# uc-vision/taichi-splatting

Measured on AMD Instinct MI355X. Metric: fwd+bwd Msplats/s, higher is better.
Workload: dtype f32; 1 GPU; config D: 6000000 random 3D gaussians, 2048x2048, SH deg 3, tile 16, fwd+bwd (render_gaussians, loss=image.sum()); n_gaussians=6000000, tile_size=16, sh_degree=3, mode=single, parallelism=single GPU

## Files before the change

### include/mi355_splat.h

```cpp
#ifndef MI355_SPLAT_H
#define MI355_SPLAT_H

#include <stddef.h>
#include <stdint.h>

#ifdef __cplusplus
extern "C" {
#endif

#define MS_VERSION 500
#define MS_ABI_GENERATION(version) ((version) / 100)

enum { MS_F32 = 0, MS_F64 = 1 };

enum {
  MS_ERR_BAD_ARG = -1,
  MS_ERR_UNSUPPORTED = -2,
  MS_ERR_TMP_TOO_SMALL = -3,
  MS_ERR_ABI = -4
};

typedef struct ms_raster_config {
  int32_t tile_size;
  int32_t antialias;
  int32_t use_alpha_blending;
  int32_t compute_visibility;
  int32_t compute_point_heuristic;
  int32_t reserved;
  double clamp_max_alpha;
  double alpha_threshold;
  double saturate_threshold;
} ms_raster_config;

int ms_version(void);
const char* ms_last_error_string(void);

int ms_project_fwd(const void* position, const void* log_scaling, const void* rotation,
                   const void* alpha_logit, const void* T_camera_world, const void* projection,
                   int image_w, int image_h, double near_plane, double far_plane,
                   double blur_cov, double clamp_margin, double alpha_threshold,
                   int64_t n, void* out_points7, void* out_depth, int32_t* out_flag,
                   int dtype, void* stream);

int ms_project_gather(const void* points7, const void* depth, const int32_t* flag,
                      const int32_t* scan, int64_t n, double near_plane, double far_plane,
                      void* out_points7, void* out_depth, void* out_ndc_depth,
                      int64_t* out_indexes, int dtype, void* stream);

int ms_project_bwd(const void* position, const void* log_scaling, const void* rotation,
                   const void* alpha_logit, const void* T_camera_world, const void* projection,
                   int image_w, int image_h, double blur_cov, double clamp_margin,
                   const int64_t* indexes, int64_t v, const void* grad_points7,
                   const void* grad_depth, void* grad_position, void* grad_log_scaling,
                   void* grad_rotation, void* grad_alpha_logit, void* grad_camera,
                   int dtype, void* stream);

int ms_sh_fwd(const void* params, const void* positions, const int64_t* indexes,
              const void* camera_pos, int64_t v, int f, int degree, void* out,
              int dtype, void* stream);

int ms_sh_fwd_active(const void* params, const void* positions, const int64_t* indexes,
                     const void* camera_pos, int64_t v, int f, int degree, int active_degree, void* out,
                     int dtype, void* stream);

int ms_sh_bwd(const void* params, const void* positions, const int64_t* indexes,
              const void* camera_pos, int64_t v, int f, int degree, const void* out,
              const void* grad_out, void* grad_params, void* grad_positions,
              void* grad_camera_pos, int unique_indexes, int dtype, void* stream);

int ms_sh_bwd_active(const void* params, const void* positions, const int64_t* indexes,
                     const void* camera_pos, int64_t v, int f, int degree, int active_degree, const void* out,
                     const void* grad_out, void* grad_params, void* grad_positions,
                     void* grad_camera_pos, int unique_indexes, int dtype, void* stream);

int ms_tile_count(const float* points7, const int32_t* order, int64_t v, int image_w, int image_h,
                  int tile_size, float alpha_threshold, int tile_row_begin, int tile_row_end,
                  int32_t* out_counts, float* out_ordered_points7 ,
                  void* stream);

int ms_depth_sort_keys(const void* depth, int64_t v, int depth16, double ndc_near, double ndc_far,
                       uint32_t* out_keys, int32_t* out_values, int dtype, void* stream);

int ms_depth_argsort(const void* depth, int64_t v, int depth16, double ndc_near, double ndc_far, int dtype,
                     uint32_t* out_sorted_keys, int32_t* out_order, void* tmp, size_t* tmp_bytes, void* stream);

int ms_exclusive_scan_i32(const int32_t* in, int64_t n, int32_t* out, int32_t* total_host,
                          void* tmp, size_t* tmp_bytes, void* stream);

int ms_tile_emit(const float* points7, const float* depth, const int32_t* order, const int32_t* cum,
                 int64_t v, int image_w, int image_h, int tile_size, float alpha_threshold,
                 int tile_row_begin, int tile_row_end, int key_mode,
                 int points_are_ordered ,
                 void* out_keys, int32_t* out_values, void* stream);

int ms_tile_emit_keys64(const float* points7, const void* depth, int depth_dtype, const int32_t* cum, int64_t v,
                        int image_w, int image_h, int tile_size, float alpha_threshold, int tile_row_begin,
                        int tile_row_end, int depth16, double ndc_near, double ndc_far, uint64_t* out_keys,
                        int32_t* out_values, void* stream);

int ms_radix_sort_pairs(const void* keys_in, const int32_t* values_in, void* keys_out,
                        int32_t* values_out, int64_t n, int key_bytes, int begin_bit, int end_bit,
                        void* tmp, size_t* tmp_bytes, void* stream);

int ms_segmented_sort_pairs(const int32_t* keys_in, const int32_t* values_in, int32_t* keys_out,
                            int32_t* values_out, int64_t n, const int64_t* start_offsets,
                            const int64_t* end_offsets, int64_t num_segments, void* stream);

int ms_find_ranges(const void* sorted_keys, int64_t k, int key_bytes, int tile_shift,
                   int64_t num_tiles, int32_t* out_ranges, void* stream);

int ms_tile_depth_sort(const int32_t* tile_ranges, int64_t num_tiles, uint64_t* sorted_keys,
                       int32_t* overlap_to_point, uint64_t* scratch, void* stream);

int ms_raster_fwd(const void* points7, const void* features, const int32_t* tile_ranges,
                  const int32_t* overlap_to_point, int image_w, int image_h, int f,
                  const ms_raster_config* cfg, void* out_image, void* out_alpha,
                  void* out_visibility, int tile_row_begin, int tile_row_end,
                  int dtype, void* stream);

int ms_raster_bwd(const void* points7, const void* features, const int32_t* tile_ranges,
                  const int32_t* overlap_to_point, const void* image, const void* grad_image,
                  int image_w, int image_h, int f, const ms_raster_config* cfg,
                  void* grad_points7, void* grad_features, void* point_heuristic,
                  int tile_row_begin, int tile_row_end, int dtype, void* stream);

#define MS_MOMENT_ROW 16
int ms_fixed_point_exponents(const float* amax_dev, int32_t* out_exp2, void* stream);
int ms_raster_bwd_moments(const void* points7, const void* features, const int32_t* tile_ranges,
                          const int32_t* overlap_to_point, const void* image, const void* grad_image,
                          int image_w, int image_h, const ms_raster_config* cfg, float* moments,
                          int deterministic, const int32_t* fixed_exp, int tile_row_begin, int tile_row_end,
                          void* stream);
int ms_raster_moments_finalize(const void* points7, const float* moments, int deterministic,
                               const int32_t* fixed_exp, int64_t n,
                               float* grad_points7, float* grad_features, float* point_heuristic,
                               void* stream);

size_t ms_raster_split_scratch_bytes(int64_t k_capacity, int tile_size, int split_min_run, int split_seg_len);
int ms_raster_fwd_split(const float* points7, const float* features, const int32_t* tile_ranges,
                        const int32_t* overlap_to_point, int64_t k_capacity, int image_w, int image_h,
                        const ms_raster_config* cfg, float* out_image, float* out_alpha, float* out_visibility,
                        void* split_scratch, int split_min_run, int split_seg_len, int tile_row_begin, int tile_row_end,
                        void* stream);
int ms_raster_bwd_moments_split(const float* points7, const float* features, const int32_t* tile_ranges,
                                const int32_t* overlap_to_point, int64_t k_capacity, const float* image,
                                const float* grad_image, int image_w, int image_h, const ms_raster_config* cfg,
                                float* moments, int deterministic, const int32_t* fixed_exp, const void* split_scratch,
                                int split_min_run, int split_seg_len, int tile_row_begin, int tile_row_end, void* stream);

int ms_probe_raster_bwd(void* start_event, void* stop_event);

#define MS_SPLAT_ROW 16
int ms_splat_rows_pack(const float* points7, const float* depth, const float* colours3, int64_t n, float* rows,
                       void* stream);
int ms_raster_fwd_rows(const float* rows, const int32_t* tile_ranges, const int32_t* overlap_to_point, int image_w,
                       int image_h, const ms_raster_config* cfg, float* out_image, float* out_alpha,
                       float* out_visibility, int tile_row_begin, int tile_row_end, void* stream);
int ms_raster_bwd_moments_rows(const float* rows, const int32_t* tile_ranges, const int32_t* overlap_to_point,
                               const float* image, const float* grad_image, int image_w, int image_h,
                               const ms_raster_config* cfg, float* moments, int deterministic,
                               const int32_t* fixed_exp, int tile_row_begin, int tile_row_end, void* stream);

#define MS_MAPPER_DIRECT 0
#define MS_MAPPER_PRESORT 1

typedef struct ms_frame_desc {
  uint32_t struct_size;
  uint32_t abi_version;
  int64_t n;
  int64_t k_capacity;
  int32_t image_w, image_h;
  int32_t dtype;
  int32_t f;
  int32_t sh_degree;
  int32_t depth16;
  int32_t tile_row_begin, tile_row_end;
  int32_t projected_input;
  int32_t mapper;
  int32_t split_long_runs;
  int32_t split_seg_len;
  int32_t sh_active_bands;
  double near_plane, far_plane, blur_cov, clamp_margin;
  ms_raster_config raster;
} ms_frame_desc;

typedef struct ms_frame_layout {
  size_t keep_n_bytes, scratch_n_bytes, keep_k_bytes, scratch_k_bytes;
  size_t points7, depth, colours, points7_f32, camera_position, counters, tile_ranges;
  size_t sorted_keys, order, counts, cum, ordered_points, tmp_n;
  size_t overlap_to_point;
  size_t keys, values, keys_sorted, tmp_k;
  size_t splat_rows;
  size_t split_scratch;
} ms_frame_layout;

typedef struct ms_frame_inputs {
  uint32_t struct_size;
  uint32_t reserved;
  const void *position, *log_scaling, *rotation, *alpha_logit, *feature, *T_camera_world, *projection;
  const void *points7, *depth, *colours;
  int32_t* longest_run_host;
  void* colours_ready_event;
} ms_frame_inputs;

enum { MS_BACKWARD_ALL = 0, MS_BACKWARD_GAUSSIANS = 1, MS_BACKWARD_RASTER = 2 };

typedef struct ms_frame_grads {
  uint32_t struct_size;
  uint32_t reserved;
  const void* image;
  const void* grad_image;
  const void *extra_points7, *extra_depth, *extra_colours;
  void* moments;
  int32_t deterministic;
  int32_t stage;
  const int32_t* fixed_exp;
  void *grad_points7, *grad_colours;
  void *grad_position, *grad_log_scaling, *grad_rotation, *grad_alpha_logit, *grad_feature, *grad_camera;
  void* point_heuristic;
  void* point_visibility;
  int32_t boundary_stride;
  int32_t gather_world;
  const void* gather_rows;
  const int32_t* gather_slots;
  const int32_t* gather_route;
  int32_t boundary_form;
  int32_t grad_image_broadcast;
} ms_frame_grads;

enum { MS_BOUNDARY_AXIS_SIGMA = 0, MS_BOUNDARY_COVARIANCE = 1 };

int ms_frame_layout_query(const ms_frame_desc* desc, ms_frame_layout* out);
int ms_frame_uses_moments(const ms_frame_desc* desc, int deterministic);
int ms_frame_project(const ms_frame_desc* desc, const ms_frame_inputs* in, void* keep_n, void* stream);
int ms_frame_project_count(const ms_frame_desc* desc, const ms_frame_inputs* in, void* keep_n, void* scratch_n,
                           int32_t* k_host, void* k_event, void* stream);
int ms_frame_sh_colours(const ms_frame_desc* desc, const ms_frame_inputs* in, void* keep_n, void* stream);
int ms_frame_map_raster(const ms_frame_desc* desc, const ms_frame_inputs* in, void* keep_n, void* scratch_n,
                        void* keep_k, void* scratch_k, void* out_image, void* out_alpha, void* out_visibility,
                        void* stream);
int ms_frame_backward(const ms_frame_desc* desc, const ms_frame_inputs* in, void* keep_n, void* keep_k,
                      const ms_frame_grads* g, void* stream);

int ms_fractional_step(int kind, int vector, float* lr_step, const int64_t* indexes,
                       const float* weight, float* m, float* v, const float* total_weight,
                       const float* grad, int64_t m_count, int d, float lr, float beta1,
                       float beta2, float eps, int bias_correction, void* stream);

int ms_fractional_update(int kind, int group_type, float* param, const float* grad, float* m, float* v,
                         const int64_t* indexes, const float* weight, const float* total_weight,
                         const float* grad_scale, const float* basis, const float* mask_lr,
                         const float* point_lr, int64_t m_count, int d, float lr, float beta1,
                         float beta2, float eps, float clip, int bias_correction, void* stream);

typedef struct ms_optim_group {
  uint32_t struct_size;
  int32_t group_type;
  float* param;
  const float* grad;
  float* m;
  float* v;
  const float* basis;
  const float* mask_lr;
  const float* point_lr;
  int32_t d;
  int32_t bias_correction;
  float lr, beta1, beta2, eps;
  float clip;
  float reserved;
} ms_optim_group;
int ms_optim_step_groups(int kind, const ms_optim_group* groups, int num_groups, const int64_t* indexes,
                         const float* weight, const float* total_weight, const float* grad_scale, int64_t m_count,
                         void* stream);

int ms_optim_visibility_weights(const int64_t* indexes, const float* visibility, int64_t m_count, float vis_beta,
                                float vis_smooth, float floor_eps, float skip_threshold, float* running_vis,
                                float* total_weight, float* out_weight, float* out_grad_scale, void* stream);

int ms_morton_codes64(const float* points3, int64_t n, const float* lower3_host, const float* inc3_host,
                      uint32_t size, uint64_t* out_codes, void* stream);

#define MS_KNN_BLOCK 256
int ms_knn_points(const float* points3, const int32_t* order, int64_t n, int k,
                  float* out_dist2, int32_t* out_index , int64_t* out_stats ,
                  void* tmp, size_t* tmp_bytes, void* stream);

int ms_camera_position(const void* t_camera_world, void* out_position3, int dtype, void* stream);

int ms_strip_route_blocks(int v);
int ms_strip_route_count(const float* points7, const float* depth ,
                         int v, int image_h, int tile_size, float alpha_threshold,
                         const int32_t* bounds_host, int world, int32_t* out_route,
                         int32_t* out_block_counts, int64_t* out_send_counts, void* stream);
int ms_strip_route_pack(const float* points7, const float* features, const float* depths,
                        const int64_t* ids, int f, int v, int world, int64_t index_offset,
                        const int32_t* route, const int32_t* block_offsets, const int64_t* send_counts,
                        int64_t bucket_capacity, int32_t* overflow_flag,
                        float* out_rows, int64_t* out_send_index, void* stream);
int ms_strip_route_pack_slots(const float* points7, const float* features, const float* depths,
                              const int64_t* ids, int f, int v, int world, int64_t index_offset,
                              const int32_t* route, const int32_t* block_offsets, const int64_t* send_counts,
                              int64_t bucket_capacity, int32_t* overflow_flag,
                              float* out_rows, int64_t* out_send_index, int32_t* out_slots, void* stream);
int ms_strip_route_pack_split(const float* points7, const float* features, const float* depths,
                              const int64_t* ids, int f, int v, int world, int64_t index_offset,
                              const int32_t* route, const int32_t* block_offsets, const int64_t* send_counts,
                              int64_t bucket_capacity, int32_t* overflow_flag, float* out_geometry_rows,
                              float* out_colour_rows, int64_t* out_send_index, int32_t* out_slots, void* stream);
int ms_strip_unpack(const float* rows, int64_t m, int f, float* out_points7, float* out_features,
                    float* out_depths, int64_t* out_ids, void* stream);
int ms_strip_return_grads(const float* back_rows, const int64_t* send_index, const int32_t* route,
                          int f, int64_t s, float* grad_points7, float* grad_features, void* stream);
int ms_strip_return_rows(const float* back_rows, const int64_t* send_index, const int32_t* route,
                         int f, int64_t s, float* grad_rows, void* stream);

int ms_densify_plan(const uint8_t* prune, const uint8_t* split, int64_t n, int children, int32_t* scan,
                    int32_t* counts, int32_t* counts_host, void* tmp, size_t* tmp_bytes, void* stream);
int ms_densify_table(const int32_t* scan, int64_t n, int children, int64_t n_out, int32_t* src_row,
                     int32_t* child_slot, void* stream);

typedef struct ms_densify_array {
  uint32_t struct_size;
  int32_t child_fill;
  const void* src;
  void* dst;
  int64_t row_bytes;
} ms_densify_array;
int ms_densify_move(const ms_densify_array* arrays, int num_arrays, const int32_t* src_row, const int32_t* child_slot,
                    int64_t n_src, int64_t n_out, void* stream);

int ms_densify_split2d(float* position, float* log_scaling, const float* rotation, float* depths, int64_t first,
                       int64_t count, int children, const float* z, const float* scale, const float* depth_offset,
                       void* stream);
int ms_densify_split3d(float* position, float* log_scaling, const float* rotation, int64_t first, int64_t count,
                       int children, const float* z, const float* scale, void* stream);

enum { MS_PAD_SAME = 0, MS_PAD_VALID = 1 };
int ms_photometric_fwd(const void* image, const void* target, int H, int W, int C, int dtype, int padding,
                       double lambda, void* map_a, void* map_b, void* map_c, void* tmp, size_t* tmp_bytes,
                       void* out_loss, void* stream);
int ms_photometric_bwd(const void* image, const void* target, const void* map_a, const void* map_b, const void* map_c,
                       const void* grad_out, int H, int W, int C, int dtype, int padding, double lambda,
                       void* grad_image, void* stream);

#define MS_SCENE_XFORM_ROWS 256
enum {
  MS_SCENE_XFORM_SRT = 0,
  MS_SCENE_XFORM_LN_S = 12,
  MS_SCENE_XFORM_QUAT = 13,
  MS_SCENE_XFORM_M1 = 17,
  MS_SCENE_XFORM_M2 = 26,
  MS_SCENE_XFORM_M3 = 51,
  MS_SCENE_XFORM_VALUES = 100
};
int ms_scene_transform(const void* position, void* out_position, const void* log_scaling, void* out_log_scaling,
                       const void* rotation, void* out_rotation, const void* feature, void* out_feature,
                       int64_t n, int f, int sh_degree, int dtype, const double* transform_host, void* stream);

#define MS_COVERAGE_CAMERA_VALUES 20
#define MS_COVERAGE_MAX_CAMERAS 65535
int ms_camera_coverage(const void* position, const void* log_scaling, const void* rotation, const void* alpha_logit,
                       const void* cameras, int num_cameras, double blur_cov, double clamp_margin,
                       double alpha_threshold, int64_t n, int32_t* out_count, void* out_max_rate, void* out_min_depth,
                       uint32_t* out_mask , int dtype, void* stream);

#define MS_RELOCATE_MAX_RATIO 51
enum { MS_RELOCATE_COPY = 0, MS_RELOCATE_ZERO_TOUCHED = 1, MS_RELOCATE_INHERIT = 2, MS_RELOCATE_OPACITY = 3,
       MS_RELOCATE_SCALE = 4 };
typedef struct ms_relocate_array {
  uint32_t struct_size;
  int32_t role;
  void* data;
  const void* fresh;
  int64_t row_bytes;
} ms_relocate_array;
int ms_relocate_weights(const float* alpha_logit, int64_t n, float threshold, int64_t* weights, int32_t* count,
                        int64_t* counts, void* stream);
int ms_relocate_draw(const int64_t* weights, const int64_t* cdf, const uint64_t* random, int64_t n, int32_t* src,
                     int32_t* count, int64_t* counts, void* stream);
int ms_relocate_fresh(const float* alpha_logit, const float* log_scaling, int scale_dims, const int32_t* count, int64_t n,
                      double min_opacity, const double* binomials, float* fresh_opacity, float* fresh_scale,
                      int64_t* counts, void* stream);
int ms_relocate_move(const ms_relocate_array* arrays, int num_arrays, const int32_t* src, const int32_t* count, int64_t n,
                     void* stream);

int ms_perturb_positions(float* position, const float* log_scaling, const float* rotation, const float* alpha_logit,
                         const float* z, int64_t n, float step, double k, double x0, void* stream);

#define MS_KMEANS_MAX_D 64
#define MS_KMEANS_MAX_K 65536
#define MS_KMEANS_CHUNK 128
#define MS_KMEANS_UPDATE_CHUNK 1024
int ms_kmeans_assign(const float* x, int64_t n, int d, const float* codebook, int k, int32_t* out_index,
                     float* out_dist2 , void* tmp, size_t* tmp_bytes, void* stream);
int ms_kmeans_update(const float* x, const int32_t* index, const float* weights , int64_t n, int d,
                     int k, float* codebook, int32_t* out_counts, double* out_weight_sums , void* tmp,
                     size_t* tmp_bytes, void* stream);

#ifdef __cplusplus
}
#endif
#endif
```

### taichi_splatting_amd/_lib.py

```python
from __future__ import annotations

import ctypes
from ctypes import c_int, c_int32, c_int64, c_double, c_float, c_void_p, c_size_t, c_char_p, POINTER
import os
from pathlib import Path
import subprocess
from typing import Optional

import torch

PACKAGE_DIR = Path(__file__).resolve().parent
CSRC_DIR = PACKAGE_DIR / 'csrc'
LIB_PATH = Path(os.environ.get('MS_SPLAT_LIB') or PACKAGE_DIR / 'libmi355_splat.so')

MS_F32, MS_F64 = 0, 1
BACKWARD_ALL, BACKWARD_GAUSSIANS, BACKWARD_RASTER = 0, 1, 2
BOUNDARY_AXIS_SIGMA, BOUNDARY_COVARIANCE = 0, 1
MAPPER_DIRECT, MAPPER_PRESORT = 0, 1
ABI_VERSION = 500
PAD_SAME, PAD_VALID = 0, 1
MOMENT_ROW = 16
SPLAT_ROW = 16
KNN_BLOCK = 256
SCENE_XFORM_ROWS = 256
SCENE_XFORM_VALUES = 100
COVERAGE_CAMERA_VALUES = 20
COVERAGE_MAX_CAMERAS = 65535
RELOCATE_MAX_RATIO = 51
KMEANS_MAX_D, KMEANS_MAX_K = 64, 65536
KMEANS_CHUNK = 128
KMEANS_UPDATE_CHUNK = 1024
RELOCATE_COPY, RELOCATE_ZERO_TOUCHED, RELOCATE_INHERIT, RELOCATE_OPACITY, RELOCATE_SCALE = range(5)

_lib: Optional[ctypes.CDLL] = None


class RasterConfigC(ctypes.Structure):
  _fields_ = [
    ('tile_size', c_int32),
    ('antialias', c_int32),
    ('use_alpha_blending', c_int32),
    ('compute_visibility', c_int32),
    ('compute_point_heuristic', c_int32),
    ('reserved', c_int32),
    ('clamp_max_alpha', c_double),
    ('alpha_threshold', c_double),
    ('saturate_threshold', c_double),
  ]


class _SizedStructure(ctypes.Structure):

  def __init__(self, *args, **kw):
    assert not args, "keyword arguments only: the leading fields are the struct's size / ABI version"
    super().__init__(**kw)
    self.struct_size = ctypes.sizeof(type(self))
    if hasattr(self, 'abi_version'):
      self.abi_version = ABI_VERSION


class FrameDescC(_SizedStructure):
  _fields_ = [
    ('struct_size', ctypes.c_uint32), ('abi_version', ctypes.c_uint32),
    ('n', c_int64), ('k_capacity', c_int64),
    ('image_w', c_int32), ('image_h', c_int32),
    ('dtype', c_int32), ('f', c_int32), ('sh_degree', c_int32), ('depth16', c_int32),
    ('tile_row_begin', c_int32), ('tile_row_end', c_int32),
    ('projected_input', c_int32), ('mapper', c_int32), ('split_long_runs', c_int32), ('split_seg_len', c_int32),
    ('sh_active_bands', c_int32),
    ('near_plane', c_double), ('far_plane', c_double), ('blur_cov', c_double), ('clamp_margin', c_double),
    ('raster', RasterConfigC),
  ]


class FrameLayoutC(ctypes.Structure):
  _fields_ = [(name, c_size_t) for name in (
    'keep_n_bytes', 'scratch_n_bytes', 'keep_k_bytes', 'scratch_k_bytes',
    'points7', 'depth', 'colours', 'points7_f32', 'camera_position', 'counters', 'tile_ranges',
    'sorted_keys', 'order', 'counts', 'cum', 'ordered_points', 'tmp_n',
    'overlap_to_point',
    'keys', 'values', 'keys_sorted', 'tmp_k',
    'splat_rows', 'split_scratch')]


class FrameInputsC(_SizedStructure):
  _fields_ = [('struct_size', ctypes.c_uint32), ('reserved', ctypes.c_uint32)] + [(name, c_void_p) for name in (
    'position', 'log_scaling', 'rotation', 'alpha_logit', 'feature', 'T_camera_world', 'projection',
    'points7', 'depth', 'colours', 'longest_run_host', 'colours_ready_event')]


class FrameGradsC(_SizedStructure):
  _fields_ = [
    ('struct_size', ctypes.c_uint32), ('reserved', ctypes.c_uint32),
    ('image', c_void_p), ('grad_image', c_void_p),
    ('extra_points7', c_void_p), ('extra_depth', c_void_p), ('extra_colours', c_void_p),
    ('moments', c_void_p), ('deterministic', c_int32), ('stage', c_int32), ('fixed_exp', c_void_p),
    ('grad_points7', c_void_p), ('grad_colours', c_void_p),
    ('grad_position', c_void_p), ('grad_log_scaling', c_void_p), ('grad_rotation', c_void_p),
    ('grad_alpha_logit', c_void_p), ('grad_feature', c_void_p), ('grad_camera', c_void_p),
    ('point_heuristic', c_void_p),
    ('point_visibility', c_void_p),
    ('boundary_stride', c_int32), ('gather_world', c_int32),
    ('gather_rows', c_void_p), ('gather_slots', c_void_p), ('gather_route', c_void_p),
    ('boundary_form', c_int32), ('grad_image_broadcast', c_int32),
  ]


class OptimGroupC(ctypes.Structure):
  _fields_ = [
    ('struct_size', ctypes.c_uint32), ('group_type', c_int32),
    ('param', c_void_p), ('grad', c_void_p), ('m', c_void_p), ('v', c_void_p),
    ('basis', c_void_p), ('mask_lr', c_void_p), ('point_lr', c_void_p),
    ('d', c_int32), ('bias_correction', c_int32),
    ('lr', c_float), ('beta1', c_float), ('beta2', c_float), ('eps', c_float), ('clip', c_float), ('reserved', c_float),
  ]


class DensifyArrayC(ctypes.Structure):
  _fields_ = [
    ('struct_size', ctypes.c_uint32), ('child_fill', c_int32),
    ('src', c_void_p), ('dst', c_void_p), ('row_bytes', c_int64),
  ]


class RelocateArrayC(ctypes.Structure):
  _fields_ = [
    ('struct_size', ctypes.c_uint32), ('role', c_int32),
    ('data', c_void_p), ('fresh', c_void_p), ('row_bytes', c_int64),
  ]


SIGNATURES = {
  'ms_version': (c_int, []),
  'ms_last_error_string': (c_char_p, []),
  'ms_project_fwd': (c_int, [c_void_p] * 6 + [c_int, c_int] + [c_double] * 5 + [c_int64, c_void_p, c_void_p, c_void_p, c_int, c_void_p]),
  'ms_project_gather': (c_int, [c_void_p] * 4 + [c_int64, c_double, c_double] + [c_void_p] * 4 + [c_int, c_void_p]),
  'ms_project_bwd': (c_int, [c_void_p] * 6 + [c_int, c_int, c_double, c_double, c_void_p, c_int64] + [c_void_p] * 7 + [c_int, c_void_p]),
  'ms_sh_fwd': (c_int, [c_void_p] * 4 + [c_int64, c_int, c_int, c_void_p, c_int, c_void_p]),
  'ms_sh_bwd': (c_int, [c_void_p] * 4 + [c_int64, c_int, c_int] + [c_void_p] * 5 + [c_int, c_int, c_void_p]),
  'ms_sh_fwd_active': (c_int, [c_void_p] * 4 + [c_int64, c_int, c_int, c_int, c_void_p, c_int, c_void_p]),
  'ms_sh_bwd_active': (c_int, [c_void_p] * 4 + [c_int64, c_int, c_int, c_int] + [c_void_p] * 5 + [c_int, c_int, c_void_p]),
  'ms_tile_count': (c_int, [c_void_p, c_void_p, c_int64, c_int, c_int, c_int, c_float, c_int, c_int, c_void_p, c_void_p, c_void_p]),
  'ms_depth_sort_keys': (c_int, [c_void_p, c_int64, c_int, c_double, c_double, c_void_p, c_void_p, c_int, c_void_p]),
  'ms_depth_argsort': (c_int, [c_void_p, c_int64, c_int, c_double, c_double, c_int, c_void_p, c_void_p, c_void_p, POINTER(c_size_t), c_void_p]),
  'ms_exclusive_scan_i32': (c_int, [c_void_p, c_int64, c_void_p, c_void_p, c_void_p, POINTER(c_size_t), c_void_p]),
  'ms_tile_emit_keys64': (c_int, [c_void_p, c_void_p, c_int, c_void_p, c_int64, c_int, c_int, c_int, c_float, c_int, c_int, c_int, ctypes.c_double, ctypes.c_double, c_void_p, c_void_p, c_void_p]),
  'ms_tile_emit': (c_int, [c_void_p, c_void_p, c_void_p, c_void_p, c_int64, c_int, c_int, c_int, c_float, c_int, c_int, c_int, c_int, c_void_p, c_void_p, c_void_p]),
  'ms_radix_sort_pairs': (c_int, [c_void_p] * 4 + [c_int64, c_int, c_int, c_int, c_void_p, POINTER(c_size_t), c_void_p]),
  'ms_segmented_sort_pairs': (c_int, [c_void_p] * 4 + [c_int64, c_void_p, c_void_p, c_int64, c_void_p]),
  'ms_find_ranges': (c_int, [c_void_p, c_int64, c_int, c_int, c_int64, c_void_p, c_void_p]),
  'ms_tile_depth_sort': (c_int, [c_void_p, c_int64, c_void_p, c_void_p, c_void_p, c_void_p]),
  'ms_fractional_step': (c_int, [c_int, c_int] + [c_void_p] * 7 + [c_int64, c_int, c_float, c_float, c_float, c_float, c_int, c_void_p]),
  'ms_morton_codes64': (c_int, [c_void_p, c_int64, c_void_p, c_void_p, ctypes.c_uint32, c_void_p, c_void_p]),
  'ms_knn_points': (c_int, [c_void_p, c_void_p, c_int64, c_int, c_void_p, c_void_p, c_void_p, c_void_p, POINTER(c_size_t), c_void_p]),
  'ms_camera_position': (c_int, [c_void_p, c_void_p, c_int, c_void_p]),
  'ms_strip_route_blocks': (c_int, [c_int]),
  'ms_strip_route_count': (c_int, [c_void_p, c_void_p, c_int, c_int, c_int, c_float, c_void_p, c_int, c_void_p, c_void_p, c_void_p, c_void_p]),
  'ms_strip_route_pack': (c_int, [c_void_p] * 4 + [c_int, c_int, c_int, c_int64] + [c_void_p] * 3 + [c_int64, c_void_p] + [c_void_p] * 2 + [c_void_p]),
  'ms_strip_unpack': (c_int, [c_void_p, c_int64, c_int] + [c_void_p] * 4 + [c_void_p]),
  'ms_strip_return_grads': (c_int, [c_void_p, c_void_p, c_void_p, c_int, c_int64, c_void_p, c_void_p, c_void_p]),
  'ms_strip_route_pack_slots': (c_int, [c_void_p] * 4 + [c_int, c_int, c_int, c_int64] + [c_void_p] * 3 + [c_int64] + [c_void_p] * 5),
  'ms_strip_route_pack_split': (c_int, [c_void_p] * 4 + [c_int, c_int, c_int, c_int64] + [c_void_p] * 3 + [c_int64] + [c_void_p] * 6),
  'ms_strip_return_rows': (c_int, [c_void_p, c_void_p, c_void_p, c_int, c_int64, c_void_p, c_void_p]),
  'ms_fractional_update': (c_int, [c_int, c_int] + [c_void_p] * 11 + [c_int64, c_int, c_float, c_float, c_float, c_float, c_float, c_int, c_void_p]),
  'ms_raster_fwd': (c_int, [c_void_p] * 4 + [c_int, c_int, c_int, POINTER(RasterConfigC)] + [c_void_p] * 3 + [c_int, c_int, c_int, c_void_p]),
  'ms_fixed_point_exponents': (c_int, [c_void_p, c_void_p, c_void_p]),
  'ms_raster_bwd_moments': (c_int, [c_void_p] * 6 + [c_int, c_int, POINTER(RasterConfigC), c_void_p, c_int, c_void_p, c_int, c_int, c_void_p]),
  'ms_raster_moments_finalize': (c_int, [c_void_p, c_void_p, c_int, c_void_p, c_int64, c_void_p, c_void_p, c_void_p, c_void_p]),
  'ms_raster_split_scratch_bytes': (c_size_t, [c_int64, c_int, c_int, c_int]),
  'ms_raster_fwd_split': (c_int, [c_void_p] * 4 + [c_int64, c_int, c_int, POINTER(RasterConfigC)] + [c_void_p] * 4 + [c_int, c_int, c_int, c_int, c_void_p]),
  'ms_raster_bwd_moments_split': (c_int, [c_void_p] * 4 + [c_int64, c_void_p, c_void_p, c_int, c_int, POINTER(RasterConfigC), c_void_p, c_int, c_void_p, c_void_p, c_int, c_int, c_int, c_int, c_void_p]),
  'ms_splat_rows_pack': (c_int, [c_void_p, c_void_p, c_void_p, c_int64, c_void_p, c_void_p]),
  'ms_raster_fwd_rows': (c_int, [c_void_p] * 3 + [c_int, c_int, POINTER(RasterConfigC)] + [c_void_p] * 3 + [c_int, c_int, c_void_p]),
  'ms_raster_bwd_moments_rows': (c_int, [c_void_p] * 5 + [c_int, c_int, POINTER(RasterConfigC), c_void_p, c_int, c_void_p, c_int, c_int, c_void_p]),
  'ms_frame_layout_query': (c_int, [POINTER(FrameDescC), POINTER(FrameLayoutC)]),
  'ms_frame_uses_moments': (c_int, [POINTER(FrameDescC), c_int]),
  'ms_frame_project': (c_int, [POINTER(FrameDescC), POINTER(FrameInputsC), c_void_p, c_void_p]),
  'ms_frame_sh_colours': (c_int, [POINTER(FrameDescC), POINTER(FrameInputsC), c_void_p, c_void_p]),
  'ms_frame_project_count': (c_int, [POINTER(FrameDescC), POINTER(FrameInputsC), c_void_p, c_void_p, c_void_p, c_void_p, c_void_p]),
  'ms_frame_map_raster': (c_int, [POINTER(FrameDescC), POINTER(FrameInputsC)] + [c_void_p] * 8),
  'ms_frame_backward': (c_int, [POINTER(FrameDescC), POINTER(FrameInputsC), c_void_p, c_void_p, POINTER(FrameGradsC), c_void_p]),
  'ms_probe_raster_bwd': (c_int, [c_void_p, c_void_p]),
  'ms_optim_step_groups': (c_int, [c_int, POINTER(OptimGroupC), c_int, c_void_p, c_void_p, c_void_p, c_void_p, c_int64, c_void_p]),
  'ms_optim_visibility_weights': (c_int, [c_void_p, c_void_p, c_int64, c_float, c_float, c_float, c_float] + [c_void_p] * 5),
  'ms_raster_bwd': (c_int, [c_void_p] * 6 + [c_int, c_int, c_int, POINTER(RasterConfigC)] + [c_void_p] * 3 + [c_int, c_int, c_int, c_void_p]),
  'ms_densify_plan': (c_int, [c_void_p, c_void_p, c_int64, c_int, c_void_p, c_void_p, c_void_p, c_void_p, POINTER(c_size_t), c_void_p]),
  'ms_densify_table': (c_int, [c_void_p, c_int64, c_int, c_int64, c_void_p, c_void_p, c_void_p]),
  'ms_densify_move': (c_int, [POINTER(DensifyArrayC), c_int, c_void_p, c_void_p, c_int64, c_int64, c_void_p]),
  'ms_densify_split2d': (c_int, [c_void_p] * 4 + [c_int64, c_int64, c_int] + [c_void_p] * 4),
  'ms_densify_split3d': (c_int, [c_void_p] * 3 + [c_int64, c_int64, c_int] + [c_void_p] * 3),
  'ms_photometric_fwd': (c_int, [c_void_p, c_void_p, c_int, c_int, c_int, c_int, c_int, c_double] + [c_void_p] * 4 + [POINTER(c_size_t), c_void_p, c_void_p]),
  'ms_photometric_bwd': (c_int, [c_void_p] * 6 + [c_int, c_int, c_int, c_int, c_int, c_double, c_void_p, c_void_p]),
  'ms_scene_transform': (c_int, [c_void_p] * 8 + [c_int64, c_int, c_int, c_int, POINTER(c_double), c_void_p]),
  'ms_camera_coverage': (c_int, [c_void_p] * 5 + [c_int, c_double, c_double, c_double, c_int64] + [c_void_p] * 4 + [c_int, c_void_p]),
  'ms_relocate_weights': (c_int, [c_void_p, c_int64, c_float] + [c_void_p] * 4),
  'ms_relocate_draw': (c_int, [c_void_p] * 3 + [c_int64] + [c_void_p] * 4),
  'ms_relocate_fresh': (c_int, [c_void_p, c_void_p, c_int, c_void_p, c_int64, c_double] + [c_void_p] * 5),
  'ms_relocate_move': (c_int, [POINTER(RelocateArrayC), c_int, c_void_p, c_void_p, c_int64, c_void_p]),
  'ms_perturb_positions': (c_int, [c_void_p] * 5 + [c_int64, c_float, c_double, c_double, c_void_p]),
  'ms_kmeans_assign': (c_int, [c_void_p, c_int64, c_int, c_void_p, c_int, c_void_p, c_void_p, c_void_p, POINTER(c_size_t), c_void_p]),
  'ms_kmeans_update': (c_int, [c_void_p] * 3 + [c_int64, c_int, c_int] + [c_void_p] * 4 + [POINTER(c_size_t), c_void_p]),
}


def build(verbose: bool = False, jobs: Optional[int] = None) -> Path:
  jobs = jobs or os.cpu_count() or 4
  cmd = ['make', '-C', str(CSRC_DIR), f'-j{jobs}']
  proc = subprocess.run(cmd, capture_output=True, text=True)
  if proc.returncode != 0:
    raise RuntimeError(f"building libmi355_splat.so failed:\n{proc.stdout}\n{proc.stderr}")
  if verbose:
    print(proc.stdout)
  return LIB_PATH


def load() -> ctypes.CDLL:
  global _lib
  if _lib is not None:
    return _lib
  if not LIB_PATH.exists():
    raise RuntimeError(
      f"{LIB_PATH} not found: the gfx950 kernel library has not been built. "
      "Run `python -c 'import __graft_entry__ as g; g.build()'` or `make -C taichi_splatting_amd/csrc`. "
      "There is no CPU fallback for this path.")
  lib = ctypes.CDLL(str(LIB_PATH))
  for name, (restype, argtypes) in SIGNATURES.items():
    fn = getattr(lib, name)
    fn.restype = restype
    fn.argtypes = argtypes
  _lib = lib
  return lib


def check(rc: int, what: str):
  if rc != 0:
    msg = load().ms_last_error_string().decode('utf-8', 'replace')
    if rc == -2:
      raise NotImplementedError(f"{what}: {msg}")
    if rc == -4:
      raise RuntimeError(f"{what}: ABI mismatch between taichi_splatting_amd/_lib.py and libmi355_splat.so: {msg}")
    if rc < 0:
      raise ValueError(f"{what}: {msg}")
    raise RuntimeError(f"{what}: HIP error {rc}: {msg}")


def ptr(t: Optional[torch.Tensor]) -> Optional[int]:
  if t is None:
    return None
  assert t.is_contiguous(), "tensor must be contiguous"
  return t.data_ptr()


def require_gpu(*tensors: torch.Tensor):
  for t in tensors:
    if t is not None and not t.is_cuda:
      raise RuntimeError(
        "taichi_splatting_amd runs on MI355X (gfx950) only: got a tensor on "
        f"{t.device}. There is no CPU fallback; move the inputs to the GPU.")


def dtype_code(dtype: torch.dtype) -> int:
  if dtype == torch.float32:
    return MS_F32
  if dtype == torch.float64:
    return MS_F64
  raise TypeError(f"unsupported dtype {dtype}: float32 or float64 expected")


def current_stream(device) -> int:
  return torch.cuda.current_stream(device).cuda_stream


def raster_config_c(config) -> RasterConfigC:
  return RasterConfigC(
    tile_size=config.tile_size, antialias=int(config.antialias),
    use_alpha_blending=int(config.use_alpha_blending),
    compute_visibility=int(config.compute_visibility),
    compute_point_heuristic=int(config.compute_point_heuristic), reserved=0,
    clamp_max_alpha=config.clamp_max_alpha, alpha_threshold=config.alpha_threshold,
    saturate_threshold=config.saturate_threshold)


def fixed_point_exponents(grad_image: torch.Tensor) -> torch.Tensor:
  amax = grad_image.detach().abs().amax().to(torch.float32).reshape(1)
  out = torch.empty((2,), dtype=torch.int32, device=grad_image.device)
  check(load().ms_fixed_point_exponents(amax.data_ptr(), out.data_ptr(), current_stream(grad_image.device)),
        "fixed_point_exponents")
  return out
```

### taichi_splatting_amd/csrc/frame.hip

```cpp
#include <cstdlib>
#include <cstring>
#include "common.h"
#include "frame_internal.h"
#include "raster_common.h"

namespace ms {

struct FrameGeom {
  int w_pad, h_pad, tiles_wide, tiles_high, num_tiles, tile_bits, row_begin, row_end;
  size_t es;
};

static FrameGeom frame_geom(const ms_frame_desc* d) {
  FrameGeom g;
  const int ts = d->raster.tile_size;
  g.tiles_wide = (d->image_w + ts - 1) / ts;
  g.tiles_high = (d->image_h + ts - 1) / ts;
  g.w_pad = g.tiles_wide * ts;
  g.h_pad = g.tiles_high * ts;
  g.num_tiles = g.tiles_wide * g.tiles_high;
  int bits = 1;
  while ((1ll << bits) < (long long)g.num_tiles) ++bits;
  g.tile_bits = bits;
  g.row_begin = d->tile_row_begin < 0 ? 0 : d->tile_row_begin;
  g.row_end = d->tile_row_end > g.tiles_high ? g.tiles_high : d->tile_row_end;
  g.es = d->dtype == MS_F64 ? 8 : 4;
  return g;
}

static int check_desc(const ms_frame_desc* d, const char* who) {
  if (!d) { set_error("%s: desc is null", who); return MS_ERR_BAD_ARG; }
  if (d->struct_size != sizeof(ms_frame_desc) || MS_ABI_GENERATION(d->abi_version) != MS_ABI_GENERATION(MS_VERSION)) {
    set_error("%s: ms_frame_desc of another ABI (struct_size %u, abi_version %u; this library: %u, %d) — set desc.struct_size = "
              "sizeof(ms_frame_desc) and desc.abi_version = MS_VERSION of the include/mi355_splat.h you compile against",
              who, d->struct_size, d->abi_version, (unsigned)sizeof(ms_frame_desc), MS_VERSION);
    return MS_ERR_ABI;
  }
  if (d->split_long_runs < 0 || d->split_seg_len < 0) { set_error("%s: negative split parameter", who); return MS_ERR_BAD_ARG; }
  if (d->n < 0 || d->k_capacity < 0) { set_error("%s: negative size", who); return MS_ERR_BAD_ARG; }
  if (d->n >= (1ll << 31) || d->k_capacity >= (1ll << 31)) { set_error("%s: sizes are int32 indexes (< 2^31)", who); return MS_ERR_BAD_ARG; }
  if (d->image_w <= 0 || d->image_h <= 0) { set_error("%s: bad image size", who); return MS_ERR_BAD_ARG; }
  if (d->dtype != MS_F32 && d->dtype != MS_F64) { set_error("%s: dtype must be MS_F32 or MS_F64", who); return MS_ERR_BAD_ARG; }
  const int ts = d->raster.tile_size;
  if (ts != 8 && ts != 16 && ts != 32) { set_error("%s: tile_size must be 8, 16 or 32 (got %d)", who, ts); return MS_ERR_UNSUPPORTED; }
  if (d->f < 1 || d->f > 4) { set_error("%s: 1..4 colour channels (got %d)", who, d->f); return MS_ERR_UNSUPPORTED; }
  if (d->sh_degree < -1 || d->sh_degree > 3) { set_error("%s: SH degree must be in [0, 3]", who); return MS_ERR_BAD_ARG; }
  if (d->sh_active_bands < 0 || d->sh_active_bands > d->sh_degree + 1) {
    set_error("%s: sh_active_bands must be 0 (all) or 1 .. sh_degree + 1 (got %d with sh_degree %d)", who, d->sh_active_bands, d->sh_degree);
    return MS_ERR_BAD_ARG;
  }
  if (d->mapper != MS_MAPPER_DIRECT && d->mapper != MS_MAPPER_PRESORT) { set_error("%s: mapper must be MS_MAPPER_DIRECT or MS_MAPPER_PRESORT (got %d)", who, d->mapper); return MS_ERR_BAD_ARG; }
  if (d->projected_input && d->sh_degree >= 0) { set_error("%s: projected input carries colours, not SH", who); return MS_ERR_BAD_ARG; }
  if (d->depth16) {
    const FrameGeom g = frame_geom(d);
    if (g.num_tiles > 65536) { set_error("%s: use_depth16 keys hold a 16 bit tile id: too many tiles", who); return MS_ERR_BAD_ARG; }
  }
  return 0;
}

static bool frame_uses_rows(const ms_frame_desc* d) {
  static const bool on = [] { const char* e = getenv("MS_SPLAT_ROWS"); return e && e[0] == '1'; }();
  return on && !d->projected_input && d->n > 0 && raster_uses_splat_rows(&d->raster, d->f, d->dtype);
}

static bool frame_uses_split(const ms_frame_desc* d) {
  return d->split_long_runs != 0 && d->n > 0 && d->k_capacity > 0 && raster_uses_splat_rows(&d->raster, d->f, d->dtype);
}
static SplitParams frame_split_params(const ms_frame_desc* d) {
  return split_params(d->raster.tile_size, d->split_long_runs, d->split_seg_len);
}

static int check_inputs(const ms_frame_inputs* in, const char* who) {
  if (!in) { set_error("%s: inputs are null", who); return MS_ERR_BAD_ARG; }
  if (in->struct_size != sizeof(ms_frame_inputs)) {
    set_error("%s: ms_frame_inputs of another ABI (struct_size %u, this library: %u)", who, in->struct_size, (unsigned)sizeof(ms_frame_inputs));
    return MS_ERR_ABI;
  }
  return 0;
}

static int check_grads(const ms_frame_grads* g, const char* who) {
  if (!g) { set_error("%s: grads are null", who); return MS_ERR_BAD_ARG; }
  if (g->struct_size != sizeof(ms_frame_grads)) {
    set_error("%s: ms_frame_grads of another ABI (struct_size %u, this library: %u)", who, g->struct_size, (unsigned)sizeof(ms_frame_grads));
    return MS_ERR_ABI;
  }
  return 0;
}

struct Carve {
  size_t off = 0;
  size_t take(size_t bytes) { const size_t o = off; off += align_up(bytes > 0 ? bytes : 1, 256); return o; }
};

static void frame_layout(const ms_frame_desc* d, ms_frame_layout* L) {
  const FrameGeom g = frame_geom(d);
  const size_t n = (size_t)d->n, k = (size_t)d->k_capacity;
  const bool own_points = !d->projected_input;
  Carve keep_n, scratch_n, keep_k, scratch_k;
  L->points7 = keep_n.take(own_points ? n * 7 * g.es : 0);
  L->depth = keep_n.take(own_points ? n * g.es : 0);
  L->colours = keep_n.take(d->sh_degree >= 0 ? n * d->f * g.es : 0);
  L->camera_position = keep_n.take(4 * g.es);
  L->counters = keep_n.take(8 * sizeof(int32_t));
  L->tile_ranges = keep_n.take((size_t)g.num_tiles * 2 * sizeof(int32_t));
  L->splat_rows = keep_n.take(frame_uses_rows(d) ? n * SPLAT_ROW * sizeof(float) : 0);
  L->keep_n_bytes = keep_n.off;

  L->sorted_keys = scratch_n.take(n * 4);
  L->order = scratch_n.take(n * 4);
  L->counts = scratch_n.take(n * 4);
  L->cum = scratch_n.take((n + 1) * 4);
  L->ordered_points = scratch_n.take(n * 7 * 4);
  L->points7_f32 = scratch_n.take(d->dtype == MS_F64 ? n * 7 * 4 : 0);
  const size_t t1 = sort_tmp_size(d->n, 4, true), t2 = scan_tmp_size(d->n);
  L->tmp_n = scratch_n.take(t1 > t2 ? t1 : t2);
  L->scratch_n_bytes = scratch_n.off;

  L->overlap_to_point = keep_k.take(k * 4);
  L->split_scratch = keep_k.take(frame_uses_split(d) ? split_scratch_bytes(d->k_capacity, d->raster.tile_size, frame_split_params(d)) : 0);
  L->keep_k_bytes = keep_k.off;

  L->keys = scratch_k.take(k * 8);
  L->values = scratch_k.take(k * 4);
  L->keys_sorted = scratch_k.take(k * 8);
  L->tmp_k = scratch_k.take(sort_tmp_size(d->k_capacity, 8));
  L->scratch_k_bytes = scratch_k.off;
}

template <typename T>
__global__ void __launch_bounds__(256)
frame_prepare_kernel(int32_t* __restrict__ counters, int32_t capacity, const T* __restrict__ Tcw, T* __restrict__ cam_out,
                     int32_t* __restrict__ ranges, int64_t range_words) {
  const int64_t i = (int64_t)blockIdx.x * blockDim.x + threadIdx.x;
  if (i < range_words) ranges[i] = 0;
  if (i == 0) {
    const int32_t k = counters[0];
    const bool ok = k >= 0 && k <= capacity;
    counters[1] = ok ? k : 0;
    counters[2] = ok ? 0 : 1;
    counters[3] = 0;
    counters[4] = 0;
    counters[5] = 0;
    if (cam_out) camera_position_solve(Tcw, cam_out);
  }
}

__global__ void __launch_bounds__(256)
f64_to_f32_kernel(const double* __restrict__ in, float* __restrict__ out, int64_t count) {
  const int64_t i = (int64_t)blockIdx.x * blockDim.x + threadIdx.x;
  if (i < count) out[i] = (float)in[i];
}

static bool mapper_presort(const ms_frame_desc& d) {
  static const int forced = [] {
    const char* e = getenv("MS_MAPPER");
    if (e && strcmp(e, "presort") == 0) return MS_MAPPER_PRESORT;
    if (e && strcmp(e, "direct") == 0) return MS_MAPPER_DIRECT;
    return -1;
  }();
  return (forced >= 0 ? forced : d.mapper) == MS_MAPPER_PRESORT;
}

static bool frame_uses_moments(const ms_frame_desc* d, int deterministic) {
  (void)deterministic;
  return d->dtype == MS_F32 && d->f == 3 && !d->raster.antialias && d->raster.use_alpha_blending;
}

}

using namespace ms;

extern "C" int ms_frame_layout_query(const ms_frame_desc* desc, ms_frame_layout* out) {
  int rc = check_desc(desc, "ms_frame_layout_query");
  if (rc) return rc;
  MS_CHECK_ARG(out != nullptr, "out is null");
  frame_layout(desc, out);
  return 0;
}

extern "C" int ms_frame_uses_moments(const ms_frame_desc* desc, int deterministic) {
  return desc && frame_uses_moments(desc, deterministic) ? 1 : 0;
}

#define MS_TRY(expr)            \
  do {                          \
    const int rc__ = (expr);    \
    if (rc__ != 0) return rc__; \
  } while (0)

static int frame_project_impl(const ms_frame_desc* desc, const ms_frame_inputs* in, void* keep_n, bool projection,
                              bool colours, void* stream, const char* who) {
  const ms_frame_desc& d = *desc;
  if (d.projected_input) { set_error("%s: projected input has no per-gaussian stage", who); return MS_ERR_BAD_ARG; }
  if (d.n == 0) return 0;
  ms_frame_layout L;
  frame_layout(desc, &L);
  char* kn = (char*)keep_n;
  if (!(in->position && in->log_scaling && in->rotation && in->alpha_logit && in->T_camera_world && in->projection)) {
    set_error("%s: null gaussian / camera input", who); return MS_ERR_BAD_ARG;
  }
  if (!in->feature) { set_error("%s: feature is null", who); return MS_ERR_BAD_ARG; }
  float* rows = frame_uses_rows(desc) ? (float*)(kn + L.splat_rows) : nullptr;
  if (projection) {
    if (d.sh_degree >= 0 && colours)
      MS_TRY(ms_camera_position(in->T_camera_world, kn + L.camera_position, d.dtype, stream));
    MS_TRY(project_fwd_launch(in->position, in->log_scaling, in->rotation, in->alpha_logit, in->T_camera_world, in->projection,
                              d.image_w, d.image_h, d.near_plane, d.far_plane, d.blur_cov, d.clamp_margin,
                              d.raster.alpha_threshold, d.n, kn + L.points7, kn + L.depth, nullptr, d.dtype, stream, rows,
                              rows && d.sh_degree < 0 ? in->feature : nullptr));
  }
  if (colours && d.sh_degree >= 0)
    MS_TRY(sh_fwd_inplace_launch(in->feature, in->position, kn + L.depth, kn + L.camera_position, d.n, d.f,
                                 d.sh_degree, d.sh_active_bands > 0 ? d.sh_active_bands - 1 : d.sh_degree, kn + L.colours,
                                 d.dtype, (hipStream_t)stream, rows));
  return 0;
}

extern "C" int ms_frame_project(const ms_frame_desc* desc, const ms_frame_inputs* in, void* keep_n, void* stream) {
  MS_TRY(check_desc(desc, "ms_frame_project"));
  MS_TRY(check_inputs(in, "ms_frame_project"));
  MS_CHECK_ARG(in && keep_n, "null pointer");
  return frame_project_impl(desc, in, keep_n, true, true, stream, "ms_frame_project");
}

extern "C" int ms_frame_sh_colours(const ms_frame_desc* desc, const ms_frame_inputs* in, void* keep_n, void* stream) {
  MS_TRY(check_desc(desc, "ms_frame_sh_colours"));
  MS_TRY(check_inputs(in, "ms_frame_sh_colours"));
  MS_CHECK_ARG(in && keep_n, "null pointer");
  const ms_frame_desc& d = *desc;
  MS_CHECK_ARG(!d.projected_input && d.sh_degree >= 0, "a frame that evaluates SH colours itself");
  MS_CHECK_ARG(!frame_uses_rows(desc), "the splat-row table is filled on the frame's own stream");
  if (d.n == 0) return 0;
  ms_frame_layout L;
  frame_layout(desc, &L);
  MS_CHECK_ARG(in->T_camera_world != nullptr, "T_camera_world is null");
  MS_TRY(ms_camera_position(in->T_camera_world, (char*)keep_n + L.camera_position, d.dtype, stream));
  return frame_project_impl(desc, in, keep_n, false, true, stream, "ms_frame_sh_colours");
}

extern "C" int ms_frame_project_count(const ms_frame_desc* desc, const ms_frame_inputs* in, void* keep_n,
                                      void* scratch_n, int32_t* k_host, void* k_event, void* stream) {
  MS_TRY(check_desc(desc, "ms_frame_project_count"));
  MS_TRY(check_inputs(in, "ms_frame_project_count"));
  MS_CHECK_ARG(in && keep_n && scratch_n, "null pointer");
  const ms_frame_desc& d = *desc;
  const FrameGeom g = frame_geom(desc);
  ms_frame_layout L;
  frame_layout(desc, &L);
  hipStream_t s = (hipStream_t)stream;
  char* kn = (char*)keep_n;
  char* sn = (char*)scratch_n;
  int32_t* counters = (int32_t*)(kn + L.counters);

  if (d.n == 0) {
    MS_CHECK_HIP(hipMemsetAsync(counters, 0, 8 * sizeof(int32_t), s));
    if (k_host) *k_host = 0;
    if (k_event) MS_CHECK_HIP(hipEventRecord((hipEvent_t)k_event, s));
    return 0;
  }

  const void* points7;
  const void* depth;
  if (!d.projected_input) {
    MS_TRY(frame_project_impl(desc, in, keep_n, true, false, stream, "ms_frame_project_count"));
    points7 = kn + L.points7;
    depth = kn + L.depth;
  } else {
    MS_CHECK_ARG(in->points7 && in->depth && in->colours, "null projected input");
    points7 = in->points7;
    depth = in->depth;
  }

  const float* points_f32 = (const float*)points7;
  if (d.dtype == MS_F64) {
    float* copy = (float*)(sn + L.points7_f32);
    f64_to_f32_kernel<<<dim3((unsigned)div_up(d.n * 7, 256)), dim3(256), 0, s>>>((const double*)points7, copy, d.n * 7);
    points_f32 = copy;
  }

  uint32_t* sorted_keys = (uint32_t*)(sn + L.sorted_keys);
  int32_t* order = (int32_t*)(sn + L.order);
  int32_t* counts = (int32_t*)(sn + L.counts);
  int32_t* cum = (int32_t*)(sn + L.cum);
  const int cull = d.projected_input ? 0 : 1;
  if (mapper_presort(d)) {
    depth_argsort_launch(depth, d.n, d.depth16, d.near_plane > 0.0 ? d.near_plane : 0.0, d.far_plane, d.dtype, cull,
                         sorted_keys, order, sn + L.tmp_n, s);
    tile_count_launch(points_f32, order, cull ? sorted_keys : nullptr, d.n, g.w_pad, g.h_pad, d.raster.tile_size,
                      (float)d.raster.alpha_threshold, g.row_begin, g.row_end, counts, (float*)(sn + L.ordered_points), s);
  } else {
    tile_count_direct_launch(points_f32, cull ? depth : nullptr, d.dtype, d.n, g.w_pad, g.h_pad, d.raster.tile_size,
                             (float)d.raster.alpha_threshold, g.row_begin, g.row_end, counts, s);
  }
  exclusive_scan_launch(counts, d.n, cum, k_host, sn + L.tmp_n, s, counters);
  MS_CHECK_LAUNCH();
  if (k_event) MS_CHECK_HIP(hipEventRecord((hipEvent_t)k_event, s));
  return 0;
}

extern "C" int ms_frame_map_raster(const ms_frame_desc* desc, const ms_frame_inputs* in, void* keep_n, void* scratch_n,
                                   void* keep_k, void* scratch_k, void* out_image, void* out_alpha,
                                   void* out_visibility, void* stream) {
  MS_TRY(check_desc(desc, "ms_frame_map_raster"));
  MS_TRY(check_inputs(in, "ms_frame_map_raster"));
  MS_CHECK_ARG(in && keep_n && scratch_n && out_image && out_alpha, "null pointer");
  const ms_frame_desc& d = *desc;
  const FrameGeom g = frame_geom(desc);
  ms_frame_layout L;
  frame_layout(desc, &L);
  hipStream_t s = (hipStream_t)stream;
  char* kn = (char*)keep_n;
  char* sn = (char*)scratch_n;
  char* kk = (char*)keep_k;
  char* sk = (char*)scratch_k;
  int32_t* counters = (int32_t*)(kn + L.counters);
  int32_t* ranges = (int32_t*)(kn + L.tile_ranges);
  int32_t* o2p = (int32_t*)(kk + L.overlap_to_point);
  const bool colours_elsewhere = !d.projected_input && d.sh_degree >= 0 && in->colours_ready_event != nullptr;

  {
    const bool want_cam = !d.projected_input && d.sh_degree >= 0 && d.n > 0 && !colours_elsewhere;
    if (want_cam) MS_CHECK_ARG(in->T_camera_world != nullptr, "T_camera_world is null");
    const int64_t words = (int64_t)g.num_tiles * 2;
    const dim3 grid((unsigned)(words > 0 ? div_up(words, 256) : 1)), block(256);
    if (d.dtype == MS_F64)
      frame_prepare_kernel<double><<<grid, block, 0, s>>>(counters, (int32_t)d.k_capacity, (const double*)in->T_camera_world,
                                                          want_cam ? (double*)(kn + L.camera_position) : nullptr, ranges, words);
    else
      frame_prepare_kernel<float><<<grid, block, 0, s>>>(counters, (int32_t)d.k_capacity, (const float*)in->T_camera_world,
                                                         want_cam ? (float*)(kn + L.camera_position) : nullptr, ranges, words);
  }
  if (!d.projected_input && !colours_elsewhere) MS_TRY(frame_project_impl(desc, in, keep_n, false, true, stream, "ms_frame_map_raster"));
  if (d.n > 0 && d.k_capacity > 0) {
    MS_CHECK_ARG(keep_k && scratch_k, "null overlap buffers");
    int32_t* values = (int32_t*)(sk + L.values);
    if (mapper_presort(d)) {
      uint32_t* keys = (uint32_t*)(sk + L.keys);
      uint32_t* keys_sorted = (uint32_t*)(sk + L.keys_sorted);
      tile_emit_ordered_launch((const float*)(sn + L.ordered_points), (const int32_t*)(sn + L.order),
                               (const int32_t*)(sn + L.cum), d.n, g.w_pad, g.h_pad, d.raster.tile_size,
                               (float)d.raster.alpha_threshold, g.row_begin, g.row_end, counters + 1, keys, values, s);
      sort_pairs_u32_dev_launch(keys, values, keys_sorted, o2p, d.k_capacity, counters + 1, g.tile_bits, sk + L.tmp_k, s);
      MS_TRY(find_ranges_dev_launch(keys_sorted, d.k_capacity, counters + 1, g.num_tiles, ranges, s, true));
    } else {
      uint64_t* keys = (uint64_t*)(sk + L.keys);
      uint64_t* keys_sorted = (uint64_t*)(sk + L.keys_sorted);
      const void* depth = d.projected_input ? in->depth : (const void*)(kn + L.depth);
      const float* points_f32 = d.dtype == MS_F64 ? (const float*)(sn + L.points7_f32)
                                                  : (const float*)(d.projected_input ? in->points7 : (const void*)(kn + L.points7));
      tile_emit_direct_launch(points_f32, depth, d.dtype, (const int32_t*)(sn + L.cum), d.n, g.w_pad, g.h_pad,
                              d.raster.tile_size, (float)d.raster.alpha_threshold, g.row_begin, g.row_end, d.depth16,
                              d.near_plane > 0.0 ? d.near_plane : 0.0, d.far_plane, counters + 1, keys, values, s);
      sort_pairs_u64_dev_launch(keys, values, keys_sorted, o2p, d.k_capacity, counters + 1, 32, 32 + g.tile_bits,
                                sk + L.tmp_k, s);
      MS_TRY(find_ranges_u64_dev_launch(keys_sorted, d.k_capacity, counters + 1, g.num_tiles, ranges, s));
      const int64_t first_tile = (int64_t)g.row_begin * g.tiles_wide;
      const int64_t strip_tiles = (int64_t)(g.row_end > g.row_begin ? g.row_end - g.row_begin : 0) * g.tiles_wide;
      tile_depth_sort_launch(ranges + 2 * first_tile, strip_tiles, keys_sorted, o2p, keys, s, counters + 3, in->longest_run_host);
    }
  }
  MS_CHECK_LAUNCH();

  const void* points7 = d.projected_input ? in->points7 : (const void*)(kn + L.points7);
  const void* colours = d.sh_degree >= 0 ? (const void*)(kn + L.colours) : (d.projected_input ? in->colours : in->feature);
  MS_CHECK_ARG(d.n == 0 || colours != nullptr, "colours are null");
  SplitScratch split{};
  const bool cut = frame_uses_split(desc) && keep_k != nullptr;
  if (cut) split = split_scratch_carve(kk + L.split_scratch, d.k_capacity, d.raster.tile_size, frame_split_params(desc));
  if (in->colours_ready_event) MS_CHECK_HIP(hipStreamWaitEvent(s, (hipEvent_t)in->colours_ready_event, 0));
  return raster_fwd_launch(points7, colours, frame_uses_rows(desc) ? (const float*)(kn + L.splat_rows) : nullptr, ranges, o2p,
                           d.image_w, d.image_h, d.f, &d.raster, out_image, out_alpha, out_visibility, g.row_begin, g.row_end,
                           d.dtype, stream, cut ? &split : nullptr, in->longest_run_host);
}

extern "C" int ms_frame_backward(const ms_frame_desc* desc, const ms_frame_inputs* in, void* keep_n, void* keep_k,
                                 const ms_frame_grads* gr, void* stream) {
  MS_TRY(check_desc(desc, "ms_frame_backward"));
  MS_TRY(check_inputs(in, "ms_frame_backward"));
  MS_TRY(check_grads(gr, "ms_frame_backward"));
  MS_CHECK_ARG(in && keep_n && gr, "null pointer");
  MS_CHECK_ARG(gr->stage == MS_BACKWARD_GAUSSIANS || (gr->image && gr->grad_image), "null image / grad_image");
  const ms_frame_desc& d = *desc;
  const FrameGeom g = frame_geom(desc);
  ms_frame_layout L;
  frame_layout(desc, &L);
  hipStream_t s = (hipStream_t)stream;
  char* kn = (char*)keep_n;
  char* kk = (char*)keep_k;
  const int32_t* ranges = (const int32_t*)(kn + L.tile_ranges);
  const int32_t* o2p = (const int32_t*)(kk + L.overlap_to_point);
  const void* points7 = d.projected_input ? in->points7 : (const void*)(kn + L.points7);
  const void* depth = d.projected_input ? in->depth : (const void*)(kn + L.depth);
  const void* colours = d.sh_degree >= 0 ? (const void*)(kn + L.colours) : (d.projected_input ? in->colours : in->feature);
  if (d.n == 0) return 0;

  const bool given = gr->stage == MS_BACKWARD_GAUSSIANS;
  const bool raster_only = gr->stage == MS_BACKWARD_RASTER || d.projected_input;
  const bool moments = !given && frame_uses_moments(desc, gr->deterministic);
  MS_CHECK_ARG(!gr->grad_image_broadcast || (!given && moments), "grad_image_broadcast: moments path only (float32 RGB, plain pdf)");
  MS_CHECK_ARG(gr->boundary_form == MS_BOUNDARY_AXIS_SIGMA || gr->boundary_form == MS_BOUNDARY_COVARIANCE, "boundary_form");
  MS_CHECK_ARG(gr->boundary_form == 0 || given || (moments && gr->stage == MS_BACKWARD_RASTER),
               "MS_BOUNDARY_COVARIANCE rows: MS_BACKWARD_GAUSSIANS, or MS_BACKWARD_RASTER on the moments path");
  if (gr->boundary_stride != 0) {
    MS_CHECK_ARG(gr->boundary_stride >= 7 + d.f && d.dtype == MS_F32, "boundary_stride: rows of >= 7 + f floats, float32 frames");
    MS_CHECK_ARG(given || (moments && raster_only), "boundary_stride: MS_BACKWARD_GAUSSIANS, or MS_BACKWARD_RASTER on the moments path");
  }
  if (given) {
    MS_CHECK_ARG(!d.projected_input, "projected input has no per-gaussian backward");
    if (gr->gather_world > 0)
      MS_CHECK_ARG(gr->gather_rows && gr->gather_slots && gr->gather_route && gr->boundary_stride >= 7 + d.f && d.dtype == MS_F32,
                   "gathered boundary gradients: rows, slots, route, boundary_stride >= 7 + f, float32");
    else
      MS_CHECK_ARG(gr->grad_points7 != nullptr, "grad_points7 is null");
  } else if (moments) {
    MS_CHECK_ARG(gr->moments != nullptr, "moments is null");
    SplitScratch split{};
    const bool cut = frame_uses_split(desc) && keep_k != nullptr;
    if (cut) split = split_scratch_carve(kk + L.split_scratch, d.k_capacity, d.raster.tile_size, frame_split_params(desc));
    MS_TRY(raster_bwd_moments_launch(points7, colours, ranges, o2p, gr->image, gr->grad_image, d.image_w, d.image_h, &d.raster,
                                     (float*)gr->moments, gr->deterministic, gr->fixed_exp, g.row_begin, g.row_end,
                                     gr->grad_image_broadcast, s,
                                     frame_uses_rows(desc) ? (const float*)(kn + L.splat_rows) : nullptr,
                                     cut ? &split : nullptr));
    if (raster_only)
      return moments_finalize_rezero_launch((const float*)points7, (float*)gr->moments, gr->deterministic, gr->fixed_exp,
                                            d.n, (float*)gr->grad_points7, (float*)gr->grad_colours,
                                            d.raster.compute_point_heuristic ? (float*)gr->point_heuristic : nullptr, s,
                                            gr->boundary_stride, d.projected_input && gr->stage != MS_BACKWARD_RASTER ? 0 : gr->boundary_form);
  } else {
    MS_CHECK_ARG(gr->grad_points7 || gr->grad_colours, "no gradient accumulator");
    MS_TRY(ms_raster_bwd(points7, colours, ranges, o2p, gr->image, gr->grad_image, d.image_w, d.image_h, d.f, &d.raster,
                         gr->grad_points7, gr->grad_colours, d.raster.compute_point_heuristic ? gr->point_heuristic : nullptr,
                         g.row_begin, g.row_end, d.dtype, stream));
    if (raster_only) return 0;
  }

  GaussianBwdArgs a{};
  a.dtype = d.dtype;
  a.n = d.n;
  a.position = in->position; a.log_scaling = in->log_scaling; a.rotation = in->rotation; a.alpha_logit = in->alpha_logit;
  a.T_camera_world = in->T_camera_world; a.projection = in->projection;
  a.image_w = d.image_w; a.image_h = d.image_h;
  a.blur_cov = d.blur_cov; a.clamp_margin = d.clamp_margin;
  a.depth = depth;
  if (moments) {
    a.moments = gr->moments; a.deterministic = gr->deterministic; a.fixed_exp = gr->fixed_exp;
    a.store_points7 = gr->grad_points7; a.store_colours = gr->grad_colours;
    a.point_heuristic = d.raster.compute_point_heuristic ? gr->point_heuristic : nullptr;
    a.point_visibility = d.raster.compute_point_heuristic ? gr->point_visibility : nullptr;
  } else {
    a.grad_points7 = gr->grad_points7; a.grad_colours = gr->grad_colours;
    a.boundary_stride = gr->boundary_stride;
    a.boundary_cov = given ? gr->boundary_form : 0;
    if (given && gr->gather_world > 0) {
      a.gather_world = gr->gather_world; a.gather_rows = gr->gather_rows;
      a.gather_slots = gr->gather_slots; a.gather_route = gr->gather_route;
    }
  }
  a.extra_points7 = gr->extra_points7; a.extra_depth = gr->extra_depth; a.extra_colours = gr->extra_colours;
  a.sh_degree = d.sh_degree; a.f = d.f; a.sh_active_bands = d.sh_active_bands;
  a.camera_position = kn + L.camera_position; a.colours = colours;
  a.grad_position = gr->grad_position; a.grad_log_scaling = gr->grad_log_scaling; a.grad_rotation = gr->grad_rotation;
  a.grad_alpha_logit = gr->grad_alpha_logit; a.grad_feature = gr->grad_feature; a.grad_camera = gr->grad_camera;
  return gaussian_bwd_launch(a, s);
}
```

### taichi_splatting_amd/csrc/frame_internal.h

```cpp
#pragma once
#include "common.h"

namespace ms {

constexpr uint32_t CULLED_DEPTH_KEY = 0xffffffffu;

template <typename T>
__device__ inline void camera_position_solve(const T* __restrict__ m, T* __restrict__ out) {
#pragma clang fp contract(off)
  double a[4][5];
  for (int r = 0; r < 4; ++r) {
    for (int c = 0; c < 4; ++c) a[r][c] = (double)m[r * 4 + c];
    a[r][4] = r == 3 ? 1.0 : 0.0;
  }
  for (int col = 0; col < 4; ++col) {
    int piv = col;
    for (int r = col + 1; r < 4; ++r)
      if (fabs(a[r][col]) > fabs(a[piv][col])) piv = r;
    for (int c = 0; c < 5; ++c) { const double t = a[col][c]; a[col][c] = a[piv][c]; a[piv][c] = t; }
    const double inv = 1.0 / a[col][col];
    for (int c = 0; c < 5; ++c) a[col][c] *= inv;
    for (int r = 0; r < 4; ++r) {
      if (r == col) continue;
      const double fct = a[r][col];
      for (int c = 0; c < 5; ++c) a[r][c] -= fct * a[col][c];
    }
  }
  for (int k = 0; k < 3; ++k) out[k] = (T)a[k][4];
}

size_t scan_tmp_size(int64_t n);
size_t sort_tmp_size(int64_t n, int key_bytes, bool adaptive = false);
void exclusive_scan_launch(const int32_t* in, int64_t n, int32_t* out, int32_t* total_host, void* tmp, hipStream_t s,
                           int32_t* total_copy = nullptr);
void depth_argsort_launch(const void* depth, int64_t n, int depth16, double ndc_near, double ndc_far, int dtype,
                          int cull, uint32_t* out_sorted_keys, int32_t* out_order, char* tmp, hipStream_t s);
void sort_pairs_u32_dev_launch(const uint32_t* keys_in, const int32_t* vals_in, uint32_t* keys_out, int32_t* vals_out,
                               int64_t capacity, const int32_t* n_dev, int end_bit, char* tmp, hipStream_t s);
int find_ranges_dev_launch(const uint32_t* sorted_keys, int64_t capacity, const int32_t* k_dev, int64_t num_tiles,
                           int32_t* out_ranges, hipStream_t s, bool zeroed = false);

void sort_pairs_u64_dev_launch(const uint64_t* keys_in, const int32_t* vals_in, uint64_t* keys_out, int32_t* vals_out,
                               int64_t capacity, const int32_t* n_dev, int begin_bit, int end_bit, char* tmp, hipStream_t s);
int find_ranges_u64_dev_launch(const uint64_t* sorted_keys, int64_t capacity, const int32_t* k_dev, int64_t num_tiles,
                               int32_t* out_ranges, hipStream_t s);

void tile_count_launch(const float* points7, const int32_t* order, const uint32_t* cull_keys, int64_t v, int image_w,
                       int image_h, int tile_size, float alpha_threshold, int row_begin, int row_end,
                       int32_t* out_counts, float* out_ordered, hipStream_t s);
void tile_emit_ordered_launch(const float* ordered_points7, const int32_t* order, const int32_t* cum, int64_t v,
                              int image_w, int image_h, int tile_size, float alpha_threshold, int row_begin,
                              int row_end, const int32_t* k_limit_dev, uint32_t* out_keys, int32_t* out_values,
                              hipStream_t s);

void tile_count_direct_launch(const float* points7, const void* cull_depth, int dtype, int64_t v, int image_w, int image_h,
                              int tile_size, float alpha_threshold, int row_begin, int row_end, int32_t* out_counts,
                              hipStream_t s);
void tile_emit_direct_launch(const float* points7, const void* depth, int dtype, const int32_t* cum, int64_t v, int image_w,
                             int image_h, int tile_size, float alpha_threshold, int row_begin, int row_end, int depth16,
                             double ndc_near, double ndc_far, const int32_t* k_limit_dev, uint64_t* out_keys,
                             int32_t* out_values, hipStream_t s);

void tile_depth_sort_launch(const int32_t* tile_ranges, int64_t num_tiles, uint64_t* sorted_keys, int32_t* overlap_to_point,
                            uint64_t* scratch, hipStream_t s, int32_t* run_stats = nullptr, int32_t* run_host = nullptr);

int project_fwd_launch(const void* position, const void* log_scaling, const void* rotation, const void* alpha_logit,
                       const void* T_camera_world, const void* projection, int image_w, int image_h, double near_plane,
                       double far_plane, double blur_cov, double clamp_margin, double alpha_threshold, int64_t n,
                       void* out_points7, void* out_depth, int32_t* out_flag, int dtype, void* stream, float* splat_rows,
                       const void* colours_in);

int sh_fwd_inplace_launch(const void* params, const void* positions, const void* depth, const void* cam_pos,
                          int64_t n, int f, int degree, int active_degree, void* out, int dtype, hipStream_t s,
                          float* splat_rows = nullptr);

bool raster_uses_splat_rows(const ms_raster_config* cfg, int f, int dtype);
int raster_fwd_launch(const void* points7, const void* features, const float* splat_rows, const int32_t* tile_ranges,
                      const int32_t* overlap_to_point, int image_w, int image_h, int f, const ms_raster_config* cfg,
                      void* out_image, void* out_alpha, void* out_visibility, int tile_row_begin, int tile_row_end,
                      int dtype, void* stream, const struct SplitScratch* split = nullptr, int32_t* long_run_word = nullptr);

int raster_bwd_moments_launch(const void* points7, const void* features, const int32_t* tile_ranges,
                              const int32_t* overlap_to_point, const void* image, const void* grad_image, int image_w,
                              int image_h, const ms_raster_config* cfg, float* moments, int deterministic,
                              const int32_t* fixed_exp, int tile_row_begin, int tile_row_end, int grad_broadcast,
                              hipStream_t s, const float* splat_rows = nullptr, const struct SplitScratch* split = nullptr);
int moments_finalize_rezero_launch(const float* points7, float* moments, int deterministic, const int32_t* fixed_exp,
                                   int64_t n, float* grad_points7, float* grad_features, float* point_heuristic,
                                   hipStream_t s, int row_stride = 0, int covariance_form = 0);

struct GaussianBwdArgs {
  int dtype;
  int64_t n;
  const void *position, *log_scaling, *rotation, *alpha_logit, *T_camera_world, *projection;
  int image_w, image_h;
  double blur_cov, clamp_margin;
  const void* depth;
  void* moments;
  int deterministic;
  const int32_t* fixed_exp;
  const void* grad_points7;
  const void* grad_colours;
  int boundary_cov;
  int boundary_stride;
  int gather_world;
  const void* gather_rows;
  const int32_t *gather_slots, *gather_route;
  const void *extra_points7, *extra_depth, *extra_colours;
  int sh_degree, f;
  int sh_active_bands;
  const void *camera_position, *colours;
  void *grad_position, *grad_log_scaling, *grad_rotation, *grad_alpha_logit;
  void* grad_feature;
  void* grad_camera;
  void *store_points7, *store_colours;
  void* point_heuristic;
  void* point_visibility;
};
int gaussian_bwd_launch(const GaussianBwdArgs& a, hipStream_t s);

}
```

### taichi_splatting_amd/csrc/mapper.hip

```cpp
#pragma clang fp contract(off)
#include "common.h"
#include "frame_internal.h"

namespace ms {

__device__ __forceinline__ void load_point7(const float* __restrict__ points, int64_t i, float g[7]) {
#pragma unroll
  for (int k = 0; k < 7; ++k) g[k] = points[i * 7 + k];
}


__device__ __forceinline__ float readlane_f(float v, int lane) {
  return __int_as_float(__builtin_amdgcn_readlane(__float_as_int(v), lane));
}
__device__ __forceinline__ ObbQuery wave_broadcast(const ObbQuery& q, int lane) {
  ObbQuery r;
  r.inv00 = readlane_f(q.inv00, lane); r.inv01 = readlane_f(q.inv01, lane);
  r.inv10 = readlane_f(q.inv10, lane); r.inv11 = readlane_f(q.inv11, lane);
  r.rel_min_x = readlane_f(q.rel_min_x, lane); r.rel_min_y = readlane_f(q.rel_min_y, lane);
  r.min_tile_x = __builtin_amdgcn_readlane(q.min_tile_x, lane); r.min_tile_y = __builtin_amdgcn_readlane(q.min_tile_y, lane);
  r.span_x = __builtin_amdgcn_readlane(q.span_x, lane); r.span_y = __builtin_amdgcn_readlane(q.span_y, lane);
  return r;
}
__device__ __forceinline__ unsigned long long wide_span_lanes(const ObbQuery& q, bool valid, int* my_span) {
  const int span = valid && q.span_x > 0 && q.span_y > 0 ? q.span_x * q.span_y : 0;
  *my_span = span;
  const int total = (int)readlane_f(wave_sum_to_lane63((float)span), 63);
  int thr = total / 32;
  thr = thr > 16 ? thr : 16;
  return __ballot(span > thr);
}
template <typename F>
__device__ __forceinline__ void wave_walk_span(const ObbQuery& b, int tile_size, int row_begin, int row_end, F on_hits) {
  const int n = b.span_x * b.span_y, lane = lane_id();
  for (int base = 0; base < n; base += 64) {
    const int idx = base + lane;
    bool hit = false;
    int tu = 0, tv = 0;
    if (idx < n) {
      tv = idx / b.span_x; tu = idx - tv * b.span_x;
      const int ty = b.min_tile_y + tv;
      hit = ty >= row_begin && ty < row_end && obb_test_tile(b, tu, tv, tile_size);
    }
    on_hits(hit, b.min_tile_x + tu, b.min_tile_y + tv);
  }
}
__device__ __forceinline__ int count_span(const ObbQuery& q, bool valid, int tile_size, int row_begin, int row_end) {
  int span;
  unsigned long long wide = wide_span_lanes(q, valid, &span);
  const bool mine_is_wide = (wide >> lane_id()) & 1ull;
  int count = 0;
  if (span > 0 && !mine_is_wide) {
    for (int tv = 0; tv < q.span_y; ++tv) {
      const int ty = q.min_tile_y + tv;
      if (ty < row_begin || ty >= row_end) continue;
      for (int tu = 0; tu < q.span_x; ++tu)
        if (obb_test_tile(q, tu, tv, tile_size)) ++count;
    }
  }
  while (wide != 0) {
    const int src = __builtin_ctzll(wide);
    wide &= wide - 1;
    const ObbQuery b = wave_broadcast(q, src);
    int total = 0;
    wave_walk_span(b, tile_size, row_begin, row_end, [&](bool hit, int, int) { total += __builtin_popcountll(__ballot(hit)); });
    if (lane_id() == src) count = total;
  }
  return count;
}
template <typename F>
__device__ __forceinline__ void emit_span(const ObbQuery& q, bool valid, int64_t first, int tile_size, int row_begin,
                                          int row_end, F emit) {
  int span;
  unsigned long long wide = wide_span_lanes(q, valid, &span);
  const bool mine_is_wide = (wide >> lane_id()) & 1ull;
  if (span > 0 && !mine_is_wide) {
    int64_t o = first;
    for (int tu = 0; tu < q.span_x; ++tu) {
      for (int tv = 0; tv < q.span_y; ++tv) {
        const int ty = q.min_tile_y + tv;
        if (ty < row_begin || ty >= row_end) continue;
        if (obb_test_tile(q, tu, tv, tile_size)) emit(o++, q.min_tile_x + tu, ty, -1);
      }
    }
  }
  while (wide != 0) {
    const int src = __builtin_ctzll(wide);
    wide &= wide - 1;
    const ObbQuery b = wave_broadcast(q, src);
    const int lo = __builtin_amdgcn_readlane((int)(uint32_t)first, src), hi = __builtin_amdgcn_readlane((int)(uint32_t)(first >> 32), src);
    int64_t o = (int64_t)(((uint64_t)(uint32_t)hi << 32) | (uint32_t)lo);
    wave_walk_span(b, tile_size, row_begin, row_end, [&](bool hit, int tx, int ty) {
      const unsigned long long m = __ballot(hit);
      if (hit) emit(o + (int)__builtin_amdgcn_mbcnt_hi((uint32_t)(m >> 32), __builtin_amdgcn_mbcnt_lo((uint32_t)m, 0u)), tx, ty, src);
      o += __builtin_popcountll(m);
    });
  }
}

__global__ void __launch_bounds__(256)
tile_count_kernel(const float* __restrict__ points, const int32_t* __restrict__ order,
                  const uint32_t* __restrict__ cull_keys, int64_t v, int image_w,
                  int image_h, int tile_size, float alpha_threshold, int row_begin, int row_end,
                  int32_t* __restrict__ counts, float* __restrict__ ordered_points) {
  const int64_t i = (int64_t)blockIdx.x * blockDim.x + threadIdx.x;
  const bool valid = i < v && !(cull_keys && cull_keys[i] == CULLED_DEPTH_KEY);
  float g[7] = {0.f, 0.f, 1.f, 0.f, 1.f, 1.f, 0.f};
  if (valid) {
    load_point7(points, order ? (int64_t)order[i] : i, g);
    if (ordered_points) {
#pragma unroll
      for (int k = 0; k < 7; ++k) ordered_points[i * 7 + k] = g[k];
    }
  }
  const ObbQuery q = obb_grid_query(g, image_w, image_h, tile_size, alpha_threshold);
  const int count = count_span(q, valid, tile_size, row_begin, row_end);
  if (i < v) counts[i] = count;
}

template <typename KeyT, int MODE>
__global__ void __launch_bounds__(256)
tile_emit_kernel(const float* __restrict__ points, const float* __restrict__ depth,
                 const int32_t* __restrict__ order, const int32_t* __restrict__ cum, int64_t v,
                 int image_w, int image_h, int tile_size, float alpha_threshold, int row_begin,
                 int row_end, int points_ordered, const int32_t* __restrict__ k_limit,
                 KeyT* __restrict__ keys, int32_t* __restrict__ values) {
  const int64_t i = (int64_t)blockIdx.x * blockDim.x + threadIdx.x;
  if (k_limit && *k_limit == 0) return;
  const bool valid = i < v && !(k_limit && cum[i + 1] == cum[i]);
  const int64_t src = valid ? (order ? (int64_t)order[i] : i) : 0;
  float g[7] = {0.f, 0.f, 1.f, 0.f, 1.f, 1.f, 0.f};
  if (valid) load_point7(points, points_ordered ? i : src, g);
  const ObbQuery q = obb_grid_query(g, image_w, image_h, tile_size, alpha_threshold);
  const int tiles_wide = image_w / tile_size;
  KeyT depth_key = 0;
  if (valid) {
    if (MODE == 1) {
      const float c = fminf(fmaxf(depth[src], 0.0f), 1.0f);
      depth_key = (KeyT)(uint32_t)(c * 65535.0f);
    } else if (MODE == 0) {
      depth_key = (KeyT)__float_as_uint(depth[src]);
    }
  }
  const uint32_t dk_lo = (uint32_t)depth_key, dk_hi = (uint32_t)((uint64_t)depth_key >> 32);
  emit_span(q, valid, valid ? (int64_t)cum[i] : 0, tile_size, row_begin, row_end, [&](int64_t o, int tx, int ty, int from) {
    const int64_t tile_id = (int64_t)tx + (int64_t)ty * tiles_wide;
    KeyT dk = depth_key;
    int32_t who = (int32_t)src;
    if (from >= 0) {
      dk = (KeyT)(((uint64_t)(uint32_t)__builtin_amdgcn_readlane((int)dk_hi, from) << 32) | (uint32_t)__builtin_amdgcn_readlane((int)dk_lo, from));
      who = __builtin_amdgcn_readlane((int32_t)src, from);
    }
    if constexpr (MODE == 2) keys[o] = (KeyT)tile_id;
    else if constexpr (MODE == 1) keys[o] = (KeyT)(dk | ((KeyT)tile_id << 16));
    else keys[o] = (KeyT)(dk | ((KeyT)tile_id << 32));
    values[o] = who;
  });
}

template <typename T>
__global__ void __launch_bounds__(256, 8)
tile_count_direct_kernel(const float* __restrict__ points, const T* __restrict__ cull_depth, int64_t v, int image_w,
                         int image_h, int tile_size, float alpha_threshold, int row_begin, int row_end,
                         int32_t* __restrict__ counts) {
  const int64_t i = (int64_t)blockIdx.x * blockDim.x + threadIdx.x;
  const bool valid = i < v && !(cull_depth && !(cull_depth[i] > T(0)));
  float g[7] = {0.f, 0.f, 1.f, 0.f, 1.f, 1.f, 0.f};
  if (valid) load_point7(points, i, g);
  const ObbQuery q = obb_grid_query(g, image_w, image_h, tile_size, alpha_threshold);
  const int count = count_span(q, valid, tile_size, row_begin, row_end);
  if (i < v) counts[i] = count;
}

template <typename T>
__global__ void __launch_bounds__(256)
tile_emit_direct_kernel(const float* __restrict__ points, const T* __restrict__ depth, const int32_t* __restrict__ cum,
                        int64_t v, int image_w, int image_h, int tile_size, float alpha_threshold, int row_begin,
                        int row_end, int depth16, double near_plane, double far_plane,
                        const int32_t* __restrict__ k_limit, uint64_t* __restrict__ keys, int32_t* __restrict__ values) {
  const int64_t i = (int64_t)blockIdx.x * blockDim.x + threadIdx.x;
  if (k_limit && *k_limit == 0) return;
  const int64_t first = i < v ? (int64_t)cum[i] : 0;
  const bool valid = i < v && cum[i + 1] != first;
  float g[7] = {0.f, 0.f, 1.f, 0.f, 1.f, 1.f, 0.f};
  if (valid) load_point7(points, i, g);
  const ObbQuery q = obb_grid_query(g, image_w, image_h, tile_size, alpha_threshold);
  const int tiles_wide = image_w / tile_size;
  const uint32_t depth_key = valid ? (uint32_t)depth_sort_key(depth[i], depth16, near_plane, far_plane) : 0u;
  emit_span(q, valid, first, tile_size, row_begin, row_end, [&](int64_t o, int tx, int ty, int from) {
    const uint64_t tile_id = (uint64_t)((int64_t)tx + (int64_t)ty * tiles_wide);
    uint32_t dk = depth_key;
    int32_t who = (int32_t)i;
    if (from >= 0) { dk = (uint32_t)__builtin_amdgcn_readlane((int)depth_key, from); who = __builtin_amdgcn_readlane((int32_t)i, from); }
    keys[o] = (tile_id << 32) | dk;
    values[o] = who;
  });
}

template <typename T>
__global__ void __launch_bounds__(256)
depth_keys_kernel(const T* __restrict__ depth, int64_t v, int depth16, double near_plane, double far_plane,
                  uint32_t* __restrict__ keys, int32_t* __restrict__ values) {
  const int64_t i = (int64_t)blockIdx.x * blockDim.x + threadIdx.x;
  if (i >= v) return;
  keys[i] = depth_sort_key(depth[i], depth16, near_plane, far_plane);
  values[i] = (int32_t)i;
}

void tile_count_launch(const float* points7, const int32_t* order, const uint32_t* cull_keys, int64_t v, int image_w,
                       int image_h, int tile_size, float alpha_threshold, int row_begin, int row_end,
                       int32_t* out_counts, float* out_ordered, hipStream_t s) {
  tile_count_kernel<<<dim3((unsigned)div_up(v, 256)), dim3(256), 0, s>>>(
      points7, order, cull_keys, v, image_w, image_h, tile_size, alpha_threshold, row_begin, row_end, out_counts, out_ordered);
}

void tile_emit_ordered_launch(const float* ordered_points7, const int32_t* order, const int32_t* cum, int64_t v,
                              int image_w, int image_h, int tile_size, float alpha_threshold, int row_begin,
                              int row_end, const int32_t* k_limit_dev, uint32_t* out_keys, int32_t* out_values,
                              hipStream_t s) {
  tile_emit_kernel<uint32_t, 2><<<dim3((unsigned)div_up(v, 256)), dim3(256), 0, s>>>(
      ordered_points7, nullptr, order, cum, v, image_w, image_h, tile_size, alpha_threshold, row_begin, row_end, 1,
      k_limit_dev, out_keys, out_values);
}

void tile_count_direct_launch(const float* points7, const void* cull_depth, int dtype, int64_t v, int image_w, int image_h,
                              int tile_size, float alpha_threshold, int row_begin, int row_end, int32_t* out_counts,
                              hipStream_t s) {
  const dim3 grid((unsigned)div_up(v, 256)), block(256);
  if (dtype == MS_F64)
    tile_count_direct_kernel<double><<<grid, block, 0, s>>>(points7, (const double*)cull_depth, v, image_w, image_h, tile_size,
                                                            alpha_threshold, row_begin, row_end, out_counts);
  else
    tile_count_direct_kernel<float><<<grid, block, 0, s>>>(points7, (const float*)cull_depth, v, image_w, image_h, tile_size,
                                                           alpha_threshold, row_begin, row_end, out_counts);
}

void tile_emit_direct_launch(const float* points7, const void* depth, int dtype, const int32_t* cum, int64_t v, int image_w,
                             int image_h, int tile_size, float alpha_threshold, int row_begin, int row_end, int depth16,
                             double ndc_near, double ndc_far, const int32_t* k_limit_dev, uint64_t* out_keys,
                             int32_t* out_values, hipStream_t s) {
  const dim3 grid((unsigned)div_up(v, 256)), block(256);
  if (dtype == MS_F64)
    tile_emit_direct_kernel<double><<<grid, block, 0, s>>>(points7, (const double*)depth, cum, v, image_w, image_h, tile_size,
                                                           alpha_threshold, row_begin, row_end, depth16, ndc_near, ndc_far,
                                                           k_limit_dev, out_keys, out_values);
  else
    tile_emit_direct_kernel<float><<<grid, block, 0, s>>>(points7, (const float*)depth, cum, v, image_w, image_h, tile_size,
                                                          alpha_threshold, row_begin, row_end, depth16, ndc_near, ndc_far,
                                                          k_limit_dev, out_keys, out_values);
}

}

using namespace ms;

extern "C" int ms_depth_sort_keys(const void* depth, int64_t v, int depth16, double ndc_near, double ndc_far,
                                  uint32_t* out_keys, int32_t* out_values, int dtype, void* stream) {
  MS_CHECK_ARG(v >= 0, "v < 0");
  MS_CHECK_ARG(dtype == MS_F32 || dtype == MS_F64, "dtype must be MS_F32 or MS_F64");
  if (v == 0) return 0;
  MS_CHECK_ARG(depth && out_keys && out_values, "null pointer");
  const dim3 grid((unsigned)div_up(v, 256)), block(256);
  if (dtype == MS_F32)
    depth_keys_kernel<float><<<grid, block, 0, (hipStream_t)stream>>>((const float*)depth, v, depth16, ndc_near, ndc_far, out_keys, out_values);
  else
    depth_keys_kernel<double><<<grid, block, 0, (hipStream_t)stream>>>((const double*)depth, v, depth16, ndc_near, ndc_far, out_keys, out_values);
  MS_CHECK_LAUNCH();
  return 0;
}

extern "C" int ms_tile_count(const float* points7, const int32_t* order, int64_t v, int image_w, int image_h, int tile_size,
                             float alpha_threshold, int tile_row_begin, int tile_row_end,
                             int32_t* out_counts, float* out_ordered_points7, void* stream) {
  MS_CHECK_ARG(v >= 0, "v < 0");
  MS_CHECK_ARG(tile_size > 0 && image_w > 0 && image_h > 0, "bad image/tile size");
  MS_CHECK_ARG(image_w % tile_size == 0 && image_h % tile_size == 0, "image size must be padded to the tile size");
  if (v == 0) return 0;
  MS_CHECK_ARG(points7 && out_counts, "null pointer");
  tile_count_kernel<<<dim3((unsigned)div_up(v, 256)), dim3(256), 0, (hipStream_t)stream>>>(
      points7, order, nullptr, v, image_w, image_h, tile_size, alpha_threshold, tile_row_begin, tile_row_end, out_counts, out_ordered_points7);
  MS_CHECK_LAUNCH();
  return 0;
}

extern "C" int ms_tile_emit(const float* points7, const float* depth, const int32_t* order, const int32_t* cum,
                            int64_t v, int image_w, int image_h, int tile_size, float alpha_threshold,
                            int tile_row_begin, int tile_row_end, int key_mode, int points_are_ordered,
                            void* out_keys, int32_t* out_values, void* stream) {
  MS_CHECK_ARG(v >= 0, "v < 0");
  MS_CHECK_ARG(key_mode >= 0 && key_mode <= 2, "key_mode must be 0 (tile|depth32), 1 (tile|depth16) or 2 (tile only)");
  MS_CHECK_ARG(tile_size > 0 && image_w > 0 && image_h > 0, "bad image/tile size");
  MS_CHECK_ARG(image_w % tile_size == 0 && image_h % tile_size == 0, "image size must be padded to the tile size");
  if (key_mode == 1) {
    const int64_t tiles = (int64_t)(image_w / tile_size) * (image_h / tile_size);
    MS_CHECK_ARG(tiles <= 65536, "use_depth16 keys hold a 16 bit tile id: too many tiles");
  }
  if (v == 0) return 0;
  MS_CHECK_ARG(points7 && cum && out_keys && out_values, "null pointer");
  MS_CHECK_ARG(key_mode == 2 || depth, "depth is null");
  const dim3 block(256), grid((unsigned)div_up(v, 256));
  hipStream_t s = (hipStream_t)stream;
#define MS_EMIT(KeyT, MODE) tile_emit_kernel<KeyT, MODE><<<grid, block, 0, s>>>(points7, depth, order, cum, v, image_w, image_h, tile_size, alpha_threshold, tile_row_begin, tile_row_end, points_are_ordered, nullptr, (KeyT*)out_keys, out_values)
  if (key_mode == 0) MS_EMIT(uint64_t, 0);
  else if (key_mode == 1) MS_EMIT(uint32_t, 1);
  else MS_EMIT(uint32_t, 2);
#undef MS_EMIT
  MS_CHECK_LAUNCH();
  return 0;
}

extern "C" int ms_tile_emit_keys64(const float* points7, const void* depth, int depth_dtype, const int32_t* cum, int64_t v,
                                   int image_w, int image_h, int tile_size, float alpha_threshold, int tile_row_begin,
                                   int tile_row_end, int depth16, double ndc_near, double ndc_far, uint64_t* out_keys,
                                   int32_t* out_values, void* stream) {
  MS_CHECK_ARG(v >= 0, "v < 0");
  MS_CHECK_ARG(depth_dtype == MS_F32 || depth_dtype == MS_F64, "depth_dtype must be MS_F32 or MS_F64");
  MS_CHECK_ARG(tile_size > 0 && image_w > 0 && image_h > 0, "bad image/tile size");
  MS_CHECK_ARG(image_w % tile_size == 0 && image_h % tile_size == 0, "image size must be padded to the tile size");
  if (depth16) {
    const int64_t tiles = (int64_t)(image_w / tile_size) * (image_h / tile_size);
    MS_CHECK_ARG(tiles <= 65536, "use_depth16 keys hold a 16 bit tile id: too many tiles");
  }
  if (v == 0) return 0;
  MS_CHECK_ARG(points7 && depth && cum && out_keys && out_values, "null pointer");
  tile_emit_direct_launch(points7, depth, depth_dtype, cum, v, image_w, image_h, tile_size, alpha_threshold, tile_row_begin,
                          tile_row_end, depth16, ndc_near > 0.0 ? ndc_near : 0.0, ndc_far, nullptr, out_keys, out_values,
                          (hipStream_t)stream);
  MS_CHECK_LAUNCH();
  return 0;
}
```

### taichi_splatting_amd/csrc/scan_sort.hip

```cpp
#include "common.h"
#include "frame_internal.h"

namespace ms {

constexpr int SCAN_THREADS = 256;
constexpr int SCAN_ITEMS = 16;
constexpr int SCAN_TILE = SCAN_THREADS * SCAN_ITEMS;

__device__ __forceinline__ int block_exclusive_scan(int v, int* lds , int* block_total) {
  const int lane = lane_id(), wave = threadIdx.x >> 6;
  int incl = v;
#pragma unroll
  for (int off = 1; off < 64; off <<= 1) {
    const int t = __shfl_up(incl, off, 64);
    if (lane >= off) incl += t;
  }
  if (lane == 63) lds[wave] = incl;
  __syncthreads();
  int wave_off = 0, total = 0;
#pragma unroll
  for (int w = 0; w < SCAN_THREADS / 64; ++w) {
    const int s = lds[w];
    if (w < wave) wave_off += s;
    total += s;
  }
  __syncthreads();
  *block_total = total;
  return wave_off + incl - v;
}

__device__ __forceinline__ void load_items(const int32_t* __restrict__ in, int64_t base, int64_t n, int (&vals)[SCAN_ITEMS]) {
  if (base + SCAN_ITEMS <= n && (reinterpret_cast<uintptr_t>(in + base) & 15) == 0) {
    const int4* p = reinterpret_cast<const int4*>(in + base);
#pragma unroll
    for (int q = 0; q < SCAN_ITEMS / 4; ++q) {
      const int4 v = p[q];
      vals[4 * q] = v.x; vals[4 * q + 1] = v.y; vals[4 * q + 2] = v.z; vals[4 * q + 3] = v.w;
    }
  } else {
#pragma unroll
    for (int k = 0; k < SCAN_ITEMS; ++k) vals[k] = base + k < n ? in[base + k] : 0;
  }
}

__device__ __forceinline__ void store_items(int32_t* __restrict__ out, int64_t base, int64_t n, const int (&vals)[SCAN_ITEMS]) {
  if (base + SCAN_ITEMS <= n && (reinterpret_cast<uintptr_t>(out + base) & 15) == 0) {
    int4* p = reinterpret_cast<int4*>(out + base);
#pragma unroll
    for (int q = 0; q < SCAN_ITEMS / 4; ++q) p[q] = make_int4(vals[4 * q], vals[4 * q + 1], vals[4 * q + 2], vals[4 * q + 3]);
  } else {
#pragma unroll
    for (int k = 0; k < SCAN_ITEMS; ++k) if (base + k < n) out[base + k] = vals[k];
  }
}

__global__ void __launch_bounds__(SCAN_THREADS)
scan_block_sums_kernel(const int32_t* __restrict__ in, int64_t n, int32_t* __restrict__ block_sums) {
  __shared__ int lds[4];
  const int64_t base = (int64_t)blockIdx.x * SCAN_TILE + (int64_t)threadIdx.x * SCAN_ITEMS;
  int items[SCAN_ITEMS];
  load_items(in, base, n, items);
  int s = 0;
#pragma unroll
  for (int k = 0; k < SCAN_ITEMS; ++k) s += items[k];
  int total;
  block_exclusive_scan(s, lds, &total);
  if (threadIdx.x == 0) block_sums[blockIdx.x] = total;
}

__global__ void __launch_bounds__(SCAN_THREADS)
scan_spine_kernel(int32_t* __restrict__ block_sums, int64_t num_blocks, int32_t* __restrict__ total_out,
                  int32_t* __restrict__ total_host, int32_t* __restrict__ total_copy = nullptr) {
  __shared__ int lds[4];
  int carry = 0;
  for (int64_t base = 0; base < num_blocks; base += SCAN_THREADS) {
    const int64_t i = base + threadIdx.x;
    const int v = i < num_blocks ? block_sums[i] : 0;
    int total;
    const int ex = block_exclusive_scan(v, lds, &total);
    if (i < num_blocks) block_sums[i] = carry + ex;
    carry += total;
  }
  if (threadIdx.x == 0) {
    *total_out = carry;
    if (total_copy) *total_copy = carry;
    if (total_host) *total_host = carry;
  }
}

__global__ void __launch_bounds__(SCAN_THREADS)
scan_downsweep_kernel(const int32_t* __restrict__ in, int64_t n, const int32_t* __restrict__ block_offsets,
                      int32_t* __restrict__ out) {
  __shared__ int lds[4];
  const int64_t base = (int64_t)blockIdx.x * SCAN_TILE + (int64_t)threadIdx.x * SCAN_ITEMS;
  int vals[SCAN_ITEMS];
  load_items(in, base, n, vals);
  int s = 0;
#pragma unroll
  for (int k = 0; k < SCAN_ITEMS; ++k) s += vals[k];
  int total;
  int prefix = block_exclusive_scan(s, lds, &total) + block_offsets[blockIdx.x];
#pragma unroll
  for (int k = 0; k < SCAN_ITEMS; ++k) {
    const int v = vals[k];
    vals[k] = prefix;
    prefix += v;
  }
  store_items(out, base, n, vals);
}

constexpr int64_t SCAN_SELF_MAX_BLOCKS = 8192;

__global__ void __launch_bounds__(SCAN_THREADS)
scan_downsweep_self_kernel(const int32_t* __restrict__ in, int64_t n, const int32_t* __restrict__ block_sums,
                           int32_t* __restrict__ out, int32_t* __restrict__ total_host,
                           int32_t* __restrict__ total_copy = nullptr) {
  __shared__ int lds[4];
  int before = 0;
  for (int j = threadIdx.x; j < (int)blockIdx.x; j += SCAN_THREADS) before += block_sums[j];
  int block_prefix;
  block_exclusive_scan(before, lds, &block_prefix);

  const int64_t base = (int64_t)blockIdx.x * SCAN_TILE + (int64_t)threadIdx.x * SCAN_ITEMS;
  int vals[SCAN_ITEMS];
  load_items(in, base, n, vals);
  int s = 0;
#pragma unroll
  for (int k = 0; k < SCAN_ITEMS; ++k) s += vals[k];
  int total;
  int prefix = block_exclusive_scan(s, lds, &total) + block_prefix;
#pragma unroll
  for (int k = 0; k < SCAN_ITEMS; ++k) {
    const int v = vals[k];
    vals[k] = prefix;
    prefix += v;
  }
  store_items(out, base, n, vals);
  if (blockIdx.x == gridDim.x - 1 && threadIdx.x == 0) {
    out[n] = block_prefix + total;
    if (total_copy) *total_copy = block_prefix + total;
    if (total_host) *total_host = block_prefix + total;
  }
}

static size_t scan_tmp_bytes(int64_t n) { return align_up((size_t)div_up(n > 0 ? n : 1, SCAN_TILE) * sizeof(int32_t), 256); }

static int exclusive_scan_i32(const int32_t* in, int64_t n, int32_t* out, int32_t* total_host, void* tmp,
                              hipStream_t s, int32_t* total_copy = nullptr) {
  const int64_t blocks = div_up(n, SCAN_TILE);
  int32_t* block_sums = (int32_t*)tmp;
  scan_block_sums_kernel<<<dim3((unsigned)blocks), dim3(SCAN_THREADS), 0, s>>>(in, n, block_sums);
  if (blocks <= SCAN_SELF_MAX_BLOCKS) {
    scan_downsweep_self_kernel<<<dim3((unsigned)blocks), dim3(SCAN_THREADS), 0, s>>>(in, n, block_sums, out, total_host, total_copy);
    return 0;
  }
  scan_spine_kernel<<<dim3(1), dim3(SCAN_THREADS), 0, s>>>(block_sums, blocks, out + n, total_host, total_copy);
  scan_downsweep_kernel<<<dim3((unsigned)blocks), dim3(SCAN_THREADS), 0, s>>>(in, n, block_sums, out);
  return 0;
}

constexpr int RS_THREADS = 256;
constexpr int RS_WAVES = RS_THREADS / 64;
constexpr int RS_ROUNDS = 16;
constexpr int RS_WAVE_ITEMS = RS_ROUNDS * 64;
constexpr int RS_TILE = RS_THREADS * RS_ROUNDS;
constexpr int RS_RADIX = 256;

template <typename KeyT>
__device__ __forceinline__ unsigned key_digit(KeyT k, int shift, unsigned mask) {
  return (unsigned)(k >> shift) & mask;
}

template <typename KeyT> struct PlainPairs {
  const KeyT* keys;
  const int32_t* vals;
  __device__ __forceinline__ KeyT key(int64_t i) const { return keys[i]; }
  __device__ __forceinline__ int32_t val(int64_t i) const { return vals[i]; }
};
template <typename T> struct DepthPairs {
  const T* depth;
  int depth16;
  double near_plane, far_plane;
  int cull;
  __device__ __forceinline__ uint32_t key(int64_t i) const {
    const T d = depth[i];
    if (cull && !(d > T(0))) return CULLED_DEPTH_KEY;
    return depth_sort_key(d, depth16, near_plane, far_plane);
  }
  __device__ __forceinline__ int32_t val(int64_t i) const { return (int32_t)i; }
};

template <typename KeyT, typename Source, bool VARY = false>
__device__ __forceinline__ void upsweep_block(const Source src, int64_t n, int shift, unsigned mask,
                                              int32_t* __restrict__ hist, int64_t num_blocks,
                                              uint32_t* __restrict__ blk_or = nullptr, uint32_t* __restrict__ blk_and = nullptr) {
  constexpr int RS_COPIES = 4;
  __shared__ unsigned cnt[RS_WAVES][RS_COPIES][RS_RADIX];
  __shared__ unsigned s_or, s_and;
  for (int i = threadIdx.x; i < RS_WAVES * RS_COPIES * RS_RADIX; i += RS_THREADS) (&cnt[0][0][0])[i] = 0;
  if (VARY && threadIdx.x == 0) { s_or = 0u; s_and = ~0u; }
  __syncthreads();
  const int wave = threadIdx.x >> 6, lane = lane_id();
  unsigned* mine = cnt[wave][lane & (RS_COPIES - 1)];
  const int64_t base = (int64_t)blockIdx.x * RS_TILE + (int64_t)wave * RS_WAVE_ITEMS + lane;
  unsigned v_or = 0u, v_and = ~0u;
  if ((int64_t)(blockIdx.x + 1) * RS_TILE <= n) {
    KeyT k[RS_ROUNDS];
#pragma unroll
    for (int j = 0; j < RS_ROUNDS; ++j) k[j] = src.key(base + j * 64);
#pragma unroll
    for (int j = 0; j < RS_ROUNDS; ++j) {
      atomicAdd(&mine[key_digit(k[j], shift, mask)], 1u);
      if (VARY && (uint32_t)k[j] != 0xffffffffu) { v_or |= (uint32_t)k[j]; v_and &= (uint32_t)k[j]; }
    }
  } else {
#pragma unroll 4
    for (int j = 0; j < RS_ROUNDS; ++j) {
      const int64_t i = base + j * 64;
      if (i < n) {
        const KeyT key = src.key(i);
        atomicAdd(&mine[key_digit(key, shift, mask)], 1u);
        if (VARY && (uint32_t)key != 0xffffffffu) { v_or |= (uint32_t)key; v_and &= (uint32_t)key; }
      }
    }
  }
  if (VARY) {
#pragma unroll
    for (int off = 32; off >= 1; off >>= 1) { v_or |= __shfl_xor(v_or, off); v_and &= __shfl_xor(v_and, off); }
    if (lane == 0) { atomicOr(&s_or, v_or); atomicAnd(&s_and, v_and); }
  }
  __syncthreads();
  for (int d = threadIdx.x; d < RS_RADIX; d += RS_THREADS) {
    unsigned t = 0;
#pragma unroll
    for (int w = 0; w < RS_WAVES; ++w)
#pragma unroll
      for (int c = 0; c < RS_COPIES; ++c) t += cnt[w][c][d];
    hist[(int64_t)d * num_blocks + blockIdx.x] = (int32_t)t;
  }
  if (VARY && threadIdx.x == 0) { blk_or[blockIdx.x] = s_or; blk_and[blockIdx.x] = s_and; }
}

template <typename KeyT, typename Source>
__global__ void __launch_bounds__(RS_THREADS)
radix_upsweep_kernel(const Source src, int64_t n, const int32_t* __restrict__ n_dev, int shift, unsigned mask,
                     int32_t* __restrict__ hist, int64_t num_blocks) {
  if (n_dev) n = *n_dev;
  upsweep_block<KeyT, Source>(src, n, shift, mask, hist, num_blocks);
}

__device__ __forceinline__ void row_scan_body(int32_t* __restrict__ hist, int64_t num_blocks, int32_t* __restrict__ digit_totals) {
  __shared__ int lds[4];
  int32_t* row = hist + (int64_t)blockIdx.x * num_blocks;
  int carry = 0;
  for (int64_t base = 0; base < num_blocks; base += SCAN_TILE) {
    const int64_t mine = base + (int64_t)threadIdx.x * SCAN_ITEMS;
    int vals[SCAN_ITEMS];
    load_items(row, mine, num_blocks, vals);
    int s = 0;
#pragma unroll
    for (int k = 0; k < SCAN_ITEMS; ++k) s += vals[k];
    int total;
    int prefix = carry + block_exclusive_scan(s, lds, &total);
#pragma unroll
    for (int k = 0; k < SCAN_ITEMS; ++k) {
      const int v = vals[k];
      vals[k] = prefix;
      prefix += v;
    }
    store_items(row, mine, num_blocks, vals);
    carry += total;
  }
  if (threadIdx.x == 0) digit_totals[blockIdx.x] = carry;
}

__global__ void __launch_bounds__(SCAN_THREADS)
radix_row_scan_kernel(int32_t* __restrict__ hist, int64_t num_blocks, int32_t* __restrict__ digit_totals) {
  row_scan_body(hist, num_blocks, digit_totals);
}

template <typename KeyT> struct DownsweepShared {
  unsigned cnt[RS_WAVES][RS_RADIX];
  int scan[4];
  unsigned digit_shift[RS_RADIX];
  KeyT keys[RS_TILE];
  int32_t vals[RS_TILE];
};

template <typename KeyT, bool FULL, typename Source>
__device__ __forceinline__ void downsweep_block(DownsweepShared<KeyT>& sh, const Source src, KeyT* __restrict__ keys_out,
                                                int32_t* __restrict__ vals_out, int64_t n, int shift, unsigned mask,
                                                const int32_t* __restrict__ hist_scanned,
                                                const int32_t* __restrict__ digit_totals, int64_t num_blocks) {
  for (int i = threadIdx.x; i < RS_WAVES * RS_RADIX; i += RS_THREADS) (&sh.cnt[0][0])[i] = 0;
  __syncthreads();

  const int wave = threadIdx.x >> 6, lane = lane_id();
  const int64_t base = (int64_t)blockIdx.x * RS_TILE + (int64_t)wave * RS_WAVE_ITEMS + lane;
  const unsigned long long lanes_below = (1ull << lane) - 1ull;

  KeyT k[RS_ROUNDS];
  int32_t v[RS_ROUNDS];
  unsigned rank[RS_ROUNDS];

#pragma unroll
  for (int j = 0; j < RS_ROUNDS; ++j) {
    const int64_t i = base + j * 64;
    const bool valid = FULL || i < n;
    k[j] = valid ? src.key(i) : (KeyT)0;
    v[j] = valid ? src.val(i) : 0;
  }

#pragma unroll
  for (int j = 0; j < RS_ROUNDS; ++j) {
    const int64_t i = base + j * 64;
    const bool valid = FULL || i < n;
    const unsigned d = key_digit(k[j], shift, mask);
    const unsigned long long valid_lanes = FULL ? ~0ull : __ballot(valid);
    unsigned peers_lo = (unsigned)valid_lanes, peers_hi = (unsigned)(valid_lanes >> 32);
#pragma unroll
    for (int b = 0; b < 8; ++b) {
      const int m = __builtin_amdgcn_sbfe((int)d, b, 1);
      const unsigned long long bal = __ballot(m != 0);
      peers_lo &= ~((unsigned)bal ^ (unsigned)m);
      peers_hi &= ~((unsigned)(bal >> 32) ^ (unsigned)m);
    }
    const unsigned long long peers = ((unsigned long long)peers_hi << 32) | peers_lo;
    const unsigned below = (unsigned)__popcll(peers & lanes_below);
    unsigned prev = 0;
    if (valid) {
      prev = sh.cnt[wave][d];
    }
    __builtin_amdgcn_wave_barrier();
    if (valid && below == 0) sh.cnt[wave][d] = prev + (unsigned)__popcll(peers);
    __builtin_amdgcn_wave_barrier();
    rank[j] = prev + below;
  }
  __syncthreads();

  {
    const int d = threadIdx.x;
    unsigned total = 0;
#pragma unroll
    for (int w = 0; w < RS_WAVES; ++w) total += sh.cnt[w][d];
    int block_total;
    const unsigned local = (unsigned)block_exclusive_scan((int)total, sh.scan, &block_total);
    unsigned run = local;
#pragma unroll
    for (int w = 0; w < RS_WAVES; ++w) {
      const unsigned c = sh.cnt[w][d];
      sh.cnt[w][d] = run;
      run += c;
    }
    int all_items;
    const unsigned digit_base = (unsigned)block_exclusive_scan(digit_totals[d], sh.scan, &all_items);
    sh.digit_shift[d] = digit_base + (unsigned)hist_scanned[(int64_t)d * num_blocks + blockIdx.x] - local;
  }
  __syncthreads();

#pragma unroll
  for (int j = 0; j < RS_ROUNDS; ++j) {
    const int64_t i = base + j * 64;
    if (FULL || i < n) {
      const unsigned d = key_digit(k[j], shift, mask);
      const unsigned lp = sh.cnt[wave][d] + rank[j];
      sh.keys[lp] = k[j];
      sh.vals[lp] = v[j];
    }
  }
  __syncthreads();
  const int64_t block_base = (int64_t)blockIdx.x * RS_TILE;
  const int block_items = FULL ? RS_TILE : (int)(n - block_base);
#pragma unroll
  for (int j = 0; j < RS_ROUNDS; ++j) {
    const int idx = (int)threadIdx.x + j * RS_THREADS;
    if (FULL || idx < block_items) {
      const KeyT key = sh.keys[idx];
      const unsigned d = key_digit(key, shift, mask);
      const int64_t pos = (int64_t)(unsigned)(sh.digit_shift[d] + (unsigned)idx);
      keys_out[pos] = key;
      vals_out[pos] = sh.vals[idx];
    }
  }
}

template <typename KeyT, typename Source>
__global__ void __launch_bounds__(RS_THREADS)
radix_downsweep_kernel(const Source src,
                       KeyT* __restrict__ keys_out, int32_t* __restrict__ vals_out, int64_t n,
                       const int32_t* __restrict__ n_dev, int shift,
                       unsigned mask, const int32_t* __restrict__ hist_scanned,
                       const int32_t* __restrict__ digit_totals, int64_t num_blocks) {
  __shared__ DownsweepShared<KeyT> sh;
  if (n_dev) {
    n = *n_dev;
    if ((int64_t)blockIdx.x * RS_TILE >= n) return;
  }
  if ((int64_t)(blockIdx.x + 1) * RS_TILE <= n)
    downsweep_block<KeyT, true>(sh, src, keys_out, vals_out, n, shift, mask, hist_scanned, digit_totals, num_blocks);
  else
    downsweep_block<KeyT, false>(sh, src, keys_out, vals_out, n, shift, mask, hist_scanned, digit_totals, num_blocks);
}

template <typename KeyT>
__global__ void __launch_bounds__(256)
copy_pairs_kernel(const KeyT* __restrict__ ki, const int32_t* __restrict__ vi, KeyT* __restrict__ ko,
                  int32_t* __restrict__ vo, int64_t n) {
  const int64_t i = (int64_t)blockIdx.x * blockDim.x + threadIdx.x;
  if (i < n) { ko[i] = ki[i]; vo[i] = vi[i]; }
}

struct SortTmp {
  size_t hist_off, scan_off, keys_off, vals_off, keys2_off, vals2_off, vary_off, total;
};

static SortTmp sort_tmp_layout(int64_t n, int key_bytes, bool adaptive = false) {
  const int64_t blocks = div_up(n > 0 ? n : 1, RS_TILE);
  SortTmp t;
  size_t off = 0;
  t.hist_off = off; off += align_up((size_t)(RS_RADIX * blocks + 1) * sizeof(int32_t), 256);
  t.scan_off = off; off += align_up((size_t)RS_RADIX * sizeof(int32_t), 256);
  t.keys_off = off; off += align_up((size_t)n * key_bytes, 256);
  t.vals_off = off; off += align_up((size_t)n * sizeof(int32_t), 256);
  t.keys2_off = t.vals2_off = t.vary_off = off;
  if (adaptive) {
    t.keys2_off = off; off += align_up((size_t)n * key_bytes, 256);
    t.vals2_off = off; off += align_up((size_t)n * sizeof(int32_t), 256);
    t.vary_off = off; off += align_up((size_t)(64 + 2 * blocks) * sizeof(uint32_t), 256);
  }
  t.total = off;
  return t;
}

template <typename KeyT, typename First>
static int radix_sort_passes(const First first, KeyT* keys_out, int32_t* vals_out, int64_t n, int begin_bit, int end_bit,
                             char* tmp, hipStream_t s, const int32_t* n_dev = nullptr) {
  const int64_t blocks = div_up(n, RS_TILE);
  const SortTmp lay = sort_tmp_layout(n, sizeof(KeyT));
  int32_t* hist = (int32_t*)(tmp + lay.hist_off);
  int32_t* digit_totals = (int32_t*)(tmp + lay.scan_off);
  KeyT* keys_alt = (KeyT*)(tmp + lay.keys_off);
  int32_t* vals_alt = (int32_t*)(tmp + lay.vals_off);
  const int passes = (end_bit - begin_bit + 7) / 8;
  const dim3 grid((unsigned)blocks), block(RS_THREADS);
  PlainPairs<KeyT> src{nullptr, nullptr};
  const int total_bits = end_bit - begin_bit, base_bits = total_bits / passes, wide = total_bits % passes;
  int shift = begin_bit;
  for (int p = 0; p < passes; shift += base_bits + (p < wide ? 1 : 0), ++p) {
    const int bits = base_bits + (p < wide ? 1 : 0);
    const unsigned mask = (1u << bits) - 1u;
    const bool to_out = ((passes - 1 - p) % 2) == 0;
    KeyT* dst_k = to_out ? keys_out : keys_alt;
    int32_t* dst_v = to_out ? vals_out : vals_alt;
    if (p == 0) radix_upsweep_kernel<KeyT, First><<<grid, block, 0, s>>>(first, n, n_dev, shift, mask, hist, blocks);
    else radix_upsweep_kernel<KeyT, PlainPairs<KeyT>><<<grid, block, 0, s>>>(src, n, n_dev, shift, mask, hist, blocks);
    radix_row_scan_kernel<<<dim3(RS_RADIX), dim3(SCAN_THREADS), 0, s>>>(hist, blocks, digit_totals);
    if (p == 0) radix_downsweep_kernel<KeyT, First><<<grid, block, 0, s>>>(first, dst_k, dst_v, n, n_dev, shift, mask, hist, digit_totals, blocks);
    else radix_downsweep_kernel<KeyT, PlainPairs<KeyT>><<<grid, block, 0, s>>>(src, dst_k, dst_v, n, n_dev, shift, mask, hist, digit_totals, blocks);
    src = PlainPairs<KeyT>{dst_k, dst_v};
  }
  return 0;
}

struct AdaptiveBufs {
  uint32_t *k_alt[2], *k_out;
  int32_t *v_alt[2], *v_out;
  uint32_t* vary;
};

__device__ __forceinline__ void adaptive_route(uint32_t vary, int p, int passes, bool& active, int& k, bool& last) {
  unsigned m = 1u;
  for (int q = 1; q < passes; ++q)
    if ((vary >> (8 * q)) & 0xffu) m |= 1u << q;
  active = ((m >> p) & 1u) != 0u;
  k = __popc(m & ((1u << p) - 1u));
  last = (m >> (p + 1)) == 0u;
}

template <typename First>
__global__ void __launch_bounds__(RS_THREADS)
depth_upsweep_first_kernel(const First first, AdaptiveBufs b, int64_t n, int32_t* __restrict__ hist, int64_t num_blocks) {
  upsweep_block<uint32_t, First, true>(first, n, 0, 0xffu, hist, num_blocks, b.vary + 64, b.vary + 64 + num_blocks);
}

__global__ void __launch_bounds__(RS_THREADS)
depth_upsweep_kernel(AdaptiveBufs b, int p, int passes, int64_t n, int32_t* __restrict__ hist, int64_t num_blocks) {
  bool active, last; int k;
  adaptive_route(b.vary[0], p, passes, active, k, last);
  if (!active) return;
  upsweep_block<uint32_t, PlainPairs<uint32_t>>(PlainPairs<uint32_t>{b.k_alt[(k - 1) & 1], b.v_alt[(k - 1) & 1]}, n, 8 * p, 0xffu, hist, num_blocks);
}

__global__ void __launch_bounds__(SCAN_THREADS)
depth_row_scan_kernel(int32_t* __restrict__ hist, int64_t num_blocks, int32_t* __restrict__ digit_totals, AdaptiveBufs b,
                      int p, int passes) {
  if (p > 0) {
    bool active, last; int k;
    adaptive_route(b.vary[0], p, passes, active, k, last);
    if (!active) return;
  }
  row_scan_body(hist, num_blocks, digit_totals);
  if (p == 0 && blockIdx.x == 0) {
    __shared__ unsigned s_or, s_and;
    if (threadIdx.x == 0) { s_or = 0u; s_and = ~0u; }
    __syncthreads();
    unsigned v_or = 0u, v_and = ~0u;
    for (int64_t i = threadIdx.x; i < num_blocks; i += blockDim.x) { v_or |= b.vary[64 + i]; v_and &= b.vary[64 + num_blocks + i]; }
    atomicOr(&s_or, v_or); atomicAnd(&s_and, v_and);
    __syncthreads();
    if (threadIdx.x == 0) b.vary[0] = s_or >= s_and && s_or != 0u ? (s_or ^ s_and) : 0u;
  }
}

template <typename First>
__global__ void __launch_bounds__(RS_THREADS)
depth_downsweep_first_kernel(const First first, AdaptiveBufs b, int passes, int64_t n,
                             const int32_t* __restrict__ hist_scanned, const int32_t* __restrict__ digit_totals, int64_t num_blocks) {
  __shared__ DownsweepShared<uint32_t> sh;
  bool active, last; int k;
  adaptive_route(b.vary[0], 0, passes, active, k, last);
  uint32_t* ko = last ? b.k_out : b.k_alt[0];
  int32_t* vo = last ? b.v_out : b.v_alt[0];
  if ((int64_t)(blockIdx.x + 1) * RS_TILE <= n) downsweep_block<uint32_t, true>(sh, first, ko, vo, n, 0, 0xffu, hist_scanned, digit_totals, num_blocks);
  else downsweep_block<uint32_t, false>(sh, first, ko, vo, n, 0, 0xffu, hist_scanned, digit_totals, num_blocks);
}

__global__ void __launch_bounds__(RS_THREADS)
depth_downsweep_kernel(AdaptiveBufs b, int p, int passes, int64_t n, const int32_t* __restrict__ hist_scanned,
                       const int32_t* __restrict__ digit_totals, int64_t num_blocks) {
  __shared__ DownsweepShared<uint32_t> sh;
  bool active, last; int k;
  adaptive_route(b.vary[0], p, passes, active, k, last);
  if (!active) return;
  uint32_t* ko = last ? b.k_out : b.k_alt[k & 1];
  int32_t* vo = last ? b.v_out : b.v_alt[k & 1];
  const PlainPairs<uint32_t> src{b.k_alt[(k - 1) & 1], b.v_alt[(k - 1) & 1]};
  if ((int64_t)(blockIdx.x + 1) * RS_TILE <= n) downsweep_block<uint32_t, true>(sh, src, ko, vo, n, 8 * p, 0xffu, hist_scanned, digit_totals, num_blocks);
  else downsweep_block<uint32_t, false>(sh, src, ko, vo, n, 8 * p, 0xffu, hist_scanned, digit_totals, num_blocks);
}

template <typename First>
static int radix_sort_depth_adaptive(const First first, uint32_t* keys_out, int32_t* vals_out, int64_t n, int end_bit,
                                     char* tmp, hipStream_t s) {
  const int64_t blocks = div_up(n, RS_TILE);
  const SortTmp lay = sort_tmp_layout(n, 4, true);
  int32_t* hist = (int32_t*)(tmp + lay.hist_off);
  int32_t* digit_totals = (int32_t*)(tmp + lay.scan_off);
  AdaptiveBufs b;
  b.k_alt[0] = (uint32_t*)(tmp + lay.keys_off); b.v_alt[0] = (int32_t*)(tmp + lay.vals_off);
  b.k_alt[1] = (uint32_t*)(tmp + lay.keys2_off); b.v_alt[1] = (int32_t*)(tmp + lay.vals2_off);
  b.k_out = keys_out; b.v_out = vals_out;
  b.vary = (uint32_t*)(tmp + lay.vary_off);
  const int passes = (end_bit + 7) / 8;
  const dim3 grid((unsigned)blocks), block(RS_THREADS);
  for (int p = 0; p < passes; ++p) {
    if (p == 0) depth_upsweep_first_kernel<First><<<grid, block, 0, s>>>(first, b, n, hist, blocks);
    else depth_upsweep_kernel<<<grid, block, 0, s>>>(b, p, passes, n, hist, blocks);
    depth_row_scan_kernel<<<dim3(RS_RADIX), dim3(SCAN_THREADS), 0, s>>>(hist, blocks, digit_totals, b, p, passes);
    if (p == 0) depth_downsweep_first_kernel<First><<<grid, block, 0, s>>>(first, b, passes, n, hist, digit_totals, blocks);
    else depth_downsweep_kernel<<<grid, block, 0, s>>>(b, p, passes, n, hist, digit_totals, blocks);
  }
  return 0;
}

template <typename KeyT>
static int radix_sort_pairs_impl(const KeyT* keys_in, const int32_t* vals_in, KeyT* keys_out,
                                 int32_t* vals_out, int64_t n, int begin_bit, int end_bit, char* tmp,
                                 hipStream_t s) {
  if ((end_bit - begin_bit + 7) / 8 == 0) {
    copy_pairs_kernel<KeyT><<<dim3((unsigned)div_up(n, 256)), dim3(256), 0, s>>>(keys_in, vals_in, keys_out, vals_out, n);
    return 0;
  }
  return radix_sort_passes<KeyT>(PlainPairs<KeyT>{keys_in, vals_in}, keys_out, vals_out, n, begin_bit, end_bit, tmp, s);
}

__global__ void __launch_bounds__(256)
segmented_rank_sort_kernel(const int32_t* __restrict__ keys_in, const int32_t* __restrict__ vals_in,
                           int32_t* __restrict__ keys_out, int32_t* __restrict__ vals_out,
                           const int64_t* __restrict__ starts, const int64_t* __restrict__ ends) {
  const int64_t b = starts[blockIdx.x], e = ends[blockIdx.x];
  for (int64_t i = b + threadIdx.x; i < e; i += blockDim.x) {
    const int32_t k = keys_in[i];
    int64_t r = 0;
    for (int64_t j = b; j < e; ++j) {
      const int32_t kj = keys_in[j];
      r += (kj < k) || (kj == k && j < i);
    }
    keys_out[b + r] = k;
    vals_out[b + r] = vals_in[i];
  }
}

template <typename KeyT>
__global__ void __launch_bounds__(256)
find_ranges_kernel(const KeyT* __restrict__ keys, int64_t k, const int32_t* __restrict__ k_dev, int shift,
                   int64_t num_tiles, int32_t* __restrict__ ranges) {
  const int64_t i = (int64_t)blockIdx.x * blockDim.x + threadIdx.x;
  if (k_dev) k = *k_dev;
  if (i >= k) return;
  const bool whole = shift >= (int)(8 * sizeof(KeyT));
  const int64_t tile = whole ? 0 : (int64_t)(keys[i] >> shift);
  const int64_t next = (i + 1 < k) ? (whole ? 0 : (int64_t)(keys[i + 1] >> shift)) : -1;
  if (i == 0 && tile < num_tiles) ranges[tile * 2 + 0] = 0;
  if (tile != next) {
    if (tile < num_tiles) ranges[tile * 2 + 1] = (int32_t)(i + 1);
    if (next >= 0 && next < num_tiles) ranges[next * 2 + 0] = (int32_t)(i + 1);
  }
}

__global__ void __launch_bounds__(256)
find_ranges4_kernel(const uint32_t* __restrict__ keys, int64_t capacity, const int32_t* __restrict__ k_dev,
                    int64_t num_tiles, int32_t* __restrict__ ranges) {
  const int64_t i0 = ((int64_t)blockIdx.x * blockDim.x + threadIdx.x) * 4;
  const int64_t k = k_dev ? (int64_t)*k_dev : capacity;
  if (i0 >= k) return;
  uint32_t t[5];
  if (i0 + 4 < k) {
    const uint4 v = *reinterpret_cast<const uint4*>(keys + i0);
    t[0] = v.x; t[1] = v.y; t[2] = v.z; t[3] = v.w; t[4] = keys[i0 + 4];
  } else {
#pragma unroll
    for (int j = 0; j < 5; ++j) t[j] = i0 + j < k ? keys[i0 + j] : 0xffffffffu;
  }
  if (i0 == 0 && (int64_t)t[0] < num_tiles) ranges[(int64_t)t[0] * 2 + 0] = 0;
#pragma unroll
  for (int j = 0; j < 4; ++j) {
    const int64_t i = i0 + j;
    if (i >= k) break;
    const int64_t tile = t[j], next = (i + 1 < k) ? (int64_t)t[j + 1] : -1;
    if (tile != next) {
      if (tile < num_tiles) ranges[tile * 2 + 1] = (int32_t)(i + 1);
      if (next >= 0 && next < num_tiles) ranges[next * 2 + 0] = (int32_t)(i + 1);
    }
  }
}

__global__ void __launch_bounds__(256)
find_ranges2_u64_kernel(const uint64_t* __restrict__ keys, int64_t capacity, const int32_t* __restrict__ k_dev,
                        int64_t num_tiles, int32_t* __restrict__ ranges) {
  const int64_t i0 = ((int64_t)blockIdx.x * blockDim.x + threadIdx.x) * 2;
  const int64_t k = k_dev ? (int64_t)*k_dev : capacity;
  uint32_t t0 = 0xffffffffu, t1 = 0xffffffffu;
  if (i0 + 1 < k) {
    const uint4 a = *reinterpret_cast<const uint4*>(keys + i0);
    t0 = a.y; t1 = a.w;
  } else if (i0 < k) {
    t0 = (uint32_t)(keys[i0] >> 32);
  }
  uint32_t t2 = (uint32_t)__shfl_down((int)t0, 1);
  if ((threadIdx.x & 63) == 63) t2 = i0 + 2 < k ? (uint32_t)(keys[i0 + 2] >> 32) : 0xffffffffu;
  if (i0 >= k) return;
  if (i0 == 0 && (int64_t)t0 < num_tiles) ranges[(int64_t)t0 * 2 + 0] = 0;
  const uint32_t t[3] = {t0, t1, t2};
#pragma unroll
  for (int j = 0; j < 2; ++j) {
    const int64_t i = i0 + j;
    if (i >= k) break;
    const int64_t tile = t[j], next = (i + 1 < k) ? (int64_t)t[j + 1] : -1;
    if (tile != next) {
      if (tile < num_tiles) ranges[tile * 2 + 1] = (int32_t)(i + 1);
      if (next >= 0 && next < num_tiles) ranges[next * 2 + 0] = (int32_t)(i + 1);
    }
  }
}

size_t scan_tmp_size(int64_t n) { return scan_tmp_bytes(n); }
size_t sort_tmp_size(int64_t n, int key_bytes, bool adaptive) { return sort_tmp_layout(n, key_bytes, adaptive).total; }

void exclusive_scan_launch(const int32_t* in, int64_t n, int32_t* out, int32_t* total_host, void* tmp, hipStream_t s,
                           int32_t* total_copy) {
  exclusive_scan_i32(in, n, out, total_host, tmp, s, total_copy);
}

void depth_argsort_launch(const void* depth, int64_t n, int depth16, double ndc_near, double ndc_far, int dtype,
                          int cull, uint32_t* out_sorted_keys, int32_t* out_order, char* tmp, hipStream_t s) {
  const int end_bit = depth16 ? 16 : 32;
  if (dtype == MS_F32)
    radix_sort_depth_adaptive(DepthPairs<float>{(const float*)depth, depth16, ndc_near, ndc_far, cull}, out_sorted_keys, out_order, n, end_bit, tmp, s);
  else
    radix_sort_depth_adaptive(DepthPairs<double>{(const double*)depth, depth16, ndc_near, ndc_far, cull}, out_sorted_keys, out_order, n, end_bit, tmp, s);
}

void sort_pairs_u32_dev_launch(const uint32_t* keys_in, const int32_t* vals_in, uint32_t* keys_out, int32_t* vals_out,
                               int64_t capacity, const int32_t* n_dev, int end_bit, char* tmp, hipStream_t s) {
  radix_sort_passes<uint32_t>(PlainPairs<uint32_t>{keys_in, vals_in}, keys_out, vals_out, capacity, 0, end_bit, tmp, s, n_dev);
}

int find_ranges_dev_launch(const uint32_t* sorted_keys, int64_t capacity, const int32_t* k_dev, int64_t num_tiles,
                           int32_t* out_ranges, hipStream_t s, bool zeroed) {
  if (num_tiles > 0 && !zeroed) MS_CHECK_HIP(hipMemsetAsync(out_ranges, 0, (size_t)num_tiles * 2 * sizeof(int32_t), s));
  if (capacity > 0)
    find_ranges4_kernel<<<dim3((unsigned)div_up(capacity, 1024)), dim3(256), 0, s>>>(sorted_keys, capacity, k_dev, num_tiles, out_ranges);
  return 0;
}

void sort_pairs_u64_dev_launch(const uint64_t* keys_in, const int32_t* vals_in, uint64_t* keys_out, int32_t* vals_out,
                               int64_t capacity, const int32_t* n_dev, int begin_bit, int end_bit, char* tmp, hipStream_t s) {
  radix_sort_passes<uint64_t>(PlainPairs<uint64_t>{keys_in, vals_in}, keys_out, vals_out, capacity, begin_bit, end_bit, tmp, s, n_dev);
}

int find_ranges_u64_dev_launch(const uint64_t* sorted_keys, int64_t capacity, const int32_t* k_dev, int64_t num_tiles,
                               int32_t* out_ranges, hipStream_t s) {
  if (capacity > 0)
    find_ranges2_u64_kernel<<<dim3((unsigned)div_up(capacity, 512)), dim3(256), 0, s>>>(sorted_keys, capacity, k_dev, num_tiles, out_ranges);
  return 0;
}

}

using namespace ms;

extern "C" int ms_exclusive_scan_i32(const int32_t* in, int64_t n, int32_t* out, int32_t* total_host,
                                     void* tmp, size_t* tmp_bytes, void* stream) {
  MS_CHECK_ARG(n >= 0, "n < 0");
  MS_CHECK_ARG(tmp_bytes != nullptr, "tmp_bytes is null");
  const size_t need = scan_tmp_bytes(n);
  if (tmp == nullptr) { *tmp_bytes = need; return 0; }
  if (*tmp_bytes < need) { set_error("ms_exclusive_scan_i32: tmp too small (%zu < %zu)", *tmp_bytes, need); return MS_ERR_TMP_TOO_SMALL; }
  MS_CHECK_ARG(out != nullptr, "out is null");
  MS_CHECK_ARG(n == 0 || in != nullptr, "in is null");
  if (n == 0) {
    MS_CHECK_HIP(hipMemsetAsync(out, 0, sizeof(int32_t), (hipStream_t)stream));
    if (total_host) *total_host = 0;
    return 0;
  }
  exclusive_scan_i32(in, n, out, total_host, tmp, (hipStream_t)stream);
  MS_CHECK_LAUNCH();
  return 0;
}

extern "C" int ms_radix_sort_pairs(const void* keys_in, const int32_t* values_in, void* keys_out,
                                   int32_t* values_out, int64_t n, int key_bytes, int begin_bit,
                                   int end_bit, void* tmp, size_t* tmp_bytes, void* stream) {
  MS_CHECK_ARG(n >= 0, "n < 0");
  MS_CHECK_ARG(key_bytes == 4 || key_bytes == 8, "key_bytes must be 4 or 8");
  MS_CHECK_ARG(begin_bit >= 0 && end_bit >= begin_bit && end_bit <= key_bytes * 8, "bad bit range");
  MS_CHECK_ARG(tmp_bytes != nullptr, "tmp_bytes is null");
  const size_t need = sort_tmp_layout(n, key_bytes).total;
  if (tmp == nullptr) { *tmp_bytes = need; return 0; }
  if (*tmp_bytes < need) { set_error("ms_radix_sort_pairs: tmp too small (%zu < %zu)", *tmp_bytes, need); return MS_ERR_TMP_TOO_SMALL; }
  if (n == 0) return 0;
  MS_CHECK_ARG(keys_in && values_in && keys_out && values_out, "null pointer");
  if (key_bytes == 4)
    radix_sort_pairs_impl<uint32_t>((const uint32_t*)keys_in, values_in, (uint32_t*)keys_out, values_out, n, begin_bit, end_bit, (char*)tmp, (hipStream_t)stream);
  else
    radix_sort_pairs_impl<uint64_t>((const uint64_t*)keys_in, values_in, (uint64_t*)keys_out, values_out, n, begin_bit, end_bit, (char*)tmp, (hipStream_t)stream);
  MS_CHECK_LAUNCH();
  return 0;
}

extern "C" int ms_depth_argsort(const void* depth, int64_t v, int depth16, double ndc_near, double ndc_far,
                               int dtype, uint32_t* out_sorted_keys, int32_t* out_order, void* tmp,
                               size_t* tmp_bytes, void* stream) {
  MS_CHECK_ARG(v >= 0, "v < 0");
  MS_CHECK_ARG(dtype == MS_F32 || dtype == MS_F64, "dtype must be MS_F32 or MS_F64");
  MS_CHECK_ARG(tmp_bytes != nullptr, "tmp_bytes is null");
  const size_t need = sort_tmp_layout(v, 4).total;
  if (tmp == nullptr) { *tmp_bytes = need; return 0; }
  if (*tmp_bytes < need) { set_error("ms_depth_argsort: tmp too small (%zu < %zu)", *tmp_bytes, need); return MS_ERR_TMP_TOO_SMALL; }
  if (v == 0) return 0;
  MS_CHECK_ARG(depth && out_sorted_keys && out_order, "null pointer");
  const int end_bit = depth16 ? 16 : 32;
  if (dtype == MS_F32)
    radix_sort_passes<uint32_t>(DepthPairs<float>{(const float*)depth, depth16, ndc_near, ndc_far, 0}, out_sorted_keys, out_order, v, 0, end_bit, (char*)tmp, (hipStream_t)stream);
  else
    radix_sort_passes<uint32_t>(DepthPairs<double>{(const double*)depth, depth16, ndc_near, ndc_far, 0}, out_sorted_keys, out_order, v, 0, end_bit, (char*)tmp, (hipStream_t)stream);
  MS_CHECK_LAUNCH();
  return 0;
}

extern "C" int ms_segmented_sort_pairs(const int32_t* keys_in, const int32_t* values_in, int32_t* keys_out,
                                       int32_t* values_out, int64_t n, const int64_t* start_offsets,
                                       const int64_t* end_offsets, int64_t num_segments, void* stream) {
  MS_CHECK_ARG(n >= 0 && num_segments >= 0, "negative size");
  if (n == 0) return 0;
  MS_CHECK_ARG(keys_in && values_in && keys_out && values_out, "null pointer");
  MS_CHECK_ARG(num_segments == 0 || (start_offsets && end_offsets), "null segment offsets");
  copy_pairs_kernel<int32_t><<<dim3((unsigned)div_up(n, 256)), dim3(256), 0, (hipStream_t)stream>>>(
      keys_in, values_in, keys_out, values_out, n);
  if (num_segments > 0)
    segmented_rank_sort_kernel<<<dim3((unsigned)num_segments), dim3(256), 0, (hipStream_t)stream>>>(
        keys_in, values_in, keys_out, values_out, start_offsets, end_offsets);
  MS_CHECK_LAUNCH();
  return 0;
}

extern "C" int ms_find_ranges(const void* sorted_keys, int64_t k, int key_bytes, int tile_shift,
                              int64_t num_tiles, int32_t* out_ranges, void* stream) {
  MS_CHECK_ARG(k >= 0 && num_tiles >= 0, "negative size");
  MS_CHECK_ARG(key_bytes == 4 || key_bytes == 8, "key_bytes must be 4 or 8");
  MS_CHECK_ARG(tile_shift >= 0 && tile_shift <= key_bytes * 8, "tile_shift outside the key");
  MS_CHECK_ARG(out_ranges != nullptr || num_tiles == 0, "out_ranges is null");
  if (num_tiles > 0)
    MS_CHECK_HIP(hipMemsetAsync(out_ranges, 0, (size_t)num_tiles * 2 * sizeof(int32_t), (hipStream_t)stream));
  if (k == 0) return 0;
  MS_CHECK_ARG(sorted_keys != nullptr, "sorted_keys is null");
  const dim3 block(256), grid((unsigned)div_up(k, 256));
  if (key_bytes == 4)
    find_ranges_kernel<uint32_t><<<grid, block, 0, (hipStream_t)stream>>>((const uint32_t*)sorted_keys, k, nullptr, tile_shift, num_tiles, out_ranges);
  else
    find_ranges_kernel<uint64_t><<<grid, block, 0, (hipStream_t)stream>>>((const uint64_t*)sorted_keys, k, nullptr, tile_shift, num_tiles, out_ranges);
  MS_CHECK_LAUNCH();
  return 0;
}
```

### taichi_splatting_amd/csrc/tile_sort.hip

```cpp
#include "common.h"
#include "frame_internal.h"

namespace ms {

constexpr int TS_THREADS = 256;
constexpr int TS_WAVES = TS_THREADS / 64;
constexpr int TS_COST_LIMIT = 64;
constexpr int SMALL_R = 4, MID_R = 10, LONG_R = 20;

constexpr int TS_PER_WAVE = 256;
struct TsShared {
  uint32_t red[2 * TS_WAVES];
  uint32_t hist[256];
};
constexpr uint64_t TS_DECLINED = ~0ull;
constexpr int TS_REPORT_ABOVE = 16384;

__device__ __forceinline__ uint32_t ts_wave_min(uint32_t v) {
#pragma unroll
  for (int o = 32; o > 0; o >>= 1) { const uint32_t w = (uint32_t)__shfl_xor((int)v, o); v = w < v ? w : v; }
  return v;
}
__device__ __forceinline__ uint32_t ts_wave_max(uint32_t v) {
#pragma unroll
  for (int o = 32; o > 0; o >>= 1) { const uint32_t w = (uint32_t)__shfl_xor((int)v, o); v = w > v ? w : v; }
  return v;
}
__device__ __forceinline__ uint32_t ts_wave_or(uint32_t v) {
#pragma unroll
  for (int o = 32; o > 0; o >>= 1) v |= (uint32_t)__shfl_xor((int)v, o);
  return v;
}
__device__ __forceinline__ uint32_t ts_wave_and(uint32_t v) {
#pragma unroll
  for (int o = 32; o > 0; o >>= 1) v &= (uint32_t)__shfl_xor((int)v, o);
  return v;
}
__device__ __forceinline__ uint32_t ts_wave_sum(uint32_t v) {
#pragma unroll
  for (int o = 32; o > 0; o >>= 1) v += (uint32_t)__shfl_xor((int)v, o);
  return v;
}
__device__ __forceinline__ uint32_t ts_wave_scan(uint32_t v) {
  const int lane = threadIdx.x & 63;
#pragma unroll
  for (int o = 1; o < 64; o <<= 1) { const uint32_t w = (uint32_t)__shfl_up((int)v, o); if (lane >= o) v += w; }
  return v;
}

__device__ __forceinline__ uint32_t ts_block_exclusive(uint32_t v, uint32_t* red, uint32_t* total) {
  const int lane = threadIdx.x & 63, wave = threadIdx.x >> 6;
  const uint32_t inc = ts_wave_scan(v);
  __syncthreads();
  if (lane == 63) red[wave] = inc;
  __syncthreads();
  uint32_t before = 0, all = 0;
#pragma unroll
  for (int w = 0; w < TS_WAVES; ++w) { const uint32_t c = red[w]; if (w < wave) before += c; all += c; }
  *total = all;
  return before + inc - v;
}

__device__ void tile_radix_sort_global(uint64_t* srt, int32_t* o2p, uint64_t* alt,
                                       int64_t b, int n, TsShared& sh, uint32_t* wcnt) {
  const int t = threadIdx.x, lane = t & 63, wave = t >> 6;
  uint32_t kor = 0u, kand = 0xffffffffu;
  for (int i = t; i < n; i += TS_THREADS) {
    const uint32_t k = (uint32_t)srt[b + i];
    srt[b + i] = ((uint64_t)k << 32) | (uint32_t)o2p[b + i];
    kor |= k;
    kand &= k;
  }
  kor = ts_wave_or(kor);
  kand = ts_wave_and(kand);
  __syncthreads();
  if (lane == 0) { sh.red[wave] = kor; sh.red[TS_WAVES + wave] = kand; }
  __syncthreads();
  kor = 0u; kand = 0xffffffffu;
#pragma unroll
  for (int w = 0; w < TS_WAVES; ++w) { kor |= sh.red[w]; kand &= sh.red[TS_WAVES + w]; }
  const uint32_t vary = kor ^ kand;

  uint64_t* src = srt;
  uint64_t* dst = alt;
  for (int pass = 0; pass < 4; ++pass) {
    if (((vary >> (8 * pass)) & 0xffu) == 0u) continue;
    const int shift = 32 + 8 * pass;
    __syncthreads();
    sh.hist[t] = 0u;
    __syncthreads();
    for (int i = t; i < n; i += TS_THREADS) atomicAdd(&sh.hist[(uint32_t)(src[b + i] >> shift) & 0xffu], 1u);
    __syncthreads();
    uint32_t total;
    const uint32_t base = ts_block_exclusive(sh.hist[t], sh.red, &total);
    __syncthreads();
    sh.hist[t] = base;
    __syncthreads();
    for (int c = 0; c < n; c += TS_WAVES * TS_PER_WAVE) {
      for (int j = t; j < TS_WAVES * 256; j += TS_THREADS) wcnt[j] = 0u;
      __syncthreads();
      uint64_t p[TS_PER_WAVE / 64];
      uint32_t rank[TS_PER_WAVE / 64];
#pragma unroll
      for (int g = 0; g < TS_PER_WAVE / 64; ++g) {
        const int i = c + wave * TS_PER_WAVE + g * 64 + lane;
        const bool valid = i < n;
        p[g] = valid ? src[b + i] : 0ull;
        const uint32_t d = (uint32_t)(p[g] >> shift) & 0xffu;
        uint64_t peers = __ballot(valid);
#pragma unroll
        for (int bit = 0; bit < 8; ++bit) {
          const bool one = (d >> bit) & 1u;
          const uint64_t bal = __ballot(one);
          peers &= one ? bal : ~bal;
        }
        const uint64_t below = peers & ((1ull << lane) - 1ull);
        uint32_t prev = 0u;
        if (valid) prev = wcnt[wave * 256 + d];
        __builtin_amdgcn_wave_barrier();
        if (valid && below == 0ull) wcnt[wave * 256 + d] = prev + (uint32_t)__popcll(peers);
        __builtin_amdgcn_wave_barrier();
        rank[g] = prev + (uint32_t)__popcll(below);
      }
      __syncthreads();
      {
        uint32_t at = sh.hist[t];
#pragma unroll
        for (int w = 0; w < TS_WAVES; ++w) { const uint32_t cw = wcnt[w * 256 + t]; wcnt[w * 256 + t] = at; at += cw; }
        sh.hist[t] = at;
      }
      __syncthreads();
#pragma unroll
      for (int g = 0; g < TS_PER_WAVE / 64; ++g) {
        const int i = c + wave * TS_PER_WAVE + g * 64 + lane;
        if (i < n) dst[b + wcnt[wave * 256 + ((uint32_t)(p[g] >> shift) & 0xffu)] + rank[g]] = p[g];
      }
      __syncthreads();
    }
    uint64_t* const swap = src; src = dst; dst = swap;
  }
  __syncthreads();
  if (src == srt && vary == 0u) return;
  for (int i = t; i < n; i += TS_THREADS) o2p[b + i] = (int32_t)(uint32_t)src[b + i];
}

struct BucketMap {
  uint32_t kmin, top;
  float base, scale;
  int by_value;
  __device__ __forceinline__ uint32_t operator()(uint32_t k) const {
    const float x = by_value ? __uint_as_float(k) - base : (float)(k - kmin);
    const uint32_t bkt = (uint32_t)(x * scale);
    return bkt < top ? bkt : top;
  }
};

template <int R>
__device__ __forceinline__ bool tile_bucket_sort(uint64_t* __restrict__ srt, int32_t* __restrict__ o2p,
                                                 int64_t b, int n, uint64_t* pairs, uint32_t* cnt, TsShared& sh) {
  const int t = threadIdx.x, lane = t & 63, wave = t >> 6;
  uint32_t key[R], id[R];
  uint32_t kmin = 0xffffffffu, kmax = 0u;
#pragma unroll
  for (int r = 0; r < R; ++r) {
    const int i = t + TS_THREADS * r;
    key[r] = 0u; id[r] = 0u;
    if (i < n) {
      key[r] = (uint32_t)srt[b + i];
      id[r] = (uint32_t)o2p[b + i];
      kmin = key[r] < kmin ? key[r] : kmin;
      kmax = key[r] > kmax ? key[r] : kmax;
    }
  }
  kmin = ts_wave_min(kmin);
  kmax = ts_wave_max(kmax);
  if (lane == 0) { sh.red[wave] = kmin; sh.red[TS_WAVES + wave] = kmax; }
  __syncthreads();
#pragma unroll
  for (int w = 0; w < TS_WAVES; ++w) {
    kmin = sh.red[w] < kmin ? sh.red[w] : kmin;
    kmax = sh.red[TS_WAVES + w] > kmax ? sh.red[TS_WAVES + w] : kmax;
  }
  if (kmin == kmax) return true;

  const uint32_t nb = (uint32_t)n;
  BucketMap bucket;
  bucket.kmin = kmin;
  bucket.top = nb - 1u;
  bucket.by_value = kmin >= 0x00800000u && kmax < 0x7f800000u;
  bucket.base = __uint_as_float(kmin);
  bucket.scale = (float)nb / (__uint_as_float(kmax) - bucket.base);
  if (bucket.by_value && !(bucket.scale < 3.0e38f)) bucket.by_value = 0;
  if (!bucket.by_value) bucket.scale = (float)nb / (float)(kmax - kmin);

  for (uint32_t j = t; j < nb; j += TS_THREADS) cnt[j] = 0u;
  __syncthreads();
  uint32_t bkt[R], slot[R];
#pragma unroll
  for (int r = 0; r < R; ++r) {
    bkt[r] = 0u; slot[r] = 0u;
    if (t + TS_THREADS * r < n) {
      bkt[r] = bucket(key[r]);
      slot[r] = atomicAdd(&cnt[bkt[r]], 1u);
    }
  }
  __syncthreads();

  const uint32_t per = (nb + TS_THREADS - 1u) / TS_THREADS;
  const uint32_t j0 = t * per, j1 = j0 + per < nb ? j0 + per : nb;
  uint32_t mine = 0u, squares = 0u;
  for (uint32_t j = j0; j < j1; ++j) { const uint32_t c = cnt[j]; mine += c; squares += c * c; }
  const uint32_t inc = ts_wave_scan(mine);
  squares = ts_wave_sum(squares);
  if (lane == 63) { sh.red[wave] = inc; sh.red[TS_WAVES + wave] = squares; }
  __syncthreads();
  uint32_t run = inc - mine, cost = 0u;
#pragma unroll
  for (int w = 0; w < TS_WAVES; ++w) {
    if (w < wave) run += sh.red[w];
    cost += sh.red[TS_WAVES + w];
  }
  if (cost > (uint32_t)TS_COST_LIMIT * nb) return false;
  for (uint32_t j = j0; j < j1; ++j) { const uint32_t c = cnt[j]; cnt[j] = run; run += c; }
  __syncthreads();

#pragma unroll
  for (int r = 0; r < R; ++r)
    if (t + TS_THREADS * r < n) pairs[cnt[bkt[r]] + slot[r]] = ((uint64_t)key[r] << 32) | id[r];
  __syncthreads();

#pragma unroll
  for (int r = 0; r < R; ++r) {
    const int i = t + TS_THREADS * r;
    if (i < n) {
      const uint64_t p = pairs[i];
      const uint32_t g = bucket((uint32_t)(p >> 32));
      const uint32_t first = cnt[g], last = g + 1u < nb ? cnt[g + 1u] : nb;
      uint32_t rank = first;
      for (uint32_t m = first; m < last; ++m) rank += pairs[m] < p ? 1u : 0u;
      o2p[b + rank] = (int32_t)(uint32_t)p;
    }
  }
  return true;
}

template <int R>
__global__ void __launch_bounds__(TS_THREADS, R <= 4 ? 8 : 1)
tile_depth_sort_kernel(const int32_t* __restrict__ ranges, uint64_t* __restrict__ srt, int32_t* __restrict__ o2p,
                       uint64_t* __restrict__ alt, int lo, int hi, int32_t* __restrict__ run_stats) {
  constexpr int CAP = TS_THREADS * R;
  __shared__ uint64_t pairs[CAP];
  __shared__ uint32_t cnt[CAP];
  __shared__ TsShared sh;
  const int64_t tile = blockIdx.x;
  const int64_t b = ranges[2 * tile];
  const int n = ranges[2 * tile + 1] - (int32_t)b;
  if (n <= lo || n > hi) return;
  const bool sorted = tile_bucket_sort<R>(srt, o2p, b, n, pairs, cnt, sh);
  if (threadIdx.x == 0) {
    alt[b] = sorted ? 0ull : TS_DECLINED;
    if (!sorted && run_stats) atomicOr(run_stats + 2, 1);
  }
}

template <int R>
__global__ void __launch_bounds__(TS_THREADS)
tile_depth_sort_long_kernel(const int32_t* __restrict__ ranges, int64_t num_tiles, uint64_t* __restrict__ srt,
                            int32_t* __restrict__ o2p, uint64_t* __restrict__ alt, int lo, int32_t* __restrict__ run_stats,
                            int32_t* __restrict__ run_host) {
  constexpr int CAP = TS_THREADS * R;
  static_assert(CAP >= TS_WAVES * 256, "the bucket counters double as the bounded path's digit counters");
  __shared__ uint64_t pairs[CAP];
  __shared__ uint32_t cnt[CAP];
  __shared__ TsShared sh;
  __shared__ int32_t todo[TS_THREADS];
  __shared__ int32_t todo_count;
  const int64_t share = (num_tiles + gridDim.x - 1) / gridDim.x;
  const int64_t first = (int64_t)blockIdx.x * share;
  const int64_t last = first + share < num_tiles ? first + share : num_tiles;
  const bool any_declined = run_stats ? run_stats[2] != 0 : true;
  for (int64_t base = first; base < last; base += TS_THREADS) {
    __syncthreads();
    if (threadIdx.x == 0) todo_count = 0;
    __syncthreads();
    const int64_t mine = base + threadIdx.x;
    if (mine < last) {
      const int64_t mb = ranges[2 * mine];
      const int mn = ranges[2 * mine + 1] - (int32_t)mb;
      if (mn > lo) {
        todo[atomicAdd(&todo_count, 1)] = (int32_t)(mine - base);
        if (mn > TS_REPORT_ABOVE && run_host) *run_host = mn;
      }
      else if (any_declined && mn > 1 && alt[mb] == TS_DECLINED) todo[atomicAdd(&todo_count, 1)] = (int32_t)(mine - base) | (1 << 30);
    }
    __syncthreads();
    const int count = todo_count;
    for (int j = 0; j < count; ++j) {
      const int entry = todo[j];
      const int64_t tile = base + (entry & 0xffff);
      const int64_t b = ranges[2 * tile];
      const int n = ranges[2 * tile + 1] - (int32_t)b;
      bool sorted = false;
      if (n <= CAP && !(entry >> 30)) sorted = tile_bucket_sort<R>(srt, o2p, b, n, pairs, cnt, sh);
      if (!sorted) {
        __syncthreads();
        tile_radix_sort_global(srt, o2p, alt, b, n, sh, cnt);
      }
      __syncthreads();
    }
  }
}

void tile_depth_sort_launch(const int32_t* tile_ranges, int64_t num_tiles, uint64_t* sorted_keys, int32_t* overlap_to_point,
                            uint64_t* scratch, hipStream_t s, int32_t* run_stats, int32_t* run_host) {
  if (num_tiles <= 0) return;
  const dim3 per_tile((unsigned)num_tiles), block(TS_THREADS);
  tile_depth_sort_kernel<SMALL_R><<<per_tile, block, 0, s>>>(tile_ranges, sorted_keys, overlap_to_point, scratch, 1,
                                                            TS_THREADS * SMALL_R, run_stats);
  tile_depth_sort_kernel<MID_R><<<per_tile, block, 0, s>>>(tile_ranges, sorted_keys, overlap_to_point, scratch,
                                                          TS_THREADS * SMALL_R, TS_THREADS * MID_R, run_stats);
  const int64_t few = 2 * 256;
  tile_depth_sort_long_kernel<LONG_R><<<dim3((unsigned)(num_tiles < few ? num_tiles : few)), block, 0, s>>>(
      tile_ranges, num_tiles, sorted_keys, overlap_to_point, scratch, TS_THREADS * MID_R, run_stats, run_host);
}

}

using namespace ms;

extern "C" int ms_tile_depth_sort(const int32_t* tile_ranges, int64_t num_tiles, uint64_t* sorted_keys,
                                  int32_t* overlap_to_point, uint64_t* scratch, void* stream) {
  MS_CHECK_ARG(num_tiles >= 0 && num_tiles < (1ll << 31), "num_tiles out of range");
  if (num_tiles == 0) return 0;
  MS_CHECK_ARG(tile_ranges && sorted_keys && overlap_to_point && scratch, "null pointer");
  tile_depth_sort_launch(tile_ranges, num_tiles, sorted_keys, overlap_to_point, scratch, (hipStream_t)stream);
  MS_CHECK_LAUNCH();
  return 0;
}
```

Before: 2038 Msplats/s.

## Sort compact tile ids with packed depth|point payload in direct mapper

The direct tile mapper now emits 16- or 32-bit tile ids plus a 64-bit payload packing depth key and point index, instead of 64-bit tile|depth keys with separate int32 values. The global radix sort runs only over the tile-id bits, and the per-tile depth sort reads depth and id from the payload. This cuts key bytes per sort pass and may reduce the number of passes. It adds a new sort/range path and a standalone ms_map_tiles_direct entry point. The per-tile sort must now always write o2p, which adds writes for single-element and constant-key tiles.

```diff
diff --git a/include/mi355_splat.h b/include/mi355_splat.h
--- a/include/mi355_splat.h
+++ b/include/mi355_splat.h
@@ -111,6 +111,12 @@
 
 int ms_tile_depth_sort(const int32_t* tile_ranges, int64_t num_tiles, uint64_t* sorted_keys,
                        int32_t* overlap_to_point, uint64_t* scratch, void* stream);
+
+int ms_map_tiles_direct(const float* points7, const void* depth, int depth_dtype, const int32_t* cum, int64_t v,
+                        int image_w, int image_h, int tile_size, float alpha_threshold, int tile_row_begin,
+                        int tile_row_end, int depth16, double ndc_near, double ndc_far, int64_t k_capacity,
+                        int32_t* out_overlap_to_point, int32_t* out_tile_ranges, int32_t* out_counters,
+                        void* scratch, size_t* scratch_bytes, void* stream);
 
 int ms_raster_fwd(const void* points7, const void* features, const int32_t* tile_ranges,
                   const int32_t* overlap_to_point, int image_w, int image_h, int f,
diff --git a/taichi_splatting_amd/_lib.py b/taichi_splatting_amd/_lib.py
--- a/taichi_splatting_amd/_lib.py
+++ b/taichi_splatting_amd/_lib.py
@@ -150,6 +150,8 @@
   'ms_segmented_sort_pairs': (c_int, [c_void_p] * 4 + [c_int64, c_void_p, c_void_p, c_int64, c_void_p]),
   'ms_find_ranges': (c_int, [c_void_p, c_int64, c_int, c_int, c_int64, c_void_p, c_void_p]),
   'ms_tile_depth_sort': (c_int, [c_void_p, c_int64, c_void_p, c_void_p, c_void_p, c_void_p]),
+  'ms_map_tiles_direct': (c_int, [c_void_p, c_void_p, c_int, c_void_p, c_int64, c_int, c_int, c_int, c_float, c_int, c_int, c_int,
+                                  c_double, c_double, c_int64, c_void_p, c_void_p, c_void_p, c_void_p, POINTER(c_size_t), c_void_p]),
   'ms_fractional_step': (c_int, [c_int, c_int] + [c_void_p] * 7 + [c_int64, c_int, c_float, c_float, c_float, c_float, c_int, c_void_p]),
   'ms_morton_codes64': (c_int, [c_void_p, c_int64, c_void_p, c_void_p, ctypes.c_uint32, c_void_p, c_void_p]),
   'ms_knn_points': (c_int, [c_void_p, c_void_p, c_int64, c_int, c_void_p, c_void_p, c_void_p, c_void_p, POINTER(c_size_t), c_void_p]),
diff --git a/taichi_splatting_amd/csrc/frame.hip b/taichi_splatting_amd/csrc/frame.hip
--- a/taichi_splatting_amd/csrc/frame.hip
+++ b/taichi_splatting_amd/csrc/frame.hip
@@ -124,8 +124,38 @@
   L->keys = scratch_k.take(k * 8);
   L->values = scratch_k.take(k * 4);
   L->keys_sorted = scratch_k.take(k * 8);
-  L->tmp_k = scratch_k.take(sort_tmp_size(d->k_capacity, 8));
+  L->tmp_k = scratch_k.take(sort_tmp_size(d->k_capacity, 4));
   L->scratch_k_bytes = scratch_k.off;
+}
+
+struct DirectMapBufs {
+  void *ids_out, *ids_alt;
+  uint64_t *payload_out, *payload_alt;
+  char* hist_tmp;
+};
+struct DirectMapGrid {
+  int w_pad, h_pad, tile_size, tiles_wide, num_tiles, tile_bits, row_begin, row_end;
+  float alpha_threshold;
+};
+
+static int direct_map_enqueue(const float* points_f32, const void* depth, int dtype, const int32_t* cum, int64_t n,
+                              const DirectMapGrid& g, int depth16, double ndc_near, double ndc_far, int64_t capacity,
+                              int32_t* counters, const DirectMapBufs& b, int32_t* ranges, int32_t* o2p,
+                              int32_t* longest_run_host, hipStream_t s) {
+  const int id_bytes = tile_id_bytes(g.num_tiles);
+  const bool in_out = tile_sort_starts_in_out(g.tile_bits);
+  tile_emit_ids_launch(points_f32, depth, dtype, cum, n, g.w_pad, g.h_pad, g.tile_size, g.alpha_threshold, g.row_begin,
+                       g.row_end, depth16, ndc_near, ndc_far, counters + 1, id_bytes, in_out ? b.ids_out : b.ids_alt,
+                       in_out ? b.payload_out : b.payload_alt, s);
+  sort_ids_payload_dev_launch(id_bytes, b.ids_out, b.payload_out, b.ids_alt, b.payload_alt, capacity, counters + 1,
+                              g.tile_bits, b.hist_tmp, s);
+  const int rc = find_ranges_ids_dev_launch(id_bytes, b.ids_out, capacity, counters + 1, g.num_tiles, ranges, s);
+  if (rc != 0) return rc;
+  const int64_t first_tile = (int64_t)g.row_begin * g.tiles_wide;
+  const int64_t strip_tiles = (int64_t)(g.row_end > g.row_begin ? g.row_end - g.row_begin : 0) * g.tiles_wide;
+  tile_payload_sort_launch(ranges + 2 * first_tile, strip_tiles, b.payload_out, o2p, b.payload_alt, s, counters + 3,
+                           longest_run_host);
+  return 0;
 }
 
 template <typename T>
@@ -344,20 +374,16 @@
       sort_pairs_u32_dev_launch(keys, values, keys_sorted, o2p, d.k_capacity, counters + 1, g.tile_bits, sk + L.tmp_k, s);
       MS_TRY(find_ranges_dev_launch(keys_sorted, d.k_capacity, counters + 1, g.num_tiles, ranges, s, true));
     } else {
-      uint64_t* keys = (uint64_t*)(sk + L.keys);
-      uint64_t* keys_sorted = (uint64_t*)(sk + L.keys_sorted);
       const void* depth = d.projected_input ? in->depth : (const void*)(kn + L.depth);
       const float* points_f32 = d.dtype == MS_F64 ? (const float*)(sn + L.points7_f32)
                                                   : (const float*)(d.projected_input ? in->points7 : (const void*)(kn + L.points7));
-      tile_emit_direct_launch(points_f32, depth, d.dtype, (const int32_t*)(sn + L.cum), d.n, g.w_pad, g.h_pad,
-                              d.raster.tile_size, (float)d.raster.alpha_threshold, g.row_begin, g.row_end, d.depth16,
-                              d.near_plane > 0.0 ? d.near_plane : 0.0, d.far_plane, counters + 1, keys, values, s);
-      sort_pairs_u64_dev_launch(keys, values, keys_sorted, o2p, d.k_capacity, counters + 1, 32, 32 + g.tile_bits,
-                                sk + L.tmp_k, s);
-      MS_TRY(find_ranges_u64_dev_launch(keys_sorted, d.k_capacity, counters + 1, g.num_tiles, ranges, s));
-      const int64_t first_tile = (int64_t)g.row_begin * g.tiles_wide;
-      const int64_t strip_tiles = (int64_t)(g.row_end > g.row_begin ? g.row_end - g.row_begin : 0) * g.tiles_wide;
-      tile_depth_sort_launch(ranges + 2 * first_tile, strip_tiles, keys_sorted, o2p, keys, s, counters + 3, in->longest_run_host);
+      const DirectMapBufs bufs{values, sk + L.tmp_k + sort_hist_size(d.k_capacity), (uint64_t*)(sk + L.keys_sorted),
+                               (uint64_t*)(sk + L.keys), sk + L.tmp_k};
+      const DirectMapGrid grid{g.w_pad, g.h_pad, d.raster.tile_size, g.tiles_wide, g.num_tiles, g.tile_bits, g.row_begin,
+                               g.row_end, (float)d.raster.alpha_threshold};
+      MS_TRY(direct_map_enqueue(points_f32, depth, d.dtype, (const int32_t*)(sn + L.cum), d.n, grid, d.depth16,
+                                d.near_plane > 0.0 ? d.near_plane : 0.0, d.far_plane, d.k_capacity, counters, bufs, ranges,
+                                o2p, in->longest_run_host, s));
     }
   }
   MS_CHECK_LAUNCH();
@@ -372,6 +398,58 @@
   return raster_fwd_launch(points7, colours, frame_uses_rows(desc) ? (const float*)(kn + L.splat_rows) : nullptr, ranges, o2p,
                            d.image_w, d.image_h, d.f, &d.raster, out_image, out_alpha, out_visibility, g.row_begin, g.row_end,
                            d.dtype, stream, cut ? &split : nullptr, in->longest_run_host);
+}
+
+extern "C" int ms_map_tiles_direct(const float* points7, const void* depth, int depth_dtype, const int32_t* cum, int64_t v,
+                                   int image_w, int image_h, int tile_size, float alpha_threshold, int tile_row_begin,
+                                   int tile_row_end, int depth16, double ndc_near, double ndc_far, int64_t k_capacity,
+                                   int32_t* out_overlap_to_point, int32_t* out_tile_ranges, int32_t* out_counters,
+                                   void* scratch, size_t* scratch_bytes, void* stream) {
+  MS_CHECK_ARG(v >= 0 && v < (1ll << 31) && k_capacity >= 0 && k_capacity < (1ll << 31), "sizes are int32 indexes (< 2^31)");
+  MS_CHECK_ARG(depth_dtype == MS_F32 || depth_dtype == MS_F64, "depth_dtype must be MS_F32 or MS_F64");
+  MS_CHECK_ARG(tile_size > 0 && image_w > 0 && image_h > 0, "bad image/tile size");
+  MS_CHECK_ARG(image_w % tile_size == 0 && image_h % tile_size == 0, "image size must be padded to the tile size");
+  MS_CHECK_ARG(scratch_bytes != nullptr, "scratch_bytes is null");
+  DirectMapGrid g;
+  g.w_pad = image_w; g.h_pad = image_h; g.tile_size = tile_size;
+  g.tiles_wide = image_w / tile_size;
+  const int tiles_high = image_h / tile_size;
+  MS_CHECK_ARG((int64_t)g.tiles_wide * tiles_high < (1ll << 31), "too many tiles");
+  g.num_tiles = g.tiles_wide * tiles_high;
+  g.tile_bits = 1;
+  while ((1ll << g.tile_bits) < (long long)g.num_tiles) ++g.tile_bits;
+  g.row_begin = tile_row_begin < 0 ? 0 : tile_row_begin;
+  g.row_end = tile_row_end > tiles_high ? tiles_high : tile_row_end;
+  g.alpha_threshold = alpha_threshold;
+  MS_CHECK_ARG(!depth16 || g.num_tiles <= 65536, "use_depth16 keys hold a 16 bit tile id: too many tiles");
+
+  Carve c;
+  const size_t k = (size_t)k_capacity;
+  const size_t payload_out = c.take(k * 8), payload_alt = c.take(k * 8), ids_out = c.take(k * 4), ids_alt = c.take(k * 4);
+  const size_t hist = c.take(sort_hist_size(k_capacity));
+  if (scratch == nullptr) { *scratch_bytes = c.off; return 0; }
+  if (*scratch_bytes < c.off) { set_error("ms_map_tiles_direct: scratch too small (%zu < %zu)", *scratch_bytes, c.off); return MS_ERR_TMP_TOO_SMALL; }
+  MS_CHECK_ARG(out_tile_ranges && out_counters, "null pointer");
+  MS_CHECK_ARG((reinterpret_cast<uintptr_t>(scratch) & 15) == 0, "scratch must be 16-byte aligned");
+
+  hipStream_t s = (hipStream_t)stream;
+  MS_CHECK_HIP(hipMemsetAsync(out_counters, 0, 8 * sizeof(int32_t), s));
+  if (v > 0) {
+    MS_CHECK_ARG(cum != nullptr, "cum is null");
+    MS_CHECK_HIP(hipMemcpyAsync(out_counters, cum + v, sizeof(int32_t), hipMemcpyDeviceToDevice, s));
+  }
+  const int64_t words = (int64_t)g.num_tiles * 2;
+  frame_prepare_kernel<float><<<dim3((unsigned)div_up(words, 256)), dim3(256), 0, s>>>(out_counters, (int32_t)k_capacity, nullptr,
+                                                                                      nullptr, out_tile_ranges, words);
+  if (v > 0 && k_capacity > 0) {
+    MS_CHECK_ARG(points7 && depth && out_overlap_to_point, "null pointer");
+    char* sc = (char*)scratch;
+    const DirectMapBufs bufs{sc + ids_out, sc + ids_alt, (uint64_t*)(sc + payload_out), (uint64_t*)(sc + payload_alt), sc + hist};
+    MS_TRY(direct_map_enqueue(points7, depth, depth_dtype, cum, v, g, depth16, ndc_near > 0.0 ? ndc_near : 0.0, ndc_far,
+                              k_capacity, out_counters, bufs, out_tile_ranges, out_overlap_to_point, nullptr, s));
+  }
+  MS_CHECK_LAUNCH();
+  return 0;
 }
 
 extern "C" int ms_frame_backward(const ms_frame_desc* desc, const ms_frame_inputs* in, void* keep_n, void* keep_k,
diff --git a/taichi_splatting_amd/csrc/frame_internal.h b/taichi_splatting_amd/csrc/frame_internal.h
--- a/taichi_splatting_amd/csrc/frame_internal.h
+++ b/taichi_splatting_amd/csrc/frame_internal.h
@@ -40,9 +40,12 @@
 int find_ranges_dev_launch(const uint32_t* sorted_keys, int64_t capacity, const int32_t* k_dev, int64_t num_tiles,
                            int32_t* out_ranges, hipStream_t s, bool zeroed = false);
 
-void sort_pairs_u64_dev_launch(const uint64_t* keys_in, const int32_t* vals_in, uint64_t* keys_out, int32_t* vals_out,
-                               int64_t capacity, const int32_t* n_dev, int begin_bit, int end_bit, char* tmp, hipStream_t s);
-int find_ranges_u64_dev_launch(const uint64_t* sorted_keys, int64_t capacity, const int32_t* k_dev, int64_t num_tiles,
+inline int tile_id_bytes(int64_t num_tiles) { return num_tiles <= 65536 ? 2 : 4; }
+inline bool tile_sort_starts_in_out(int tile_bits) { return ((tile_bits + 7) / 8) % 2 == 0; }
+size_t sort_hist_size(int64_t n);
+void sort_ids_payload_dev_launch(int id_bytes, void* ids_out, uint64_t* payload_out, void* ids_alt, uint64_t* payload_alt,
+                                 int64_t capacity, const int32_t* n_dev, int tile_bits, char* hist_tmp, hipStream_t s);
+int find_ranges_ids_dev_launch(int id_bytes, const void* sorted_ids, int64_t capacity, const int32_t* k_dev, int64_t num_tiles,
                                int32_t* out_ranges, hipStream_t s);
 
 void tile_count_launch(const float* points7, const int32_t* order, const uint32_t* cull_keys, int64_t v, int image_w,
@@ -61,8 +64,16 @@
                              double ndc_near, double ndc_far, const int32_t* k_limit_dev, uint64_t* out_keys,
                              int32_t* out_values, hipStream_t s);
 
+void tile_emit_ids_launch(const float* points7, const void* depth, int dtype, const int32_t* cum, int64_t v, int image_w,
+                          int image_h, int tile_size, float alpha_threshold, int row_begin, int row_end, int depth16,
+                          double ndc_near, double ndc_far, const int32_t* k_limit_dev, int id_bytes, void* out_tiles,
+                          uint64_t* out_payload, hipStream_t s);
+
 void tile_depth_sort_launch(const int32_t* tile_ranges, int64_t num_tiles, uint64_t* sorted_keys, int32_t* overlap_to_point,
                             uint64_t* scratch, hipStream_t s, int32_t* run_stats = nullptr, int32_t* run_host = nullptr);
+
+void tile_payload_sort_launch(const int32_t* tile_ranges, int64_t num_tiles, uint64_t* sorted_payload, int32_t* overlap_to_point,
+                              uint64_t* scratch, hipStream_t s, int32_t* run_stats = nullptr, int32_t* run_host = nullptr);
 
 int project_fwd_launch(const void* position, const void* log_scaling, const void* rotation, const void* alpha_logit,
                        const void* T_camera_world, const void* projection, int image_w, int image_h, double near_plane,
diff --git a/taichi_splatting_amd/csrc/mapper.hip b/taichi_splatting_amd/csrc/mapper.hip
--- a/taichi_splatting_amd/csrc/mapper.hip
+++ b/taichi_splatting_amd/csrc/mapper.hip
@@ -197,6 +197,30 @@
   });
 }
 
+template <typename T, typename IdT>
+__global__ void __launch_bounds__(256)
+tile_emit_ids_kernel(const float* __restrict__ points, const T* __restrict__ depth, const int32_t* __restrict__ cum,
+                     int64_t v, int image_w, int image_h, int tile_size, float alpha_threshold, int row_begin,
+                     int row_end, int depth16, double near_plane, double far_plane,
+                     const int32_t* __restrict__ k_limit, IdT* __restrict__ tiles, uint64_t* __restrict__ payload) {
+  const int64_t i = (int64_t)blockIdx.x * blockDim.x + threadIdx.x;
+  if (k_limit && *k_limit == 0) return;
+  const int64_t first = i < v ? (int64_t)cum[i] : 0;
+  const bool valid = i < v && cum[i + 1] != first;
+  float g[7] = {0.f, 0.f, 1.f, 0.f, 1.f, 1.f, 0.f};
+  if (valid) load_point7(points, i, g);
+  const ObbQuery q = obb_grid_query(g, image_w, image_h, tile_size, alpha_threshold);
+  const int tiles_wide = image_w / tile_size;
+  const uint32_t depth_key = valid ? (uint32_t)depth_sort_key(depth[i], depth16, near_plane, far_plane) : 0u;
+  emit_span(q, valid, first, tile_size, row_begin, row_end, [&](int64_t o, int tx, int ty, int from) {
+    uint32_t dk = depth_key;
+    int32_t who = (int32_t)i;
+    if (from >= 0) { dk = (uint32_t)__builtin_amdgcn_readlane((int)depth_key, from); who = __builtin_amdgcn_readlane((int32_t)i, from); }
+    tiles[o] = (IdT)(tx + ty * tiles_wide);
+    payload[o] = ((uint64_t)dk << 32) | (uint32_t)who;
+  });
+}
+
 template <typename T>
 __global__ void __launch_bounds__(256)
 depth_keys_kernel(const T* __restrict__ depth, int64_t v, int depth16, double near_plane, double far_plane,
@@ -250,6 +274,17 @@
                                                           k_limit_dev, out_keys, out_values);
 }
 
+void tile_emit_ids_launch(const float* points7, const void* depth, int dtype, const int32_t* cum, int64_t v, int image_w,
+                          int image_h, int tile_size, float alpha_threshold, int row_begin, int row_end, int depth16,
+                          double ndc_near, double ndc_far, const int32_t* k_limit_dev, int id_bytes, void* out_tiles,
+                          uint64_t* out_payload, hipStream_t s) {
+  const dim3 grid((unsigned)div_up(v, 256)), block(256);
+#define MS_EMIT_IDS(T, IdT) tile_emit_ids_kernel<T, IdT><<<grid, block, 0, s>>>(points7, (const T*)depth, cum, v, image_w, image_h, tile_size, alpha_threshold, row_begin, row_end, depth16, ndc_near, ndc_far, k_limit_dev, (IdT*)out_tiles, out_payload)
+  if (dtype == MS_F64) { if (id_bytes == 2) MS_EMIT_IDS(double, uint16_t); else MS_EMIT_IDS(double, uint32_t); }
+  else { if (id_bytes == 2) MS_EMIT_IDS(float, uint16_t); else MS_EMIT_IDS(float, uint32_t); }
+#undef MS_EMIT_IDS
+}
+
 }
 
 using namespace ms;
diff --git a/taichi_splatting_amd/csrc/scan_sort.hip b/taichi_splatting_amd/csrc/scan_sort.hip
--- a/taichi_splatting_amd/csrc/scan_sort.hip
+++ b/taichi_splatting_amd/csrc/scan_sort.hip
@@ -172,12 +172,24 @@
 }
 
 template <typename KeyT> struct PlainPairs {
+  using value_type = int32_t;
+  static constexpr bool dense_keys = true;
   const KeyT* keys;
   const int32_t* vals;
   __device__ __forceinline__ KeyT key(int64_t i) const { return keys[i]; }
   __device__ __forceinline__ int32_t val(int64_t i) const { return vals[i]; }
 };
+template <typename KeyT> struct WidePairs {
+  using value_type = uint64_t;
+  static constexpr bool dense_keys = true;
+  const KeyT* keys;
+  const uint64_t* vals;
+  __device__ __forceinline__ KeyT key(int64_t i) const { return keys[i]; }
+  __device__ __forceinline__ uint64_t val(int64_t i) const { return vals[i]; }
+};
 template <typename T> struct DepthPairs {
+  using value_type = int32_t;
+  static constexpr bool dense_keys = false;
   const T* depth;
   int depth16;
   double near_plane, far_plane;
@@ -204,7 +216,23 @@
   unsigned* mine = cnt[wave][lane & (RS_COPIES - 1)];
   const int64_t base = (int64_t)blockIdx.x * RS_TILE + (int64_t)wave * RS_WAVE_ITEMS + lane;
   unsigned v_or = 0u, v_and = ~0u;
-  if ((int64_t)(blockIdx.x + 1) * RS_TILE <= n) {
+  bool counted = false;
+  if constexpr (sizeof(KeyT) == 2 && Source::dense_keys && !VARY) {
+    if ((int64_t)(blockIdx.x + 1) * RS_TILE <= n && (reinterpret_cast<uintptr_t>(src.keys) & 15) == 0) {
+      static_assert(RS_ROUNDS == 16, "two uint4 per thread");
+      const uint4* p = reinterpret_cast<const uint4*>(src.keys + (int64_t)blockIdx.x * RS_TILE + (int64_t)threadIdx.x * RS_ROUNDS);
+      const uint4 a = p[0], b = p[1];
+      const uint32_t w[8] = {a.x, a.y, a.z, a.w, b.x, b.y, b.z, b.w};
+#pragma unroll
+      for (int j = 0; j < 8; ++j) {
+        atomicAdd(&mine[key_digit((KeyT)(w[j] & 0xffffu), shift, mask)], 1u);
+        atomicAdd(&mine[key_digit((KeyT)(w[j] >> 16), shift, mask)], 1u);
+      }
+      counted = true;
+    }
+  }
+  if (counted) {
+  } else if ((int64_t)(blockIdx.x + 1) * RS_TILE <= n) {
     KeyT k[RS_ROUNDS];
 #pragma unroll
     for (int j = 0; j < RS_ROUNDS; ++j) k[j] = src.key(base + j * 64);
@@ -279,17 +307,18 @@
   row_scan_body(hist, num_blocks, digit_totals);
 }
 
-template <typename KeyT> struct DownsweepShared {
+template <typename KeyT, typename ValT> struct DownsweepShared {
   unsigned cnt[RS_WAVES][RS_RADIX];
   int scan[4];
   unsigned digit_shift[RS_RADIX];
+  ValT vals[RS_TILE];
   KeyT keys[RS_TILE];
-  int32_t vals[RS_TILE];
 };
 
 template <typename KeyT, bool FULL, typename Source>
-__device__ __forceinline__ void downsweep_block(DownsweepShared<KeyT>& sh, const Source src, KeyT* __restrict__ keys_out,
-                                                int32_t* __restrict__ vals_out, int64_t n, int shift, unsigned mask,
+__device__ __forceinline__ void downsweep_block(DownsweepShared<KeyT, typename Source::value_type>& sh, const Source src,
+                                                KeyT* __restrict__ keys_out,
+                                                typename Source::value_type* __restrict__ vals_out, int64_t n, int shift, unsigned mask,
                                                 const int32_t* __restrict__ hist_scanned,
                                                 const int32_t* __restrict__ digit_totals, int64_t num_blocks) {
   for (int i = threadIdx.x; i < RS_WAVES * RS_RADIX; i += RS_THREADS) (&sh.cnt[0][0])[i] = 0;
@@ -299,8 +328,9 @@
   const int64_t base = (int64_t)blockIdx.x * RS_TILE + (int64_t)wave * RS_WAVE_ITEMS + lane;
   const unsigned long long lanes_below = (1ull << lane) - 1ull;
 
+  using ValT = typename Source::value_type;
   KeyT k[RS_ROUNDS];
-  int32_t v[RS_ROUNDS];
+  ValT v[RS_ROUNDS];
   unsigned rank[RS_ROUNDS];
 
 #pragma unroll
@@ -308,7 +338,7 @@
     const int64_t i = base + j * 64;
     const bool valid = FULL || i < n;
     k[j] = valid ? src.key(i) : (KeyT)0;
-    v[j] = valid ? src.val(i) : 0;
+    v[j] = valid ? src.val(i) : (ValT)0;
   }
 
 #pragma unroll
@@ -387,11 +417,11 @@
 template <typename KeyT, typename Source>
 __global__ void __launch_bounds__(RS_THREADS)
 radix_downsweep_kernel(const Source src,
-                       KeyT* __restrict__ keys_out, int32_t* __restrict__ vals_out, int64_t n,
+                       KeyT* __restrict__ keys_out, typename Source::value_type* __restrict__ vals_out, int64_t n,
                        const int32_t* __restrict__ n_dev, int shift,
                        unsigned mask, const int32_t* __restrict__ hist_scanned,
                        const int32_t* __restrict__ digit_totals, int64_t num_blocks) {
-  __shared__ DownsweepShared<KeyT> sh;
+  __shared__ DownsweepShared<KeyT, typename Source::value_type> sh;
   if (n_dev) {
     n = *n_dev;
     if ((int64_t)blockIdx.x * RS_TILE >= n) return;
@@ -432,18 +462,17 @@
   return t;
 }
 
-template <typename KeyT, typename First>
-static int radix_sort_passes(const First first, KeyT* keys_out, int32_t* vals_out, int64_t n, int begin_bit, int end_bit,
-                             char* tmp, hipStream_t s, const int32_t* n_dev = nullptr) {
+static int radix_pass_count(int begin_bit, int end_bit) { return (end_bit - begin_bit + 7) / 8; }
+
+template <typename KeyT, typename Plain, typename First>
+static int radix_sort_passes_on(const First first, KeyT* keys_out, typename Plain::value_type* vals_out, KeyT* keys_alt,
+                                typename Plain::value_type* vals_alt, int32_t* hist, int32_t* digit_totals ,
+                                int64_t n, int begin_bit, int end_bit, hipStream_t s, const int32_t* n_dev = nullptr) {
+  using ValT = typename Plain::value_type;
   const int64_t blocks = div_up(n, RS_TILE);
-  const SortTmp lay = sort_tmp_layout(n, sizeof(KeyT));
-  int32_t* hist = (int32_t*)(tmp + lay.hist_off);
-  int32_t* digit_totals = (int32_t*)(tmp + lay.scan_off);
-  KeyT* keys_alt = (KeyT*)(tmp + lay.keys_off);
-  int32_t* vals_alt = (int32_t*)(tmp + lay.vals_off);
-  const int passes = (end_bit - begin_bit + 7) / 8;
+  const int passes = radix_pass_count(begin_bit, end_bit);
   const dim3 grid((unsigned)blocks), block(RS_THREADS);
-  PlainPairs<KeyT> src{nullptr, nullptr};
+  Plain src{nullptr, nullptr};
   const int total_bits = end_bit - begin_bit, base_bits = total_bits / passes, wide = total_bits % passes;
   int shift = begin_bit;
   for (int p = 0; p < passes; shift += base_bits + (p < wide ? 1 : 0), ++p) {
@@ -451,15 +480,24 @@
     const unsigned mask = (1u << bits) - 1u;
     const bool to_out = ((passes - 1 - p) % 2) == 0;
     KeyT* dst_k = to_out ? keys_out : keys_alt;
-    int32_t* dst_v = to_out ? vals_out : vals_alt;
+    ValT* dst_v = to_out ? vals_out : vals_alt;
     if (p == 0) radix_upsweep_kernel<KeyT, First><<<grid, block, 0, s>>>(first, n, n_dev, shift, mask, hist, blocks);
-    else radix_upsweep_kernel<KeyT, PlainPairs<KeyT>><<<grid, block, 0, s>>>(src, n, n_dev, shift, mask, hist, blocks);
+    else radix_upsweep_kernel<KeyT, Plain><<<grid, block, 0, s>>>(src, n, n_dev, shift, mask, hist, blocks);
     radix_row_scan_kernel<<<dim3(RS_RADIX), dim3(SCAN_THREADS), 0, s>>>(hist, blocks, digit_totals);
     if (p == 0) radix_downsweep_kernel<KeyT, First><<<grid, block, 0, s>>>(first, dst_k, dst_v, n, n_dev, shift, mask, hist, digit_totals, blocks);
-    else radix_downsweep_kernel<KeyT, PlainPairs<KeyT>><<<grid, block, 0, s>>>(src, dst_k, dst_v, n, n_dev, shift, mask, hist, digit_totals, blocks);
-    src = PlainPairs<KeyT>{dst_k, dst_v};
-  }
-  return 0;
+    else radix_downsweep_kernel<KeyT, Plain><<<grid, block, 0, s>>>(src, dst_k, dst_v, n, n_dev, shift, mask, hist, digit_totals, blocks);
+    src = Plain{dst_k, dst_v};
+  }
+  return 0;
+}
+
+template <typename KeyT, typename First>
+static int radix_sort_passes(const First first, KeyT* keys_out, int32_t* vals_out, int64_t n, int begin_bit, int end_bit,
+                             char* tmp, hipStream_t s, const int32_t* n_dev = nullptr) {
+  const SortTmp lay = sort_tmp_layout(n, sizeof(KeyT));
+  return radix_sort_passes_on<KeyT, PlainPairs<KeyT>>(first, keys_out, vals_out, (KeyT*)(tmp + lay.keys_off),
+                                                      (int32_t*)(tmp + lay.vals_off), (int32_t*)(tmp + lay.hist_off),
+                                                      (int32_t*)(tmp + lay.scan_off), n, begin_bit, end_bit, s, n_dev);
 }
 
 struct AdaptiveBufs {
@@ -516,7 +554,7 @@
 __global__ void __launch_bounds__(RS_THREADS)
 depth_downsweep_first_kernel(const First first, AdaptiveBufs b, int passes, int64_t n,
                              const int32_t* __restrict__ hist_scanned, const int32_t* __restrict__ digit_totals, int64_t num_blocks) {
-  __shared__ DownsweepShared<uint32_t> sh;
+  __shared__ DownsweepShared<uint32_t, int32_t> sh;
   bool active, last; int k;
   adaptive_route(b.vary[0], 0, passes, active, k, last);
   uint32_t* ko = last ? b.k_out : b.k_alt[0];
@@ -528,7 +566,7 @@
 __global__ void __launch_bounds__(RS_THREADS)
 depth_downsweep_kernel(AdaptiveBufs b, int p, int passes, int64_t n, const int32_t* __restrict__ hist_scanned,
                        const int32_t* __restrict__ digit_totals, int64_t num_blocks) {
-  __shared__ DownsweepShared<uint32_t> sh;
+  __shared__ DownsweepShared<uint32_t, int32_t> sh;
   bool active, last; int k;
   adaptive_route(b.vary[0], p, passes, active, k, last);
   if (!active) return;
@@ -635,25 +673,31 @@
   }
 }
 
+template <typename IdT>
 __global__ void __launch_bounds__(256)
-find_ranges2_u64_kernel(const uint64_t* __restrict__ keys, int64_t capacity, const int32_t* __restrict__ k_dev,
-                        int64_t num_tiles, int32_t* __restrict__ ranges) {
-  const int64_t i0 = ((int64_t)blockIdx.x * blockDim.x + threadIdx.x) * 2;
+find_ranges_ids_kernel(const IdT* __restrict__ ids, int64_t capacity, const int32_t* __restrict__ k_dev,
+                       int64_t num_tiles, int32_t* __restrict__ ranges) {
+  constexpr int PER = 16 / (int)sizeof(IdT);
+  const int64_t i0 = ((int64_t)blockIdx.x * blockDim.x + threadIdx.x) * PER;
   const int64_t k = k_dev ? (int64_t)*k_dev : capacity;
-  uint32_t t0 = 0xffffffffu, t1 = 0xffffffffu;
-  if (i0 + 1 < k) {
-    const uint4 a = *reinterpret_cast<const uint4*>(keys + i0);
-    t0 = a.y; t1 = a.w;
-  } else if (i0 < k) {
-    t0 = (uint32_t)(keys[i0] >> 32);
-  }
-  uint32_t t2 = (uint32_t)__shfl_down((int)t0, 1);
-  if ((threadIdx.x & 63) == 63) t2 = i0 + 2 < k ? (uint32_t)(keys[i0 + 2] >> 32) : 0xffffffffu;
   if (i0 >= k) return;
-  if (i0 == 0 && (int64_t)t0 < num_tiles) ranges[(int64_t)t0 * 2 + 0] = 0;
-  const uint32_t t[3] = {t0, t1, t2};
-#pragma unroll
-  for (int j = 0; j < 2; ++j) {
+  uint32_t t[PER + 1];
+  if (i0 + PER < k && (reinterpret_cast<uintptr_t>(ids) & 15) == 0) {
+    const uint4 v = *reinterpret_cast<const uint4*>(ids + i0);
+    const uint32_t w[4] = {v.x, v.y, v.z, v.w};
+#pragma unroll
+    for (int j = 0; j < PER; ++j) {
+      if constexpr (sizeof(IdT) == 2) t[j] = (w[j >> 1] >> (16 * (j & 1))) & 0xffffu;
+      else t[j] = w[j];
+    }
+    t[PER] = (uint32_t)ids[i0 + PER];
+  } else {
+#pragma unroll
+    for (int j = 0; j <= PER; ++j) t[j] = i0 + j < k ? (uint32_t)ids[i0 + j] : 0u;
+  }
+  if (i0 == 0 && (int64_t)t[0] < num_tiles) ranges[(int64_t)t[0] * 2 + 0] = 0;
+#pragma unroll
+  for (int j = 0; j < PER; ++j) {
     const int64_t i = i0 + j;
     if (i >= k) break;
     const int64_t tile = t[j], next = (i + 1 < k) ? (int64_t)t[j + 1] : -1;
@@ -694,15 +738,31 @@
   return 0;
 }
 
-void sort_pairs_u64_dev_launch(const uint64_t* keys_in, const int32_t* vals_in, uint64_t* keys_out, int32_t* vals_out,
-                               int64_t capacity, const int32_t* n_dev, int begin_bit, int end_bit, char* tmp, hipStream_t s) {
-  radix_sort_passes<uint64_t>(PlainPairs<uint64_t>{keys_in, vals_in}, keys_out, vals_out, capacity, begin_bit, end_bit, tmp, s, n_dev);
-}
-
-int find_ranges_u64_dev_launch(const uint64_t* sorted_keys, int64_t capacity, const int32_t* k_dev, int64_t num_tiles,
+size_t sort_hist_size(int64_t n) { return sort_tmp_layout(n, 0).keys_off; }
+
+template <typename IdT>
+static void sort_ids_payload(IdT* ids_out, uint64_t* payload_out, IdT* ids_alt, uint64_t* payload_alt, int64_t capacity,
+                             const int32_t* n_dev, int tile_bits, char* hist_tmp, hipStream_t s) {
+  const SortTmp lay = sort_tmp_layout(capacity, 0);
+  const bool even = radix_pass_count(0, tile_bits) % 2 == 0;
+  const WidePairs<IdT> first{even ? ids_out : ids_alt, even ? payload_out : payload_alt};
+  radix_sort_passes_on<IdT, WidePairs<IdT>>(first, ids_out, payload_out, ids_alt, payload_alt, (int32_t*)(hist_tmp + lay.hist_off),
+                                            (int32_t*)(hist_tmp + lay.scan_off), capacity, 0, tile_bits, s, n_dev);
+}
+
+void sort_ids_payload_dev_launch(int id_bytes, void* ids_out, uint64_t* payload_out, void* ids_alt, uint64_t* payload_alt,
+                                 int64_t capacity, const int32_t* n_dev, int tile_bits, char* hist_tmp, hipStream_t s) {
+  if (id_bytes == 2) sort_ids_payload<uint16_t>((uint16_t*)ids_out, payload_out, (uint16_t*)ids_alt, payload_alt, capacity, n_dev, tile_bits, hist_tmp, s);
+  else sort_ids_payload<uint32_t>((uint32_t*)ids_out, payload_out, (uint32_t*)ids_alt, payload_alt, capacity, n_dev, tile_bits, hist_tmp, s);
+}
+
+int find_ranges_ids_dev_launch(int id_bytes, const void* sorted_ids, int64_t capacity, const int32_t* k_dev, int64_t num_tiles,
                                int32_t* out_ranges, hipStream_t s) {
-  if (capacity > 0)
-    find_ranges2_u64_kernel<<<dim3((unsigned)div_up(capacity, 512)), dim3(256), 0, s>>>(sorted_keys, capacity, k_dev, num_tiles, out_ranges);
+  if (capacity <= 0) return 0;
+  if (id_bytes == 2)
+    find_ranges_ids_kernel<uint16_t><<<dim3((unsigned)div_up(capacity, 256 * 8)), dim3(256), 0, s>>>((const uint16_t*)sorted_ids, capacity, k_dev, num_tiles, out_ranges);
+  else
+    find_ranges_ids_kernel<uint32_t><<<dim3((unsigned)div_up(capacity, 256 * 4)), dim3(256), 0, s>>>((const uint32_t*)sorted_ids, capacity, k_dev, num_tiles, out_ranges);
   return 0;
 }
 
diff --git a/taichi_splatting_amd/csrc/tile_sort.hip b/taichi_splatting_amd/csrc/tile_sort.hip
--- a/taichi_splatting_amd/csrc/tile_sort.hip
+++ b/taichi_splatting_amd/csrc/tile_sort.hip
@@ -61,13 +61,19 @@
   return before + inc - v;
 }
 
+template <bool PAYLOAD>
 __device__ void tile_radix_sort_global(uint64_t* srt, int32_t* o2p, uint64_t* alt,
                                        int64_t b, int n, TsShared& sh, uint32_t* wcnt) {
   const int t = threadIdx.x, lane = t & 63, wave = t >> 6;
   uint32_t kor = 0u, kand = 0xffffffffu;
   for (int i = t; i < n; i += TS_THREADS) {
-    const uint32_t k = (uint32_t)srt[b + i];
-    srt[b + i] = ((uint64_t)k << 32) | (uint32_t)o2p[b + i];
+    uint32_t k;
+    if constexpr (PAYLOAD) {
+      k = (uint32_t)(srt[b + i] >> 32);
+    } else {
+      k = (uint32_t)srt[b + i];
+      srt[b + i] = ((uint64_t)k << 32) | (uint32_t)o2p[b + i];
+    }
     kor |= k;
     kand &= k;
   }
@@ -140,7 +146,7 @@
     uint64_t* const swap = src; src = dst; dst = swap;
   }
   __syncthreads();
-  if (src == srt && vary == 0u) return;
+  if (!PAYLOAD && src == srt && vary == 0u) return;
   for (int i = t; i < n; i += TS_THREADS) o2p[b + i] = (int32_t)(uint32_t)src[b + i];
 }
 
@@ -155,7 +161,7 @@
   }
 };
 
-template <int R>
+template <int R, bool PAYLOAD>
 __device__ __forceinline__ bool tile_bucket_sort(uint64_t* __restrict__ srt, int32_t* __restrict__ o2p,
                                                  int64_t b, int n, uint64_t* pairs, uint32_t* cnt, TsShared& sh) {
   const int t = threadIdx.x, lane = t & 63, wave = t >> 6;
@@ -166,8 +172,14 @@
     const int i = t + TS_THREADS * r;
     key[r] = 0u; id[r] = 0u;
     if (i < n) {
-      key[r] = (uint32_t)srt[b + i];
-      id[r] = (uint32_t)o2p[b + i];
+      if constexpr (PAYLOAD) {
+        const uint64_t p = srt[b + i];
+        key[r] = (uint32_t)(p >> 32);
+        id[r] = (uint32_t)p;
+      } else {
+        key[r] = (uint32_t)srt[b + i];
+        id[r] = (uint32_t)o2p[b + i];
+      }
       kmin = key[r] < kmin ? key[r] : kmin;
       kmax = key[r] > kmax ? key[r] : kmax;
     }
@@ -181,7 +193,14 @@
     kmin = sh.red[w] < kmin ? sh.red[w] : kmin;
     kmax = sh.red[TS_WAVES + w] > kmax ? sh.red[TS_WAVES + w] : kmax;
   }
-  if (kmin == kmax) return true;
+  if (kmin == kmax) {
+    if constexpr (PAYLOAD) {
+#pragma unroll
+      for (int r = 0; r < R; ++r)
+        if (t + TS_THREADS * r < n) o2p[b + t + TS_THREADS * r] = (int32_t)id[r];
+    }
+    return true;
+  }
 
   const uint32_t nb = (uint32_t)n;
   BucketMap bucket;
@@ -244,10 +263,10 @@
   return true;
 }
 
-template <int R>
-__global__ void __launch_bounds__(TS_THREADS, R <= 4 ? 8 : 1)
-tile_depth_sort_kernel(const int32_t* __restrict__ ranges, uint64_t* __restrict__ srt, int32_t* __restrict__ o2p,
-                       uint64_t* __restrict__ alt, int lo, int hi, int32_t* __restrict__ run_stats) {
+template <int R, bool PAYLOAD>
+__device__ __forceinline__ void tile_depth_sort_body(const int32_t* __restrict__ ranges, uint64_t* __restrict__ srt,
+                                                     int32_t* __restrict__ o2p, uint64_t* __restrict__ alt, int lo, int hi,
+                                                     int32_t* __restrict__ run_stats) {
   constexpr int CAP = TS_THREADS * R;
   __shared__ uint64_t pairs[CAP];
   __shared__ uint32_t cnt[CAP];
@@ -256,7 +275,7 @@
   const int64_t b = ranges[2 * tile];
   const int n = ranges[2 * tile + 1] - (int32_t)b;
   if (n <= lo || n > hi) return;
-  const bool sorted = tile_bucket_sort<R>(srt, o2p, b, n, pairs, cnt, sh);
+  const bool sorted = tile_bucket_sort<R, PAYLOAD>(srt, o2p, b, n, pairs, cnt, sh);
   if (threadIdx.x == 0) {
     alt[b] = sorted ? 0ull : TS_DECLINED;
     if (!sorted && run_stats) atomicOr(run_stats + 2, 1);
@@ -264,10 +283,23 @@
 }
 
 template <int R>
-__global__ void __launch_bounds__(TS_THREADS)
-tile_depth_sort_long_kernel(const int32_t* __restrict__ ranges, int64_t num_tiles, uint64_t* __restrict__ srt,
-                            int32_t* __restrict__ o2p, uint64_t* __restrict__ alt, int lo, int32_t* __restrict__ run_stats,
-                            int32_t* __restrict__ run_host) {
+__global__ void __launch_bounds__(TS_THREADS, R <= 4 ? 8 : 1)
+tile_depth_sort_kernel(const int32_t* __restrict__ ranges, uint64_t* __restrict__ srt, int32_t* __restrict__ o2p,
+                       uint64_t* __restrict__ alt, int lo, int hi, int32_t* __restrict__ run_stats) {
+  tile_depth_sort_body<R, false>(ranges, srt, o2p, alt, lo, hi, run_stats);
+}
+template <int R>
+__global__ void __launch_bounds__(TS_THREADS, R <= 4 ? 8 : 1)
+tile_payload_sort_kernel(const int32_t* __restrict__ ranges, uint64_t* __restrict__ payload, int32_t* __restrict__ o2p,
+                         uint64_t* __restrict__ alt, int lo, int hi, int32_t* __restrict__ run_stats) {
+  tile_depth_sort_body<R, true>(ranges, payload, o2p, alt, lo, hi, run_stats);
+}
+
+template <int R, bool PAYLOAD>
+__device__ __forceinline__ void tile_depth_sort_long_body(const int32_t* __restrict__ ranges, int64_t num_tiles,
+                                                          uint64_t* __restrict__ srt, int32_t* __restrict__ o2p,
+                                                          uint64_t* __restrict__ alt, int lo, int32_t* __restrict__ run_stats,
+                                                          int32_t* __restrict__ run_host) {
   constexpr int CAP = TS_THREADS * R;
   static_assert(CAP >= TS_WAVES * 256, "the bucket counters double as the bounded path's digit counters");
   __shared__ uint64_t pairs[CAP];
@@ -301,14 +333,29 @@
       const int64_t b = ranges[2 * tile];
       const int n = ranges[2 * tile + 1] - (int32_t)b;
       bool sorted = false;
-      if (n <= CAP && !(entry >> 30)) sorted = tile_bucket_sort<R>(srt, o2p, b, n, pairs, cnt, sh);
+      if (n <= CAP && !(entry >> 30)) sorted = tile_bucket_sort<R, PAYLOAD>(srt, o2p, b, n, pairs, cnt, sh);
       if (!sorted) {
         __syncthreads();
-        tile_radix_sort_global(srt, o2p, alt, b, n, sh, cnt);
-      }
-      __syncthreads();
-    }
-  }
+        tile_radix_sort_global<PAYLOAD>(srt, o2p, alt, b, n, sh, cnt);
+      }
+      __syncthreads();
+    }
+  }
+}
+
+template <int R>
+__global__ void __launch_bounds__(TS_THREADS)
+tile_depth_sort_long_kernel(const int32_t* __restrict__ ranges, int64_t num_tiles, uint64_t* __restrict__ srt,
+                            int32_t* __restrict__ o2p, uint64_t* __restrict__ alt, int lo, int32_t* __restrict__ run_stats,
+                            int32_t* __restrict__ run_host) {
+  tile_depth_sort_long_body<R, false>(ranges, num_tiles, srt, o2p, alt, lo, run_stats, run_host);
+}
+template <int R>
+__global__ void __launch_bounds__(TS_THREADS)
+tile_payload_sort_long_kernel(const int32_t* __restrict__ ranges, int64_t num_tiles, uint64_t* __restrict__ payload,
+                              int32_t* __restrict__ o2p, uint64_t* __restrict__ alt, int lo, int32_t* __restrict__ run_stats,
+                              int32_t* __restrict__ run_host) {
+  tile_depth_sort_long_body<R, true>(ranges, num_tiles, payload, o2p, alt, lo, run_stats, run_host);
 }
 
 void tile_depth_sort_launch(const int32_t* tile_ranges, int64_t num_tiles, uint64_t* sorted_keys, int32_t* overlap_to_point,
@@ -324,6 +371,19 @@
       tile_ranges, num_tiles, sorted_keys, overlap_to_point, scratch, TS_THREADS * MID_R, run_stats, run_host);
 }
 
+void tile_payload_sort_launch(const int32_t* tile_ranges, int64_t num_tiles, uint64_t* sorted_payload, int32_t* overlap_to_point,
+                              uint64_t* scratch, hipStream_t s, int32_t* run_stats, int32_t* run_host) {
+  if (num_tiles <= 0) return;
+  const dim3 per_tile((unsigned)num_tiles), block(TS_THREADS);
+  tile_payload_sort_kernel<SMALL_R><<<per_tile, block, 0, s>>>(tile_ranges, sorted_payload, overlap_to_point, scratch, 0,
+                                                              TS_THREADS * SMALL_R, run_stats);
+  tile_payload_sort_kernel<MID_R><<<per_tile, block, 0, s>>>(tile_ranges, sorted_payload, overlap_to_point, scratch,
+                                                            TS_THREADS * SMALL_R, TS_THREADS * MID_R, run_stats);
+  const int64_t few = 2 * 256;
+  tile_payload_sort_long_kernel<LONG_R><<<dim3((unsigned)(num_tiles < few ? num_tiles : few)), block, 0, s>>>(
+      tile_ranges, num_tiles, sorted_payload, overlap_to_point, scratch, TS_THREADS * MID_R, run_stats, run_host);
+}
+
 }
 
 using namespace ms;
```

New measurement: 2079 Msplats/s, median of 6. 2.0% higher.
